# ZYM-PKU/UDiffText

Hardware: AMD Instinct MI355X
Metric: 512x512 50-step denoised images/sec (UDiffText hot path: conditioner + 50 CFG Euler steps + VAE decode) (higher is better)
Workload: dtype bf16; 1 GPU; 512x512, 50 Euler/DDIM(eta 0) steps, CFG 5.0, 9-char labels, noise_iters 0; global batch 4 per step sharded over 1 GPU(s) = 4 images per GPU in micro-batches of 4: every UNet call runs ONE batch of 4 (8 samples with CFG); 3 such batch(es) in flight per GPU on separate launch streams; BASELINE.json configs[1]; global_batch=4, weights=synthetic (name-keyed recipe), 1361.2 M parameters, launch=hipGraph replay of the sampler steps, in_flight=3, batches_per_unet_call=1

## Files before the change

include/udt_kernels.h:

```cpp
#ifndef UDT_KERNELS_H
#define UDT_KERNELS_H

#include <stddef.h>
#include <stdint.h>

#ifdef __cplusplus
extern "C" {
#endif

typedef enum {
  UDT_OK = 0,
  UDT_ERR_BAD_SHAPE = -1,
  UDT_ERR_BAD_ARG = -2,
  UDT_ERR_WORKSPACE = -3,
  UDT_ERR_HIP = -4,
  UDT_ERR_NO_DEVICE = -5,
  UDT_ERR_ASYNC = -6
} udt_status;

typedef enum {
  UDT_DTYPE_F32 = 0,
  UDT_DTYPE_BF16 = 1,
  UDT_DTYPE_FP8_E4M3 = 2
} udt_dtype;

#define UDT_GEMM_OUT_F32     (1 << 0)
#define UDT_GEMM_GEGLU       (1 << 1)
#define UDT_GEMM_RELU        (1 << 2)
#define UDT_GEMM_TRANSPOSED  (1 << 3)
#define UDT_GEMM_CONV        (1 << 4)
#define UDT_GEMM_SILU_OUT    (1 << 5)
#define UDT_GEMM_MX8         (1 << 7)

typedef struct {
  const void* a;
  const void* a2;
  const void* w;
  const float* bias;
  const void* residual;
  const float* rowvec;
  void* out;
  int32_t M, N, K;
  int32_t lda, ldo, ldr;
  int32_t ldw;
  int32_t batch;
  int64_t stride_a, stride_w, stride_out, stride_res;
  int32_t Hin, Win, C1, C2, Hout, Wout;
  int32_t ksize;
  int32_t stride;
  int32_t pad_t, pad_l;
  int32_t upsample;
  int32_t rows_per_batch;
  int32_t ld_rowvec;
  int32_t flags;
  float alpha;
  const float* colscale;
  const float* in_scsh;
  int32_t in_act;
  float* colstats;
  int32_t cu_share;
  const float* ln_colsum;
  float ln_eps;
  const void* a_scale;
  void* q8_out;
  void* q8_scale;
  int32_t ld_q8;
  int32_t q8_fixed_col;
  float q8_fixed_mul;
  float* rowstat_out;
  const float* rowstat_in;
  int32_t rowstat_in_parts;
} udt_gemm_desc;

size_t udt_gemm_workspace_bytes(const udt_gemm_desc* d);
int udt_gemm(const udt_gemm_desc* d, void* workspace, size_t workspace_bytes, void* stream);
int32_t udt_gemm_colstats_rows(const udt_gemm_desc* d);
int32_t udt_gemm_rowstat_parts(const udt_gemm_desc* d);
int32_t udt_gemm_q8_ok(const udt_gemm_desc* d);
int32_t udt_gemm_colstats_slots(const udt_gemm_desc* d);
int32_t udt_gemm_in_scsh_ok(const udt_gemm_desc* d);
int udt_gn_silu_conv3x3_fwd(const udt_gemm_desc* d, void* workspace, size_t workspace_bytes, void* stream);
int udt_ln_gemm_fwd(const udt_gemm_desc* d, void* workspace, size_t workspace_bytes, void* stream);
int udt_check_async_error(void* workspace, size_t workspace_bytes, void* stream);

int udt_attn_fwd(const void* q, const void* k, const void* vt, void* o,
                 int32_t batch, int32_t heads, int32_t nq, int32_t nk,
                 int32_t ldq, int32_t ldk, int32_t ldvt, int32_t ldo,
                 int64_t q_bstride, int64_t k_bstride, int64_t vt_bstride, int64_t o_bstride,
                 float scale, void* stream);

int udt_xattn_fwd(const void* q, const void* k, const void* v, void* o, float* probs,
                  int32_t batch, int32_t heads, int32_t head_dim, int32_t nq, int32_t L,
                  int32_t ldq, int32_t ldkv, int32_t ldo, float scale, void* stream);

int udt_attn_rowv_fwd(const void* q, const void* k, const void* v, void* o,
                      int32_t batch, int32_t heads, int32_t nq, int32_t nk,
                      int32_t ldq, int32_t ldk, int32_t ldv, int32_t ldo,
                      int64_t q_bstride, int64_t k_bstride, int64_t v_bstride, int64_t o_bstride,
                      float scale, void* stream);
int udt_attn_rowv_q8_fwd(const void* q, const void* k, const void* v, void* o,
                         int32_t batch, int32_t heads, int32_t nq, int32_t nk,
                         int32_t ldq, int32_t ldk, int32_t ldv, int32_t ldo,
                         int64_t q_bstride, int64_t k_bstride, int64_t v_bstride, int64_t o_bstride,
                         float scale, void* q8_out, void* q8_scale, int32_t ld_q8, void* stream);

int udt_attn_mx8_fwd(const void* qkv8, const void* qkv_scale, void* o, int32_t batch, int32_t heads, int32_t n,
                     int32_t ld8, int32_t ldo, float scale, float v_inv, void* q8_out, void* q8_scale, int32_t ld_q8,
                     void* stream);

int udt_attn512_fwd(const void* q, const void* k, const void* v, void* o,
                    int32_t batch, int32_t nq, int32_t nk,
                    int32_t ldq, int32_t ldk, int32_t ldv, int32_t ldo,
                    int64_t q_bstride, int64_t k_bstride, int64_t v_bstride, int64_t o_bstride,
                    float scale, void* stream);

size_t udt_attn512_workspace_bytes(int32_t batch, int32_t nq, int32_t nk);
int udt_attn512_split_fwd(const void* q, const void* k, const void* v, void* o,
                          int32_t batch, int32_t nq, int32_t nk,
                          int32_t ldq, int32_t ldk, int32_t ldv, int32_t ldo,
                          int64_t q_bstride, int64_t k_bstride, int64_t v_bstride, int64_t o_bstride,
                          float scale, void* workspace, size_t workspace_bytes, void* stream);

int udt_mattn_fwd(const void* q, const void* k, const void* v, void* o, const float* mask, const uint8_t* kpm,
                  int32_t batch, int32_t heads, int32_t head_dim, int32_t nq, int32_t lk,
                  int32_t ldq, int32_t ldk, int32_t ldv, int32_t ldo, int32_t ldmask,
                  int64_t q_bstride, int64_t k_bstride, int64_t v_bstride, int64_t o_bstride, float scale, void* stream);

int32_t udt_tattn_hp(int32_t heads);
int udt_tattn_prepare(const void* kv, int32_t ldkv, const void* wq, int32_t ldwq, const void* wo, int32_t ldwo,
                      const float* gamma, const float* beta, void* A, float* sc, void* BmT, int32_t B, int32_t L,
                      int32_t C, int32_t heads, float scale, void* stream);
int udt_tattn_fused(const void* x, void* out, const void* A, const float* sc, const void* BmT, const float* bias,
                    int32_t B, int32_t n_tok, int32_t C, int32_t heads, int32_t zero_samples, float eps, void* stream);
int32_t udt_tattn_rowstat_parts(int32_t B, int32_t n_tok, int32_t C);
int udt_tattn_fused_q8(const void* x, void* out, const void* A, const float* sc, const void* BmT, const float* bias,
                       int32_t B, int32_t n_tok, int32_t C, int32_t heads, int32_t zero_samples, float eps, void* q8_out,
                       void* q8_scale, float* rowstat_out, void* stream);

int udt_softmax_rows(void* x, int64_t rows, int32_t cols, int32_t ld, void* stream);

int32_t udt_gn_nchunks(int64_t HW, int32_t C);
int udt_gn_stats(const void* x, const void* x2, float* partials, int32_t B, int64_t HW, int32_t C, int32_t C2,
                 int32_t G, void* stream);
int udt_gn_apply(const void* x, const void* x2, void* y, const float* partials, const float* gamma,
                 const float* beta, int32_t B, int64_t HW, int32_t C, int32_t C2, int32_t G, float eps, int32_t act,
                 void* stream);
int32_t udt_gn_strip_ok(int32_t B, int64_t HW, int32_t C1, int32_t C2, int32_t G);
int udt_gn_strip(const void* x, const void* x2, void* y, const float* gamma, const float* beta, int32_t B, int64_t HW,
                 int32_t C1, int32_t C2, int32_t G, float eps, int32_t act, void* stream);

int udt_gn_finalize(const float* stats1, int32_t slots1, int32_t C1, const float* stats2, int32_t slots2, int32_t C2,
                    const float* gamma, const float* beta, float* scsh, int32_t B, int64_t HW, int32_t G, float eps,
                    void* stream);

int udt_gn_apply_scsh(const void* x, const void* x2, void* y, const float* scsh, int32_t B, int64_t HW, int32_t C1,
                      int32_t C2, int32_t act, void* stream);

int udt_gn_strip_stats(const void* x, const void* x2, void* y, const float* stats1, int32_t slots1, const float* stats2,
                       int32_t slots2, const float* gamma, const float* beta, int32_t B, int64_t HW, int32_t C1, int32_t C2,
                       int32_t G, float eps, int32_t act, void* stream);

int udt_layernorm(const void* x, void* y, const float* gamma, const float* beta,
                  int64_t rows, int32_t C, float eps, void* stream);
int udt_unet_input(const float* x, void* xin, int32_t B, int32_t hw, int32_t cpad, float c_in, void* stream);
int udt_cfg_euler_step(float* x, const float* eps, float* denoised_out, int32_t B, int32_t hw, int32_t ld_eps,
                       float c_out, float sigma, float sigma_next, float cfg_scale, void* stream);
typedef struct {
  float kx, kd, ka, kp, kn;
  float c_out, scale;
} udt_sampler_coefs;
int udt_cfg_sampler_step(const float* xin, const float* eps, const float* aux, const float* prev, const float* noise,
                         float* xout, float* denoised_out, int32_t B, int32_t hw, int32_t ld_eps, udt_sampler_coefs k,
                         void* stream);
#define UDT_MULTISTEP_MAX 8
typedef struct {
  float c_out, scale, sigma;
  int32_t n;
  float k[UDT_MULTISTEP_MAX];
  const float* hist[UDT_MULTISTEP_MAX];
} udt_multistep_coefs;
int udt_cfg_multistep_step(const float* xin, const float* eps, float* xout, float* d_out, int32_t B, int32_t hw,
                           int32_t ld_eps, udt_multistep_coefs k, void* stream);
int udt_posterior_sample(const float* moments, const float* noise, float* z, int32_t B, int32_t hw, int32_t ldm,
                         float scale, void* stream);
int udt_nchw_to_nhwc(const float* x, void* y, int32_t B, int32_t C, int64_t HW, int32_t cpad, float scale,
                     void* stream);
int udt_nhwc_to_nchw(const void* x, float* y, int32_t B, int32_t C, int64_t HW, int32_t ld, int32_t src_is_f32,
                     void* stream);
int udt_nhwc_set_channels(const float* src, void* dst, int32_t B, int32_t C, int64_t HW, int32_t cpad, int32_t c0,
                          void* stream);
int udt_embed_tokens(const int32_t* idx, const float* table, const float* pe, void* out, int32_t n_tok, int32_t L,
                     int32_t D, void* stream);
int udt_timestep_embedding(const float* t, void* out, int32_t n, int32_t dim, void* stream);
int udt_mask_downsample(const float* mask, float* out, int32_t B, int32_t H, int32_t W, void* stream);
int udt_local_loss(const float* probs, const float* mask, const float* seg_mask, const float* gkernel9,
                   float* loss_accum, int32_t B, int32_t heads, int32_t size, int32_t L, int32_t seg_l,
                   int32_t Hm, int32_t Wm, void* stream);
int udt_local_loss_tiled(const float* probs, const float* mask, const float* seg_mask, const float* gkernel9,
                         float* loss_accum, int32_t n_samples, int32_t mask_batch, int32_t heads, int32_t size, int32_t L,
                         int32_t seg_l, int32_t Hm, int32_t Wm, void* stream);
int udt_attn_bwd(const void* q, const void* k, const void* v, const void* o, const void* d_o, void* dq, void* dk, void* dv,
                 float* lse_ws, float* dsum_ws, int32_t batch, int32_t heads, int32_t n, int32_t ldq, int32_t ldo, int32_t ldd,
                 float scale, void* stream);
int udt_xattn_bwd(const void* k, const void* v, const float* probs, const float* d_probs, const void* d_o, void* dq, int32_t batch,
                  int32_t heads, int32_t head_dim, int32_t nq, int32_t L, int32_t ldkv, int32_t ldo, int32_t lddq, float scale,
                  void* stream);
int udt_local_loss_bwd(const float* probs, const float* mask, const float* seg_mask, const float* gkernel9, float* d_probs,
                       float* loss_accum, float* scratch , int32_t n_samples,
                       int32_t mask_batch, int32_t heads, int32_t size, int32_t L, int32_t seg_l, int32_t Hm, int32_t Wm, float weight,
                       void* stream);
int udt_local_loss_bwd_hw(const float* probs, const float* mask, const float* seg_mask, const float* gkernel9, float* d_probs,
                          float* loss_accum, float* scratch , int32_t n_samples, int32_t mask_batch,
                          int32_t heads, int32_t h, int32_t w, int32_t L, int32_t seg_l, int32_t Hm, int32_t Wm, float weight,
                          void* stream);
int udt_local_loss_tiled_hw(const float* probs, const float* mask, const float* seg_mask, const float* gkernel9, float* loss_accum,
                            float* scratch , int32_t n_samples, int32_t mask_batch, int32_t heads,
                            int32_t h, int32_t w, int32_t L, int32_t seg_l, int32_t Hm, int32_t Wm, void* stream);
int udt_layernorm_bwd(const void* x, const void* dy, const float* gamma, const void* add, void* dx, int64_t rows, int32_t C, float eps,
                      void* stream);
int udt_gn_bwd(const void* x, const void* dy, const float* gamma, const float* beta, const void* add, void* dx, float* partials, int32_t B,
               int32_t HW, int32_t C, int32_t groups, float eps, int32_t silu, void* stream);
int udt_geglu_fwd(const void* ag, void* out, int64_t rows, int32_t inner, void* stream);
int udt_geglu_bwd(const void* ag, const void* dy, void* dag, int64_t rows, int32_t inner, void* stream);
int udt_sum2x2_bf16(const void* dy, void* dx, int32_t B, int32_t H, int32_t W, int32_t C, void* stream);
int udt_center_tokens(const float* x, void* out, int32_t B, int32_t L, int32_t D, void* stream);
int udt_transpose_bf16(const void* in, void* out, int32_t R, int32_t C, int32_t ld, int32_t Rp, void* stream);
int udt_reduce_rows_f32(const float* in, float* out, int32_t P, int64_t n, int32_t accumulate, void* stream);
int32_t udt_colparts(int64_t rows);
int udt_colsum_bf16(const void* x, float* partials, float* out, int64_t rows, int32_t C, void* stream);
int udt_ln_param_grad(const void* x, const void* dy, float* partials, float* dgamma_dbeta, int64_t rows, int32_t C, float eps, void* stream);
int32_t udt_wgrad_splits(int64_t R, int32_t N, int32_t K);
int udt_wgrad_bf16(const void* dy, const void* x, float* dw, float* partials, int64_t R, int32_t N, int32_t K, int32_t ldy, int32_t ldx,
                   void* stream);
// ... 55 lines not shown
```

udifftext_amd/csrc/gemm.hip:

```cpp
#include "common.h"
#include <stdio.h>
#include <stdlib.h>
#include <string.h>
#include <atomic>
#include <cmath>

hipError_t udt_lean_launch_gemm(int cfg, const void* lparams, int smem, int G, int geglu, int ln, hipStream_t s);
hipError_t udt_lean_launch_conv3(const void* c3params, hipStream_t s);

namespace {
#include "tile_common.h"

struct GemmParams {
  const uint16_t* a;
  const uint16_t* a2;
  const uint16_t* w;
  const uint16_t* zero;
  const float* bias;
  const uint16_t* res;
  const float* rowvec;
  void* out;
  const float* colscale;
  const float* in_scsh;
  float* colstats;
// ... 728 lines not shown
  if (mx8 || emit) {
    if (conv1 || d->rowvec || mode == 0 || (mode > 0 && mode != 1)) return false;
    if (mx8 && (!d->a_scale || d->K % 128 != 0 || d->lda % 16 != 0 || (d->ldw > 0 && d->ldw % 16 != 0))) return false;
    if (mx8 && ln && (!d->rowstat_in || d->rowstat_in_parts <= 0)) return false;
    if (!mx8 && geglu) return false;
    if (mx8 && geglu && !(ln && emit)) return false;
    if (mx8 && !geglu && ln && emit && d->rowstat_out) return false;
    if (emit && (want_stats || !d->q8_scale || d->ld_q8 % 8 != 0 || d->N % (geglu ? 64 : 32) != 0)) return false;
    if (d->rowstat_out && (!emit || geglu)) return false;
    if (d->q8_fixed_col > 0 && (!emit || geglu || d->q8_fixed_col % 32 != 0 || !(d->q8_fixed_mul > 0.f))) return false;
    if ((reinterpret_cast<uintptr_t>(d->q8_out) | reinterpret_cast<uintptr_t>(d->colscale)) & 15) return false;
  } else if (d->rowstat_out || d->rowstat_in) {
    return false;
  }
  const int KT = mx8 ? 128 : BK;
  if (d->N <= 64 || d->N % 8 != 0 || d->K % KT != 0 || (!conv1 && d->lda % 8 != 0) || (d->ldo % 8 != 0 && d->out)) return false;
  if (d->residual && d->ldr % 8 != 0) return false;
  if (geglu && (d->N % 64 != 0 || d->residual || d->rowvec)) return false;
  const long long ldw = d->ldw > 0 ? d->ldw : d->K;
  const long long lda_eff = conv1 ? (d->C1 > d->C2 ? d->C1 : d->C2) : d->lda;
  if ((long long)d->M * lda_eff * 2 >= (1LL << 31) || (long long)d->N * ldw * 2 >= (1LL << 31)) return false;
  if (d->M >= (1 << 28)) return false;
  if ((reinterpret_cast<uintptr_t>(d->out) | reinterpret_cast<uintptr_t>(d->residual) | reinterpret_cast<uintptr_t>(d->bias) |
       reinterpret_cast<uintptr_t>(d->rowvec) | reinterpret_cast<uintptr_t>(d->ln_colsum)) & 15) return false;
  if (d->rowvec && ((d->ld_rowvec > 0 ? d->ld_rowvec : d->N) % 4 != 0)) return false;
  if (mode > 0 && mode != 1 && mode != 6 && mode != 7) return false;
  if (!mx8 && (!emit || (ln && !geglu && !d->rowstat_out)) && (mode == 7 || (mode < 0 && rowres_on()))) {
    const bool emit_fits = !emit || ((d->q8_fixed_col <= 0 || d->q8_fixed_col % 64 == 0) && (long long)d->M * d->ld_q8 < (1LL << 31) &&
                                     (long long)d->M * (d->out ? d->ldo : 0) * 2 < (1LL << 31) && (long long)((d->N + 127) / 128) * d->M * 4 < (1LL << 31));
    if (ln && !want_stats && d->K == 320 && d->N % 64 == 0 && !d->residual && !d->rowvec && !conv1 && emit_fits &&
        (reinterpret_cast<uintptr_t>(d->a) & 15) == 0) {
      const int tiles_m = (d->M + 255) / 256, chunks = d->N / 64;
      int ns = (device_cus() + tiles_m - 1) / tiles_m;
      if (ns > chunks / 4) ns = chunks / 4;
      const int cmax = geglu ? 20 : 16;
      const int ns_min = (chunks + cmax - 1) / cmax;
      if (ns < ns_min) ns = ns_min;
      const long long wgs = (long long)tiles_m * ns;
      if (ns >= 1 && (mode == 7 || emit || (geglu ? wgs * 4 >= 3LL * device_cus() : wgs >= device_cus()))) {
        t.cfg = 7; t.stats_rows = 0; t.nw = 4; t.bm = 256; t.bn = 64; t.smem = 0;
        t.tiles_m = tiles_m; t.kt_per = (chunks + ns - 1) / ns; t.tiles_n = (chunks + t.kt_per - 1) / t.kt_per;
        t.tiles = t.tiles_m * t.tiles_n; t.nkt = d->K / BK; t.splitk = 1; t.n_block = 1;
        t.G = round_workgroups(t.tiles);
        return true;
      }
    }
    if (mode == 7 || (emit && ln)) return false;
  }
  t.cfg = (mode > 0) ? mode : 1;
  if (!mx8 && !emit) {
  if (!geglu && d->N % 160 == 0 && d->N % 128 != 0 && t.cfg == 1) t.cfg = 5;
  if (mode <= 0 && d->N >= 768 && (long long)((d->M + 255) / 256) * ((d->N + 255) / 256) >= 2LL * device_cus() &&
      (d->cu_share <= 1 || lean256_under_lanes())) t.cfg = 6;
  }
  t.stats_rows = 0;
  if (want_stats) {
    if (t.cfg != 1 && t.cfg != 5) {
      if (mode > 0) return false;
      t.cfg = (d->N % 160 == 0 && d->N % 128 != 0) ? 5 : 1;
    }
    if (mx8) t.cfg = 1;
    t.stats_rows = t.cfg == 1 ? 64 : 32;
    const int rpb = d->rows_per_batch > 0 ? d->rows_per_batch : d->M;
    if (rpb % t.stats_rows != 0) return false;
  }
  switch (t.cfg) {
    case 1: t.nw = 4; t.bm = 128; t.bn = 128; t.smem = 2 * (128 + 128) * ROW_BYTES; break;
    case 5: t.nw = 4; t.bm = 128; t.bn = 160; t.smem = 128 * 160 * 4; break;
    case 6: t.nw = 8; t.bm = 256; t.bn = 256; t.smem = 2 * (256 + 256) * ROW_BYTES; break;
    default: return false;
  }
  {
    const int epi = (t.cfg == 6 ? t.bm * t.bn : t.bm * t.bn * 4) + ((ln && t.cfg != 5) ? t.bm * 8 : 0);
    if (t.smem < epi) t.smem = epi;
  }
  t.tiles_m = (d->M + t.bm - 1) / t.bm;
  t.tiles_n = (d->N + t.bn - 1) / t.bn;
  t.tiles = t.tiles_m * t.tiles_n;
  t.nkt = d->K / KT;
  int slots = device_cus() * ((t.cfg == 1 || t.cfg == 5) ? 2 : 1) / share_of(d);
  if (slots < 1) slots = 1;
  int sk = 1;
  const int knob = lean_splitk_knob();
  if (!ln && t.tiles <= 1023) {
    if (knob > 1) sk = knob;
    else if (knob < 0 && t.tiles * 2 <= slots && t.nkt >= (mx8 ? 20 : 40)) { sk = slots / t.tiles; if (sk > t.nkt / (mx8 ? 8 : 16)) sk = t.nkt / (mx8 ? 8 : 16); }
    if (sk > t.nkt / 4) sk = t.nkt / 4;
    while (sk > 1 && (long long)t.tiles * sk * t.bm * t.bn * 4 > (64LL << 20)) --sk;
    if (sk < 1) sk = 1;
  }
  t.kt_per = (t.nkt + sk - 1) / sk;
  t.splitk = (t.nkt + t.kt_per - 1) / t.kt_per;
  const int units = t.tiles * t.splitk;
  t.G = round_workgroups(units);
  int nb = g_n_block.load(std::memory_order_relaxed);
  if (nb <= 0) nb = (t.tiles_m <= 8) ? t.tiles_n : 8;
  if (nb > t.tiles_n) nb = t.tiles_n;
  t.n_block = nb;
  return true;
}

size_t lean_workspace(const LeanPlan& t) {
  return t.splitk > 1 ? G8_HEADER_BYTES + (size_t)t.tiles * t.splitk * t.bm * t.bn * sizeof(float) : 0;
}

std::atomic<int> g_lean_conv{-1};
std::atomic<int> g_wide_conv{-2};
int wide_conv_mode() {
  int v = g_wide_conv.load(std::memory_order_relaxed);
  if (v == -2) {
    const char* e = getenv("UDT_WIDE_CONV");
    v = e ? atoi(e) : -1;
    g_wide_conv.store(v, std::memory_order_relaxed);
  }
  return v;
}
#ifdef UDT_MEASURE
std::atomic<int> g_lconv_dbg{0};
#endif

std::atomic<int> g_wide_lanes_eff{-2};
double wide_lanes_eff() {
  int v = g_wide_lanes_eff.load(std::memory_order_relaxed);
  if (v == -2) {
    const char* e = getenv("UDT_WIDE_LANES_EFF");
    v = e ? atoi(e) : 70;
    g_wide_lanes_eff.store(v, std::memory_order_relaxed);
  }
  return v / 100.0;
}

int conv_chunk_slices(long long tiles, int slots, int chunks, int knob) {
  long long sk = 1;
  if (tiles <= 1023) {
    if (knob > 1) { sk = knob; if (sk > chunks) sk = chunks; }
    else if (knob < 0 && tiles * 2 <= slots && chunks >= 10) { sk = slots / tiles; if (sk > chunks / 4) sk = chunks / 4; }
    if (sk < 1) sk = 1;
  }
  return (int)sk;
}

bool lean_conv_plan(const udt_gemm_desc* d, lg::C3Params& c, bool want_stats) {
  int on = g_lean_conv.load(std::memory_order_relaxed);
  if (on < 0) {
    const char* e = getenv("UDT_LEAN_CONV");
    on = (e && e[0] == '0') ? 0 : 1;
    g_lean_conv.store(on, std::memory_order_relaxed);
  }
  if (!on || lean_mode() == 0) return false;
  if (d->flags != UDT_GEMM_CONV || d->ksize != 3 || d->stride != 1 || d->pad_t != 1 || d->pad_l != 1) return false;
  if (d->C2 != 0 || d->in_scsh || d->colscale || d->batch > 1) return false;
  if (want_stats && !lean_stats_enabled()) return false;
  if (d->N < 128 || d->N % 8 != 0 || d->C1 <= 0 || d->C1 % 64 != 0) return false;
  const bool ups = d->upsample != 0;
  if (d->Hout != (d->Hin << (ups ? 1 : 0)) || d->Wout != (d->Win << (ups ? 1 : 0))) return false;
  c.bn = 128; c.wgm = 2;
  bool wide = false;
  int wide_slots = device_cus();
  {
    const int wm = wide_conv_mode();
    if (wm != 0 && !ups && d->N % 160 == 0 && d->Wout % 16 == 0 && d->Hout % 16 == 0) {
      const int cus = device_cus(), share = d->cu_share > 1 ? d->cu_share : 1;
      wide_slots = cus / share > 0 ? cus / share : 1;
      const long long wt = (long long)(d->M / 256) * (d->N / 160);
      const long long sk = conv_chunk_slices(wt, wide_slots, d->C1 / 64, lean_splitk_knob());
      const long long units = wt * sk;
      const long long rounds = (units + cus - 1) / cus;
      const double eff = units > cus ? (double)units / (double)(rounds * cus) : ((double)units * share >= cus ? 1.0 : (double)units * share / cus);
      wide = (wm > 0) || (sk <= 2 && eff >= ((share >= 3 && share_of(d) >= 3) ? wide_lanes_eff() : 0.85));
    }
  }
  if (wide) { c.geo = 3; c.tw = 16; c.th = 16; c.bn = 160; c.wgm = 4; }
  else if (d->Wout % 16 == 0 && d->Hout % 8 == 0) { c.geo = ups ? 2 : 0; c.tw = 16; c.th = 8; }
  else if (!ups && d->Wout % 8 == 0 && d->Hout % 8 == 0) { c.geo = 1; c.tw = 8; c.th = 8; }
  else return false;
  if (d->ldo % 8 != 0 || (d->residual && d->ldr % 8 != 0)) return false;
  const long long ldw = d->ldw > 0 ? d->ldw : d->K;
  if ((long long)d->M * d->C1 * 2 >= (1LL << 31) || (long long)d->N * ldw * 2 >= (1LL << 31)) return false;
  if ((reinterpret_cast<uintptr_t>(d->out) | reinterpret_cast<uintptr_t>(d->residual) | reinterpret_cast<uintptr_t>(d->bias) |
       reinterpret_cast<uintptr_t>(d->rowvec)) & 15) return false;
  if (d->rowvec && ((d->ld_rowvec > 0 ? d->ld_rowvec : d->N) % 4 != 0)) return false;
  c.dbg = 0;
#ifdef UDT_MEASURE
  c.dbg = g_lconv_dbg.load(std::memory_order_relaxed);
#endif
  c.N = d->N; c.C = d->C1; c.H = d->Hin; c.W = d->Win; c.B = d->M / (d->Hout * d->Wout);
  c.ldw = (int)ldw; c.ldo = d->ldo; c.ldr = d->ldr; c.ldrv = d->ld_rowvec > 0 ? d->ld_rowvec : d->N;
  c.alpha = d->alpha;
  c.tiles_x = d->Wout / c.tw; c.tiles_y = d->Hout / c.th;
  c.tiles_m = c.B * c.tiles_x * c.tiles_y;
  c.tiles_n = (d->N + c.bn - 1) / c.bn;
  c.tiles = c.tiles_m * c.tiles_n;
  c.chunks = c.C / 64;
  const int slots = c.geo == 3 ? wide_slots : (2 * device_cus() / share_of(d) > 0 ? 2 * device_cus() / share_of(d) : 1);
  int sk = conv_chunk_slices(c.tiles, slots, c.chunks, lean_splitk_knob());
  while (sk > 1 && (long long)c.tiles * sk * c.tw * c.th * c.bn * 4 > (64LL << 20)) --sk;
  c.ch_per = (c.chunks + sk - 1) / sk;
  c.splitk = (c.chunks + c.ch_per - 1) / c.ch_per;
  c.G = round_workgroups(c.tiles * c.splitk);
  {
    const double patch = (double)((ups ? c.tw / 2 : c.tw) + 2) * ((ups ? c.th / 2 : c.th) + 2) * c.C * 2.0, wtile = 9.0 * c.bn * c.C * 2.0;
    int nb = g_n_block.load(std::memory_order_relaxed);
    if (nb <= 0) nb = (int)(std::sqrt(64.0 * patch / wtile) + 0.5);
    if (nb < 1) nb = 1;
    if (nb > c.tiles_n) nb = c.tiles_n;
    c.n_block = nb;
  }
  c.a_bytes = (unsigned)((long long)c.B * d->Hin * d->Win * d->C1 * 2);
  c.w_bytes = (unsigned)((long long)d->N * ldw * 2);
  c.counters = nullptr; c.slabs = nullptr;
  return true;
}

size_t lean_conv_workspace(const lg::C3Params& c) {
  return c.splitk > 1 ? G8_HEADER_BYTES + (size_t)c.tiles * c.splitk * c.tw * c.th * c.bn * sizeof(float) : 0;
}

bool lean_stats_probe(const udt_gemm_desc* d, int& rows, int& slots) {
  if (d->in_scsh) return false;
  {
    lg::C3Params c3;
    if (lean_conv_plan(d, c3, true)) {
      rows = c3.tw * c3.th / c3.wgm;
      slots = c3.tiles_m * c3.wgm;
      return true;
    }
  }
  if ((d->flags & UDT_GEMM_CONV) && d->ksize == 3) return false;
  LeanPlan lt;
  if (lean_plan(d, lt, true)) {
    rows = lt.stats_rows;
    slots = lt.tiles_m * (lt.bm / lt.stats_rows);
    return true;
  }
  return false;
}
}

extern "C" int udt_debug_set(const char* key, int32_t value) {
  if (!key) return UDT_ERR_BAD_ARG;
  if (!strcmp(key, "n_block")) { g_n_block.store(value); return UDT_OK; }
  if (!strcmp(key, "rows_epi")) { g_rows_epi.store(value ? 1 : 0); return UDT_OK; }
  if (!strcmp(key, "lean")) { g_lean.store(value < 0 ? -2 : value); return UDT_OK; }
  if (!strcmp(key, "rowres")) { g_rowres.store(value < 0 ? 1 : (value ? 1 : 0)); return UDT_OK; }
  if (!strcmp(key, "wide_lanes_eff")) { g_wide_lanes_eff.store(value < 0 ? -2 : value); return UDT_OK; }
  if (!strcmp(key, "conv_n4")) { g_conv_n4.store(value < 0 ? -2 : (value ? 1 : 0)); return UDT_OK; }
  if (!strcmp(key, "lean256_lanes")) { g_lean256_lanes.store(value < 0 ? -2 : (value ? 1 : 0)); return UDT_OK; }
  if (!strcmp(key, "lean_splitk")) { g_lean_splitk.store(value); return UDT_OK; }
  if (!strcmp(key, "share_splitk")) { g_share_splitk.store(value < 0 ? -2 : (value ? 1 : 0)); return UDT_OK; }
  if (!strcmp(key, "lean_conv")) { g_lean_conv.store(value < 0 ? -1 : (value ? 1 : 0)); return UDT_OK; }
  if (!strcmp(key, "wide_conv")) { g_wide_conv.store(value < 0 ? -1 : (value ? 1 : 0)); return UDT_OK; }
#ifdef UDT_MEASURE
  if (!strcmp(key, "lconv_dbg")) { g_lconv_dbg.store(value); return UDT_OK; }
  static const struct { const char* k; int bit; } bits[] = {{"no_xchg", 28}, {"no_epi", 27}, {"no_store", 26}, {"no_res", 25},
                                                            {"no_bias", 24}, {"no_fast", 22}};
  for (const auto& b : bits)
    if (!strcmp(key, b.k)) {
      int cur = g_dbg_bits.load();
      g_dbg_bits.store((cur & ~(1 << b.bit)) | (value ? (1 << b.bit) : 0));
      return UDT_OK;
    }
#endif
  return UDT_ERR_BAD_ARG;
}

extern "C" int udt_check_async_error(void* workspace, size_t workspace_bytes, void* stream) {
  if (!workspace || workspace_bytes < G8_HEADER_BYTES) return UDT_ERR_BAD_ARG;
  hipStream_t s = reinterpret_cast<hipStream_t>(stream);
  int err = 0;
  hipError_t e = hipMemcpyAsync(&err, reinterpret_cast<int*>(workspace) + 1023, sizeof(int), hipMemcpyDeviceToHost, s);
  if (e == hipSuccess) e = hipStreamSynchronize(s);
  if (e != hipSuccess) return udt_set_hip_error(e);
  if (err == 0) return UDT_OK;
  e = hipMemsetAsync(workspace, 0, G8_HEADER_BYTES, s);
  if (e == hipSuccess) e = hipStreamSynchronize(s);
  if (e != hipSuccess) return udt_set_hip_error(e);
  return UDT_ERR_ASYNC;
}

extern "C" int32_t udt_gemm_colstats_rows(const udt_gemm_desc* d) { return d ? colstats_rows(d) : 0; }
extern "C" int32_t udt_gemm_colstats_slots(const udt_gemm_desc* d) { return d ? colstats_slots(d) : 0; }
extern "C" int32_t udt_gemm_q8_ok(const udt_gemm_desc* d) {
  if (!d || !d->q8_out || d->M <= 0 || d->N <= 0 || d->K <= 0) return 0;
  LeanPlan lt;
  return lean_plan(d, lt, d->colstats != nullptr) ? 1 : 0;
}

extern "C" int32_t udt_gemm_rowstat_parts(const udt_gemm_desc* d) {
  if (!d || d->M <= 0 || d->N <= 0 || d->K <= 0) return 0;
  udt_gemm_desc t = *d;
  alignas(16) static const uint64_t probe_dst[2] = {0, 0};
  if (!t.q8_out) { t.q8_out = const_cast<uint64_t*>(probe_dst); t.q8_scale = const_cast<uint64_t*>(probe_dst); if (t.ld_q8 <= 0) t.ld_q8 = (t.N + 15) / 16 * 16; }
  LeanPlan lt;
  if (!lean_plan(&t, lt, false) || lt.cfg != 1 || (d->flags & UDT_GEMM_GEGLU)) return 0;
  return (d->N + 63) / 64;
}
extern "C" int32_t udt_gemm_in_scsh_ok(const udt_gemm_desc* d) {
  if (!d || d->K <= 0 || d->K % BK != 0) return 0;
  c3p::Geo ge;
  return conv3p_geometry(d, ge, true) ? 1 : 0;
}

extern "C" int udt_gn_silu_conv3x3_fwd(const udt_gemm_desc* d, void* workspace, size_t workspace_bytes, void* stream) {
  if (!d || !(d->flags & UDT_GEMM_CONV) || d->ksize != 3 || d->stride != 1 || d->pad_t != 1 || d->pad_l != 1 || !d->in_scsh)
    return UDT_ERR_BAD_ARG;
  return udt_gemm(d, workspace, workspace_bytes, stream);
}

extern "C" int udt_ln_gemm_fwd(const udt_gemm_desc* d, void* workspace, size_t workspace_bytes, void* stream) {
  if (!d || !d->ln_colsum || !d->bias || !(d->ln_eps > 0.f)) return UDT_ERR_BAD_ARG;
  LeanPlan lt;
  if (!lean_plan(d, lt, false)) return UDT_ERR_BAD_SHAPE;
  return udt_gemm(d, workspace, workspace_bytes, stream);
}

extern "C" size_t udt_gemm_workspace_bytes(const udt_gemm_desc* d) {
  if (!d || d->K <= 0 || d->M <= 0 || d->N <= 0 || d->K % k_tile(d) != 0) return 0;
  if (conv_n4_applies(d)) return 0;
  {
    LeanPlan lt;
    if (lean_plan(d, lt, d->colstats != nullptr)) return lean_workspace(lt);
    lg::C3Params c3;
    if (lean_conv_plan(d, c3, d->colstats != nullptr)) return lean_conv_workspace(c3);
  }
  {
    c3p::Geo ge;
    if (conv3p_geometry(d, ge, d->in_scsh != nullptr)) {
      TilePlan t3 = plan_tiles3p(d, ge);
      if (!t3.fixup) return 0;
      return G8_HEADER_BYTES + (size_t)t3.G * t3.bm * t3.bn * sizeof(float);
    }
  }
  if (use_gemm8(d)) {
    TilePlan t8 = plan_tiles8(d);
    if (!t8.fixup) return 0;
    return G8_HEADER_BYTES + (size_t)t8.G * t8.bm * t8.bn * sizeof(float);
  }
  TilePlan t = plan_tiles(d);
  if (t.bm != 256 || !t.fixup) return 0;
  return G8_HEADER_BYTES + (size_t)t.G * 2 * SLAB_FLOATS * sizeof(float);
}

extern "C" int udt_gemm(const udt_gemm_desc* d, void* workspace, size_t workspace_bytes, void* stream) {
  if (!d || !d->a || !d->w) return UDT_ERR_BAD_ARG;
  if (d->M <= 0 || d->N <= 0 || d->K <= 0) return UDT_ERR_BAD_SHAPE;
  if (d->K % k_tile(d) != 0) return UDT_ERR_BAD_SHAPE;
  if (d->N % 4 != 0) return UDT_ERR_BAD_SHAPE;
  const bool mx8 = (d->flags & UDT_GEMM_MX8) != 0;
  if (mx8 || d->q8_out || d->rowstat_out || d->rowstat_in) {
    LeanPlan lt8;
    if (!lean_plan(d, lt8, d->colstats != nullptr)) return UDT_ERR_BAD_ARG;
  } else if (d->colscale) {
    return UDT_ERR_BAD_ARG;
  }
  const bool conv = (d->flags & UDT_GEMM_CONV) != 0;
  const bool trans = (d->flags & UDT_GEMM_TRANSPOSED) != 0;
  const int batch = d->batch > 0 ? d->batch : 1;
  if (conv) {
    if (d->ksize != 1 && d->ksize != 3) return UDT_ERR_BAD_SHAPE;
    if (d->C1 <= 0 || d->C1 % BK != 0 || d->C2 % BK != 0) return UDT_ERR_BAD_SHAPE;
    if (d->C2 > 0 && !d->a2) return UDT_ERR_BAD_ARG;
    if (d->K != d->ksize * d->ksize * (d->C1 + d->C2)) return UDT_ERR_BAD_SHAPE;
    if (d->Hout <= 0 || d->Wout <= 0 || d->M % (d->Hout * d->Wout) != 0) return UDT_ERR_BAD_SHAPE;
    if (d->stride != 1 && d->stride != 2) return UDT_ERR_BAD_SHAPE;
    if (trans || batch != 1) return UDT_ERR_BAD_ARG;
  } else {
    if (d->lda < d->K || d->lda % 8 != 0) return UDT_ERR_BAD_SHAPE;
  }
  if (!d->out && !d->q8_out) return UDT_ERR_BAD_ARG;
  if (trans) {
    if (d->rows_per_batch <= 0 || d->rows_per_batch % 4 != 0 || d->M % d->rows_per_batch != 0)
      return UDT_ERR_BAD_SHAPE;
    if (d->flags & (UDT_GEMM_OUT_F32 | UDT_GEMM_GEGLU | UDT_GEMM_RELU | UDT_GEMM_SILU_OUT)) return UDT_ERR_BAD_ARG;
    if (d->residual || d->rowvec || batch != 1) return UDT_ERR_BAD_ARG;
  } else {
    if (d->ldo % 4 != 0) return UDT_ERR_BAD_SHAPE;
    if (d->residual && d->ldr % 4 != 0) return UDT_ERR_BAD_SHAPE;
  }
  if (d->flags & UDT_GEMM_GEGLU) {
    if (d->N % 64 != 0 || (d->flags & UDT_GEMM_OUT_F32) || d->residual || d->rowvec) return UDT_ERR_BAD_ARG;
  }
  if (d->rowvec && d->rows_per_batch <= 0) return UDT_ERR_BAD_ARG;

  hipStream_t s = reinterpret_cast<hipStream_t>(stream);
  if (conv_n4_applies(d)) {
    cn4::Params cp;
    cp.a = reinterpret_cast<const uint16_t*>(d->a); cp.w = reinterpret_cast<const uint16_t*>(d->w); cp.bias = d->bias;
    cp.out = reinterpret_cast<float*>(d->out);
    cp.B = d->M / (d->Hout * d->Wout); cp.H = d->Hin; cp.W = d->Win; cp.C = d->C1;
    cp.ldw = d->ldw > 0 ? d->ldw : d->K; cp.ldo = d->ldo;
    cp.tiles_x = (d->Win + 7) / 8; cp.tiles_y = (d->Hin + 7) / 8;
    const size_t smem = (size_t)100 * (d->C1 + 8) * 2 + (size_t)4 * 9 * d->C1 * 2;
    static AttrOnce once;
    hipError_t ea = once.ensure(reinterpret_cast<const void*>(cn4::conv3x3_n4_kernel), 100 * (512 + 8) * 2 + 4 * 9 * 512 * 2);
    if (ea != hipSuccess) return udt_set_hip_error(ea);
    UdtProfScope profn(0, s);
    if (profn.rec) {
      char tag[96];
      snprintf(tag, sizeof(tag), "conv_n4 M=%d N=%d K=%d %dx%d", d->M, d->N, d->K, d->Hin, d->Win);
      udt_prof_tag(profn.rec, tag);
    }
    hipLaunchKernelGGL(cn4::conv3x3_n4_kernel, dim3((unsigned)(cp.B * cp.tiles_x * cp.tiles_y)), dim3(256), smem, s, cp);
    UDT_CHECK_LAUNCH();
    return UDT_OK;
  }
  TilePlan t = plan_tiles(d);

  GemmParams p;
  p.a = reinterpret_cast<const uint16_t*>(d->a);
  p.a2 = reinterpret_cast<const uint16_t*>(d->a2);
  p.w = reinterpret_cast<const uint16_t*>(d->w);
  p.zero = udt_zero_page();
  if (!p.zero) return UDT_ERR_HIP;
  p.bias = d->bias;
  p.res = reinterpret_cast<const uint16_t*>(d->residual);
  p.rowvec = d->rowvec;
  p.out = d->out;
  p.colscale = d->colscale;
  p.in_scsh = d->in_scsh;
  p.in_act = d->in_act;
  p.colstats = d->colstats;
  p.slabs = nullptr;
  if (d->colstats && colstats_rows(d) == 0) return UDT_ERR_BAD_ARG;
  if (d->in_scsh && !udt_gemm_in_scsh_ok(d)) return UDT_ERR_BAD_ARG;
  if (d->in_act != 0 && d->in_act != 1) return UDT_ERR_BAD_ARG;
  p.M = d->M; p.N = d->N; p.K = d->K;
  p.lda = d->lda; p.ldo = d->ldo; p.ldr = d->ldr;
  p.ldw = d->ldw > 0 ? d->ldw : d->K;
  if (p.ldw < d->K || p.ldw % 8 != 0) return UDT_ERR_BAD_SHAPE;
  if (mx8 && d->lda < d->K) return UDT_ERR_BAD_SHAPE;
  p.sA = d->stride_a; p.sW = d->stride_w; p.sO = d->stride_out; p.sR = d->stride_res;
  p.Hin = d->Hin; p.Win = d->Win; p.C1 = d->C1; p.C2 = d->C2; p.Hout = d->Hout; p.Wout = d->Wout;
  p.ksz = d->ksize; p.stride = d->stride; p.pad_t = d->pad_t; p.pad_l = d->pad_l; p.ups = d->upsample ? 1 : 0;
  p.rows_per_batch = d->rows_per_batch > 0 ? d->rows_per_batch : d->M;
  p.ldrv = d->ld_rowvec > 0 ? d->ld_rowvec : d->N;
  if (d->flags & ~PUBLIC_FLAGS) return UDT_ERR_BAD_ARG;
  p.flags = d->flags | (g_rows_epi.load(std::memory_order_relaxed) ? 0 : INTERNAL_DIRECT_EPI);
#ifdef UDT_MEASURE
  p.flags |= g_dbg_bits.load(std::memory_order_relaxed);
#endif
  p.n_block = 1;
  p.alpha = d->alpha;
  const int cls = (conv && d->ksize == 3) ? 0 : 1;
  {
    LeanPlan lt;
    if (lean_plan(d, lt, d->colstats != nullptr)) {
      lg::LParams lp;
      lp.colstats = d->colstats;
      const bool conv1 = (d->flags & UDT_GEMM_CONV) != 0;
      lp.a = p.a; lp.a2 = (conv1 && d->C2 > 0) ? p.a2 : nullptr; lp.w = p.w; lp.bias = p.bias; lp.res = p.res; lp.rowvec = p.rowvec;
      lp.ln_s = d->ln_colsum;
      lp.out = reinterpret_cast<uint16_t*>(d->out);
      lp.M = d->M; lp.N = d->N; lp.K = d->K;
      lp.lda = conv1 ? d->C1 : p.lda; lp.ldw = p.ldw; lp.ldo = p.ldo; lp.ldr = p.ldr; lp.ldrv = p.ldrv; lp.rows_per_batch = p.rows_per_batch;
      lp.lda2 = conv1 ? d->C2 : 0;
      lp.kt_split = (conv1 && d->C2 > 0) ? d->C1 / BK : lt.nkt;
      lp.a2_bytes = (unsigned)((long long)d->M * (conv1 ? d->C2 : 0) * 2);
      lp.alpha = d->alpha; lp.ln_eps = d->ln_eps;
      lp.tiles_m = lt.tiles_m; lp.tiles_n = lt.tiles_n; lp.n_block = lt.n_block; lp.tiles = lt.tiles;
      lp.nkt = lt.nkt; lp.splitk = lt.splitk; lp.kt_per = lt.kt_per;
      lp.a_bytes = (unsigned)((long long)d->M * lp.lda * elem_bytes(d));
      lp.w_bytes = (unsigned)((long long)d->N * p.ldw * elem_bytes(d));
      lp.a_scale = mx8 ? reinterpret_cast<const uint32_t*>(d->a_scale) : nullptr;
      lp.colscale = d->colscale;
      lp.rowstat_in = d->rowstat_in; lp.rowstat_in_parts = d->rowstat_in_parts;
      lp.q8_out = reinterpret_cast<uint8_t*>(d->q8_out); lp.q8_scale = reinterpret_cast<uint32_t*>(d->q8_scale); lp.ld_q8 = d->ld_q8;
      lp.rowstat_out = d->rowstat_out;
      lp.q8_fixed_col = d->q8_fixed_col > 0 ? d->q8_fixed_col : 0x7fffffff;
      lp.q8_fixed_mul = d->q8_fixed_mul;
      lp.G = lt.G;
      lp.counters = nullptr; lp.slabs = nullptr;
      if (lt.splitk > 1) {
        if (!workspace || workspace_bytes < lean_workspace(lt)) return UDT_ERR_WORKSPACE;
        lp.counters = reinterpret_cast<int*>(workspace);
        lp.slabs = reinterpret_cast<float*>(reinterpret_cast<char*>(workspace) + G8_HEADER_BYTES);
      }
      UdtProfScope profl(cls, s);
      if (profl.rec) {
        char tag[96];
        snprintf(tag, sizeof(tag), "lean%d%s%s M=%d N=%d K=%d fl=0x%x ln=%d tile=%dx%d units=%d splitk=%d", lt.cfg, mx8 ? "-mx8" : "", d->q8_out ? "+q8" : "",
                 d->M, d->N, d->K, d->flags, d->ln_colsum ? 1 : 0, lt.bm, lt.bn, lt.tiles * lt.splitk, lt.splitk);
        udt_prof_tag(profl.rec, tag);
      }
      const bool geglu = (d->flags & UDT_GEMM_GEGLU) != 0, ln = d->ln_colsum != nullptr;
      hipError_t el;
      el = udt_lean_launch_gemm(lt.cfg, &lp, lt.smem, lt.G, geglu ? 1 : 0, ln ? 1 : 0, s);
      if (el != hipSuccess) return udt_set_hip_error(el);
      return UDT_OK;
    }
  }
  if (d->ln_colsum) return UDT_ERR_BAD_ARG;
  {
    lg::C3Params c3;
    if (lean_conv_plan(d, c3, d->colstats != nullptr)) {
      c3.colstats = d->colstats;
      c3.a = p.a; c3.w = p.w; c3.bias = p.bias; c3.res = p.res; c3.rowvec = p.rowvec; c3.out = reinterpret_cast<uint16_t*>(d->out);
      if (c3.splitk > 1) {
        if (!workspace || workspace_bytes < lean_conv_workspace(c3)) return UDT_ERR_WORKSPACE;
        c3.counters = reinterpret_cast<int*>(workspace);
        c3.slabs = reinterpret_cast<float*>(reinterpret_cast<char*>(workspace) + G8_HEADER_BYTES);
      }
      UdtProfScope profc(cls, s);
      if (profc.rec) {
        char tag[96];
        snprintf(tag, sizeof(tag), "%s%s M=%d N=%d K=%d %dx%d tile=%dx%d units=%d splitk=%d nb=%d", c3.geo == 3 ? "wconv3" : "lconv3", d->upsample ? "+up" : "", d->M, d->N, d->K,
                 d->Hin, d->Win, c3.tw, c3.th, c3.tiles * c3.splitk, c3.splitk, c3.n_block);
        udt_prof_tag(profc.rec, tag);
      }
      const hipError_t ec = udt_lean_launch_conv3(&c3, s);
      if (ec != hipSuccess) return udt_set_hip_error(ec);
      return UDT_OK;
    }
  }
  {
    c3p::CParams cp;
    if (conv3p_geometry(d, cp.geo, d->in_scsh != nullptr)) {
      const TilePlan t3 = plan_tiles3p(d, cp.geo);
      p.tiles_m = t3.tiles_m; p.tiles_n = t3.tiles_n; p.tiles_per_batch = t3.tiles_m * t3.tiles_n;
      {
        const double patch = (double)cp.geo.prows_img * cp.geo.NI * cp.geo.C * 2.0;
        const double wtile = 9.0 * t3.bn * cp.geo.C * 2.0;
        const double S = (double)(t3.tiles < t3.G ? t3.tiles : t3.G) / 8.0;
        int nb = (int)(std::sqrt((S < 1.0 ? 1.0 : S) * patch / wtile) + 0.5);
        if (nb < 1) nb = 1;
        if (nb > t3.tiles_n) nb = t3.tiles_n;
        p.n_block = nb;
      }
      p.n_ktiles = t3.nkt;
      p.total_iters = t3.total;
      p.iters_per_wg = t3.ipw;
      p.G = t3.G;
      const long long in_px = (long long)cp.geo.B * d->Hin * d->Win;
      cp.base.a_bytes = (unsigned)(in_px * d->C1 * 2);
      cp.a2_bytes = (unsigned)((long long)d->M * d->C2 * 2);
      cp.scsh_bytes = (unsigned)((long long)cp.geo.B * cp.geo.chunks * 512);
      cp.base.w_bytes = (unsigned)((long long)d->N * p.ldw * 2);
      cp.base.g = p;
      cp.base.flags = nullptr; cp.base.err = nullptr; cp.base.slab_base = nullptr;
      if (t3.fixup) {
        const size_t need = G8_HEADER_BYTES + (size_t)t3.G * t3.bm * t3.bn * sizeof(float);
        if (!workspace || workspace_bytes < need) return UDT_ERR_WORKSPACE;
        cp.base.flags = reinterpret_cast<int*>(workspace);
        cp.base.err = cp.base.flags + 1023;
        cp.base.slab_base = reinterpret_cast<float*>(reinterpret_cast<char*>(workspace) + G8_HEADER_BYTES);
      }
      UdtProfScope prof3(cls, s);
      if (prof3.rec) {
        char tag[96];
        snprintf(tag, sizeof(tag), "conv3p%s%s M=%d N=%d K=%d %dx%d tile=%dx%dx%d bn=%d G=%d ipw=%d", d->in_scsh ? "+gn" : "", d->upsample ? "+up" : "", d->M,
                 d->N, d->K, d->Hin, d->Win, cp.geo.TW, cp.geo.TH, cp.geo.NI, t3.bn, t3.G, t3.ipw);
        udt_prof_tag(prof3.rec, tag);
      }
      hipError_t e3;
      const bool st3 = d->colstats != nullptr;
      if (t3.bn == 160) e3 = st3 ? launch3p<8, 1, 1, 5, true, true>(cp, t3, s) : launch3p<8, 1, 1, 5, true, false>(cp, t3, s);
      else e3 = st3 ? launch3p<4, 2, 2, 2, true, true>(cp, t3, s) : launch3p<4, 2, 2, 2, true, false>(cp, t3, s);
      if (e3 != hipSuccess) return udt_set_hip_error(e3);
      return UDT_OK;
    }
  }
  if (use_gemm8(d)) {
    const TilePlan t8 = plan_tiles8(d);
    p.tiles_m = t8.tiles_m; p.tiles_n = t8.tiles_n; p.tiles_per_batch = t8.tiles_m * t8.tiles_n;
    const int n_block_knob = g_n_block.load(std::memory_order_relaxed);
    if (n_block_knob != 0 && !conv) {
      const long long wt = (long long)t8.bn * d->K * elem_bytes(d);
      long long nb = 1;
      if (n_block_knob > 0) nb = n_block_knob;
      else if (t8.tiles_m <= 8 || trans) nb = t8.tiles_n;
      else if (t8.tiles_n >= 8) nb = (4LL << 20) / (wt > 0 ? wt : 1);
      if (nb < 1) nb = 1;
      if (nb > t8.tiles_n) nb = t8.tiles_n;
      p.n_block = (int)nb;
    }
    p.n_ktiles = t8.nkt;
    p.total_iters = t8.total;
    p.iters_per_wg = t8.ipw;
    p.G = t8.G;
    g8::Params pp;
    pp.g = p;
    pp.flags = nullptr; pp.err = nullptr; pp.slab_base = nullptr;
    pp.a_bytes = conv ? 0u : (unsigned)((long long)d->M * d->lda * elem_bytes(d));
    pp.w_bytes = (unsigned)((long long)d->N * p.ldw * elem_bytes(d));
    if (t8.fixup) {
      const size_t need = G8_HEADER_BYTES + (size_t)t8.G * t8.bm * t8.bn * sizeof(float);
      if (!workspace || workspace_bytes < need) return UDT_ERR_WORKSPACE;
      pp.flags = reinterpret_cast<int*>(workspace);
      pp.err = pp.flags + 1023;
      pp.slab_base = reinterpret_cast<float*>(reinterpret_cast<char*>(workspace) + G8_HEADER_BYTES);
    }
    UdtProfScope prof8(cls, s);
    if (prof8.rec) {
      char tag[96];
      snprintf(tag, sizeof(tag), "gemm8 M=%d N=%d K=%d conv=%d ks=%d fl=0x%x tile=%dx%d G=%d ipw=%d b=%d",
               d->M, d->N, d->K, conv ? 1 : 0, d->ksize, d->flags, t8.bm, t8.bn, t8.G, t8.ipw, batch);
      udt_prof_tag(prof8.rec, tag);
    }
    hipError_t e8;
    const bool st = d->colstats != nullptr;
    if (t8.bn == 160) {
      if (st) e8 = conv ? launch8<8, 1, 1, 5, true, false, true>(pp, t8, s) : launch8<8, 1, 1, 5, false, false, true>(pp, t8, s);
      else e8 = conv ? launch8<8, 1, 1, 5, true, false>(pp, t8, s) : launch8<8, 1, 1, 5, false, false>(pp, t8, s);
    } else if (trans) {
      e8 = launch8<4, 2, 2, 2, false, true>(pp, t8, s);
    } else if (st) {
      e8 = conv ? launch8<4, 2, 2, 2, true, false, true>(pp, t8, s) : launch8<4, 2, 2, 2, false, false, true>(pp, t8, s);
    } else {
      e8 = conv ? launch8<4, 2, 2, 2, true, false>(pp, t8, s) : launch8<4, 2, 2, 2, false, false>(pp, t8, s);
    }
    if (e8 != hipSuccess) return udt_set_hip_error(e8);
    return UDT_OK;
  }

  p.tiles_m = t.tiles_m; p.tiles_n = t.tiles_n; p.tiles_per_batch = t.tiles_m * t.tiles_n;
  p.n_ktiles = t.nkt;
  p.total_iters = t.total;
  p.iters_per_wg = t.ipw;
  p.G = t.G;

  if (t.fixup) {
    const size_t need = G8_HEADER_BYTES + (size_t)t.G * 2 * SLAB_FLOATS * sizeof(float);
    if (!workspace || workspace_bytes < need) return UDT_ERR_WORKSPACE;
    p.slabs = reinterpret_cast<float*>(reinterpret_cast<char*>(workspace) + G8_HEADER_BYTES);
  }

  UdtProfScope prof(cls, s);
  if (prof.rec) {
    char tag[96];
    snprintf(tag, sizeof(tag), "gemm M=%d N=%d K=%d conv=%d ks=%d fl=0x%x tile=%dx%d G=%d ipw=%d b=%d", d->M, d->N, d->K,
             conv ? 1 : 0, d->ksize, d->flags, t.bm, t.bn, t.G, t.ipw, batch);
    udt_prof_tag(prof.rec, tag);
  }

  if (t.bm != 256) return UDT_ERR_BAD_SHAPE;
  const hipError_t e = conv ? launch_cfg<256, 64, 4, 1, true, false>(p, t, s) : launch_cfg<256, 64, 4, 1, false, false>(p, t, s);
  if (e != hipSuccess) return udt_set_hip_error(e);
  return UDT_OK;
}
```

udifftext_amd/csrc/lean.h:

```cpp
#pragma once

namespace lg {

using g8::wait_vm;
UDT_DEVINL void raw_barrier() {
  asm volatile("s_waitcnt lgkmcnt(0)" ::: "memory");
  __builtin_amdgcn_s_barrier();
  asm volatile("" ::: "memory");
}
using g8::buf_lds16;
using g8::OOB;

typedef __attribute__((ext_vector_type(2))) __bf16 bf2_t;
UDT_DEVINL float dot2_bf16(uint32_t a, uint32_t b, float c) {
  return __builtin_amdgcn_fdot2_f32_bf16(__builtin_bit_cast(bf2_t, a), __builtin_bit_cast(bf2_t, b), c, false);
}

template <int CPR, int RPI>
UDT_DEVINL void wave_colstats(char* wl, int lane, const float (&cs)[8], const float (&cq)[8], float* dst, bool col_ok) {
#pragma unroll
  for (int h = 0; h < 2; ++h) {
    f32x4 a = {cs[4 * h + 0], cs[4 * h + 1], cs[4 * h + 2], cs[4 * h + 3]};
    f32x4 b = {cq[4 * h + 0], cq[4 * h + 1], cq[4 * h + 2], cq[4 * h + 3]};
    *reinterpret_cast<f32x4*>(wl + lane * 64 + h * 16) = a;
// ... 450 lines not shown
      if (p.res) {
#pragma unroll
        for (int i = 0; i < NIT; ++i) {
          const int row = i * RPI + rl;
          const int m = m0 + row0 + prow0 + row;
          u32x4 z = {0u, 0u, 0u, 0u};
          rv[i] = z;
          if (col_ok && row < PROWS && m < p.M) rv[i] = *reinterpret_cast<const u32x4*>(p.res + (long long)m * p.ldr + n);
        }
      }
#pragma unroll
      for (int tb = 0; tb < TMB; ++tb) {
        const int row = tb * 32 + l31;
#pragma unroll
        for (int tn = 0; tn < TN; ++tn)
#pragma unroll
          for (int q = 0; q < 4; ++q) {
            const int chunk = (tn * 8 + q * 2 + hi) ^ (row & 7);
            const f32x16& a16 = acc[pass * TMB + tb][tn];
            f32x4 v = {a16[q * 4 + 0], a16[q * 4 + 1], a16[q * 4 + 2], a16[q * 4 + 3]};
            *reinterpret_cast<f32x4*>(wl + row * EROW + chunk * 16) = v;
          }
      }
#pragma unroll
      for (int i = 0; i < NIT; ++i) {
        const int row = i * RPI + rl;
        const int m = m0 + row0 + prow0 + row;
        const bool ok = col_ok && row < PROWS && m < p.M;
        const int rr = row < PROWS ? row : 0;
        const char* rp = wl + rr * EROW;
        const int sw = rr & 7;
        const f32x4 v0 = *reinterpret_cast<const f32x4*>(rp + (((2 * c8) ^ sw) << 4));
        const f32x4 v1 = *reinterpret_cast<const f32x4*>(rp + (((2 * c8 + 1) ^ sw) << 4));
        float o[8];
#pragma unroll
        for (int j = 0; j < 4; ++j) {
          o[j] = v0[j];
          o[4 + j] = v1[j];
        }
        if constexpr (FP8) {
#pragma unroll
          for (int j = 0; j < 4; ++j) o[j] *= w0[j], o[4 + j] *= w1[j];
        }
        if constexpr (LN) {
          float mean, rstd;
          row_stats(prow0 + rr, mean, rstd);
#pragma unroll
          for (int j = 0; j < 4; ++j) {
            o[j] = rstd * (o[j] - mean * s0[j]);
            o[4 + j] = rstd * (o[4 + j] - mean * s1[j]);
          }
        }
#pragma unroll
        for (int j = 0; j < 4; ++j) {
          o[j] = o[j] * p.alpha + b0[j];
          o[4 + j] = o[4 + j] * p.alpha + b1[j];
        }
        if (p.rowvec && ok) {
          const float* rvp = p.rowvec + (long long)(m / p.rows_per_batch) * p.ldrv + n;
          const f32x4 r0 = *reinterpret_cast<const f32x4*>(rvp);
          const f32x4 r1 = *reinterpret_cast<const f32x4*>(rvp + 4);
#pragma unroll
          for (int j = 0; j < 4; ++j) {
            o[j] += r0[j];
            o[4 + j] += r1[j];
          }
        }
        if (p.res) {
#pragma unroll
          for (int j = 0; j < 4; ++j) {
            o[2 * j] += bf16_lo(rv[i][j]);
            o[2 * j + 1] += bf16_hi(rv[i][j]);
          }
        }
        if constexpr (EMIT) {
          {
            const u32x4 rb = {pack_bf16x2(o[0], o[1]), pack_bf16x2(o[2], o[3]), pack_bf16x2(o[4], o[5]), pack_bf16x2(o[6], o[7])};
#pragma unroll
            for (int j = 0; j < 4; ++j) o[2 * j] = bf16_lo(rb[j]), o[2 * j + 1] = bf16_hi(rb[j]);
          }
          uint32_t sb;
          u32x2 q8 = mx8_quant_row8(o, sb);
          if (n >= p.q8_fixed_col) {
            q8 = e4m3_fixed_row8(o, p.q8_fixed_mul);
            sb = 127u;
          }
          float ps = 0.f, pq = 0.f;
          if (p.rowstat_out) {
            static_assert(CPR == 8 || CPR == 16, "row statistics: 64- or 128-column wave blocks");
#pragma unroll
            for (int j = 0; j < 8; ++j) ps += o[j], pq += o[j] * o[j];
            ps = dpp_add<0xB1>(ps); pq = dpp_add<0xB1>(pq);
            ps = dpp_add<0x4E>(ps); pq = dpp_add<0x4E>(pq);
            ps = dpp_add<0x141>(ps); pq = dpp_add<0x141>(pq);
            if constexpr (CPR == 16) { ps = dpp_add<0x140>(ps); pq = dpp_add<0x140>(pq); }
          }
          if (ok) {
            *reinterpret_cast<u32x2*>(p.q8_out + (long long)m * p.ld_q8 + n) = q8;
            if ((c8 & 3) == 0) reinterpret_cast<uint8_t*>(p.q8_scale)[((long long)(n >> 7) * p.M + m) * 4 + ((n >> 5) & 3)] = (uint8_t)sb;
            if (p.rowstat_out && c8 == 0) {
              f32x2 st2 = {ps, pq};
              reinterpret_cast<f32x2*>(p.rowstat_out)[(long long)((n0 + col0) / WCOLS) * p.M + m] = st2;
            }
          }
        }
        if (ok) {
          u32x4 pk = {pack_bf16x2(o[0], o[1]), pack_bf16x2(o[2], o[3]), pack_bf16x2(o[4], o[5]), pack_bf16x2(o[6], o[7])};
          if (!EMIT || p.out) *reinterpret_cast<u32x4*>(p.out + (long long)m * p.ldo + n) = pk;
          if constexpr (STATS) {
#pragma unroll
            for (int j = 0; j < 4; ++j) {
              const float a = bf16_lo(pk[j]), bb = bf16_hi(pk[j]);
              cs[2 * j] += a; cq[2 * j] += a * a;
              cs[2 * j + 1] += bb; cq[2 * j + 1] += bb * bb;
            }
          }
        }
      }
    }
    if constexpr (STATS) {
      const int slot = (m0 + row0) / WROWS;
      wave_colstats<CPR, RPI>(wl, lane, cs, cq, p.colstats + ((long long)slot * p.N + n) * 2, col_ok);
    }
  }
}


template <int MAXN>
UDT_DEVINL void wait_vm_upto(int n) {
  if constexpr (MAXN == 0) wait_vm<0>();
  else {
    if (n >= MAXN) wait_vm<MAXN>();
    else wait_vm_upto<MAXN - 1>(n);
  }
}

template <int TW, int TH, bool UPS>
struct C3Geo {
  static constexpr int PX = TW * TH;
  static constexpr int TM = PX / 64;
  static constexpr int PW = (UPS ? TW / 2 : TW) + 2, PH = (UPS ? TH / 2 : TH) + 2;
  static constexpr int PROWS = PW * PH;
  static constexpr int PIECES = (PROWS + 7) / 8;
  static constexpr int PATCH_BYTES = PIECES * 1024;
  static constexpr int W_BYTES = 128 * ROW_BYTES;
  static constexpr int NRING = (3 * W_BYTES + 2 * PATCH_BYTES <= 80 * 1024) ? 3 : 2;
  static constexpr int RING = NRING * W_BYTES + 2 * PATCH_BYTES;
  static constexpr int STAGING = 4 * TM * 32 * 256;
  static constexpr int SMEM = RING > STAGING ? RING : STAGING;
  static_assert(PX == 128 || PX == 64, "128 or 64 output pixels per workgroup");
  static_assert(SMEM <= 80 * 1024, "two workgroups per CU");
};

template <int TW, int TH, bool UPS, bool STATS = false>
__global__ void __launch_bounds__(256, 2) lconv3_kernel(const C3Params p) {
  using Geo = C3Geo<TW, TH, UPS>;
  constexpr int NW = 4, TM = Geo::TM, TN = 2, BN = 128, BMPX = Geo::PX;
  constexpr int C3_PW = Geo::PW, C3_PROWS = Geo::PROWS, C3_PIECES = Geo::PIECES, C3_PATCH_BYTES = Geo::PATCH_BYTES;
  constexpr int C3_W_BYTES = Geo::W_BYTES, C3_TW = TW, C3_TH = TH;
  constexpr int WROWS = TM * 32;
  constexpr int WP = 4;
  constexpr int PP = (C3_PIECES + NW - 1) / NW;
  constexpr int EROW = 64 * 4;
  extern __shared__ __attribute__((aligned(16))) char smem[];
  char* const wring = smem;
  constexpr int NR = Geo::NRING;
  char* const patches = smem + NR * C3_W_BYTES;

  const int tid = threadIdx.x;
  const int wave = __builtin_amdgcn_readfirstlane(tid >> 6);
  const int lane = tid & 63;
  const int l31 = lane & 31;
  const int hi = lane >> 5;
  const int l3 = lane >> 3;
  const int pslot = lane & 7;
  const int wm = wave >> 1, wn = wave & 1;
  const int row0 = wm * WROWS, col0 = wn * 64;
  const int swz_w = (l31 >> 1) & 7;
  const int w_frag_row = (col0 + l31) * ROW_BYTES;

  const int unit = range_index(blockIdx.x, p.G);
  if (unit >= p.tiles * p.splitk) return;
  const int tile = unit / p.splitk;
  const int slice = unit - tile * p.splitk;
  int tile_m, n0;
  {
    const int per_block = p.tiles_m * p.n_block;
    const int blk = tile / per_block;
    const int r = tile - blk * per_block;
    int nbw = p.tiles_n - blk * p.n_block;
    if (nbw > p.n_block) nbw = p.n_block;
    tile_m = r / nbw;
    n0 = (blk * p.n_block + (r - tile_m * nbw)) * BN;
  }
  const int per_img = p.tiles_x * p.tiles_y;
  const int b = tile_m / per_img;
  const int rt = tile_m - b * per_img;
  const int ty = rt / p.tiles_x;
  const int y0 = ty * C3_TH, x0 = (rt - ty * p.tiles_x) * C3_TW;
  const int c0 = slice * p.ch_per;
  int c1 = c0 + p.ch_per;
  if (c1 > p.chunks) c1 = p.chunks;

  const __amdgpu_buffer_rsrc_t rsrc_a = __builtin_amdgcn_make_buffer_rsrc(const_cast<uint16_t*>(p.a), 0, p.a_bytes, 0x00020000);
  const __amdgpu_buffer_rsrc_t rsrc_w = __builtin_amdgcn_make_buffer_rsrc(const_cast<uint16_t*>(p.w), 0, p.w_bytes, 0x00020000);
  auto patch_swz = [](int prow, int yy) { return ((prow - 2 * yy) >> 1) & 7; };
  unsigned w_voff[WP], p_voff[PP];
  int p_piece[PP];
#pragma unroll
  for (int i = 0; i < WP; ++i) {
    const int row = (wave + NW * i) * 8 + l3;
    const int kw = (pslot ^ ((row >> 1) & 7)) * 8;
    const int n = n0 + row;
    w_voff[i] = (n < p.N) ? (unsigned)(((long long)n * p.ldw + kw) * 2) : OOB;
  }
#pragma unroll
  for (int i = 0; i < PP; ++i) {
    int idx = wave + NW * i;
    while (idx >= C3_PIECES) idx -= NW;
    p_piece[i] = idx;
    const int prow = idx * 8 + l3;
    const int yy = prow / C3_PW;
    const int xx = prow - yy * C3_PW;
    const int gy = (UPS ? (y0 >> 1) : y0) + yy - 1, gx = (UPS ? (x0 >> 1) : x0) + xx - 1;
    const bool ok = (prow < C3_PROWS) && ((unsigned)gy < (unsigned)p.H) && ((unsigned)gx < (unsigned)p.W);
    const int koff = (pslot ^ patch_swz(prow, yy)) * 8;
    p_voff[i] = ok ? (unsigned)(((((long long)b * p.H + gy) * p.W + gx) * p.C + koff) * 2) : OOB;
  }
  int a_prow[TM], a_py[TM];
#pragma unroll
  for (int tm = 0; tm < TM; ++tm) {
    const int ml = row0 + tm * 32 + l31;
    const int py = ml / TW, px = ml - py * TW;
    a_py[tm] = py;
    a_prow[tm] = UPS ? (py | (px << 16)) : (py * C3_PW + px);
  }
  auto issue_w = [&](int st, int c, int tap) {
    const int soff = (tap * p.C + c * 64) * 2;
    char* wbuf = wring + st * C3_W_BYTES;
#pragma unroll
    for (int i = 0; i < WP; ++i) buf_lds16(rsrc_w, wbuf + (wave + NW * i) * 1024, w_voff[i], soff);
  };
  auto issue_patch = [&](int c) {
    char* pbuf = patches + (c & 1) * C3_PATCH_BYTES;
#pragma unroll
    for (int i = 0; i < PP; ++i) buf_lds16(rsrc_a, pbuf + p_piece[i] * 1024, p_voff[i], c * 128);
  };

  f32x16 acc[TM][TN];
#pragma unroll
  for (int i = 0; i < TM; ++i)
#pragma unroll
    for (int j = 0; j < TN; ++j)
#pragma unroll
      for (int r = 0; r < 16; ++r) acc[i][j][r] = 0.f;

  issue_patch(c0);
#pragma unroll
  for (int j = 0; j < NR - 1; ++j) issue_w(j, c0, j);
  int st = 0;
  for (int c = c0; c < c1; ++c) {
    const bool nxt = (c + 1 < c1);
    const char* pbuf = patches + (c & 1) * C3_PATCH_BYTES;
#pragma unroll
    for (int tap = 0; tap < 9; ++tap) {
      {
        const int w_ahead = nxt ? NR - 2 : ((8 - tap) < NR - 2 ? (8 - tap) : NR - 2);
        const bool patch_ahead = nxt && tap >= 1 && tap <= NR - 1;
        wait_vm_upto<(NR - 2) * WP + PP>(w_ahead * WP + (patch_ahead ? PP : 0));
      }
      raw_barrier();
      if (!UDT_DBG(p.dbg, 0)) {
        const int ahead = tap + NR - 1;
        int s2 = st + NR - 1;
        if (s2 >= NR) s2 -= NR;
        if (ahead < 9) issue_w(s2, c, ahead);
        else if (nxt) issue_w(s2, c + 1, ahead - 9);
      }
      if (tap == 0 && nxt && !UDT_DBG(p.dbg, 1)) issue_patch(c + 1);
      const int dy = tap / 3, dx = tap - dy * 3;
      const char* wbuf = wring + st * C3_W_BYTES;
      bf16x8_t fx[4][TM], fw[4][TN];
      if (!UDT_DBG(p.dbg, 3)) {
#pragma unroll
        for (int t = 0; t < TM; ++t) {
          int prow, yy;
          if constexpr (UPS) {
            const int py = a_prow[t] & 0xffff, px = a_prow[t] >> 16;
            yy = ((py + dy - 1) >> 1) + 1;
            prow = yy * C3_PW + (((px + dx - 1) >> 1) + 1);
          } else {
            yy = a_py[t] + dy;
            prow = a_prow[t] + dy * C3_PW + dx;
          }
          const int arow = prow * ROW_BYTES, aswz = patch_swz(prow, yy);
#pragma unroll
          for (int ks = 0; ks < 4; ++ks) fx[ks][t] = lds_read_frag(pbuf + arow + (((ks * 2 + hi) ^ aswz) << 4));
        }
#pragma unroll
        for (int ks = 0; ks < 4; ++ks) {
          const int slot = ((ks * 2 + hi) ^ swz_w) << 4;
#pragma unroll
          for (int t = 0; t < TN; ++t) fw[ks][t] = lds_read_frag(wbuf + w_frag_row + t * 32 * ROW_BYTES + slot);
        }
      }
      if (UDT_DBG(p.dbg, 2)) {
#pragma unroll
        for (int ks = 0; ks < 4; ++ks) {
#pragma unroll
          for (int tm = 0; tm < TM; ++tm) asm volatile("" ::"v"(fx[ks][tm]));
#pragma unroll
          for (int tn = 0; tn < TN; ++tn) asm volatile("" ::"v"(fw[ks][tn]));
        }
      } else {
#pragma unroll
        for (int ks = 0; ks < 4; ++ks)
#pragma unroll
          for (int tm = 0; tm < TM; ++tm)
#pragma unroll
            for (int tn = 0; tn < TN; ++tn) acc[tm][tn] = mfma32(fw[ks][tn], fx[ks][tm], acc[tm][tn]);
      }
      st = (st + 1 == NR) ? 0 : st + 1;
    }
  }
  raw_barrier();

  if (p.splitk > 1) {
    f32x4* slab = reinterpret_cast<f32x4*>(p.slabs + (long long)unit * (BMPX * BN));
#pragma unroll
    for (int tm = 0; tm < TM; ++tm)
#pragma unroll
      for (int tn = 0; tn < TN; ++tn)
#pragma unroll
        for (int q = 0; q < 4; ++q) {
          f32x4 v = {acc[tm][tn][q * 4 + 0], acc[tm][tn][q * 4 + 1], acc[tm][tn][q * 4 + 2], acc[tm][tn][q * 4 + 3]};
          store16_sc1(slab + ((tm * TN + tn) * 4 + q) * 256 + tid, v);
        }
    asm volatile("s_waitcnt vmcnt(0)" ::: "memory");
    __syncthreads();
    int* const bcast = reinterpret_cast<int*>(smem);
    if (tid == 0) {
      const int t = __hip_atomic_fetch_add(p.counters + tile, 1, __ATOMIC_RELAXED, __HIP_MEMORY_SCOPE_AGENT);
      const int last = (t == p.splitk - 1) ? 1 : 0;
      if (last) {
        __builtin_amdgcn_fence(__ATOMIC_ACQUIRE, "agent");
        __hip_atomic_store(p.counters + tile, 0, __ATOMIC_RELAXED, __HIP_MEMORY_SCOPE_AGENT);
      }
      *bcast = last;
    }
    __syncthreads();
    const bool last = *bcast != 0;
    __syncthreads();
    if (!last) return;
#pragma unroll
    for (int i = 0; i < TM; ++i)
#pragma unroll
      for (int j = 0; j < TN; ++j)
#pragma unroll
        for (int r = 0; r < 16; ++r) acc[i][j][r] = 0.f;
    for (int s = 0; s < p.splitk; ++s) {
      const f32x4* sl = reinterpret_cast<const f32x4*>(p.slabs + ((long long)tile * p.splitk + s) * (BMPX * BN));
#pragma unroll
      for (int tm = 0; tm < TM; ++tm)
#pragma unroll
        for (int tn = 0; tn < TN; ++tn)
#pragma unroll
          for (int q = 0; q < 4; ++q) {
            const f32x4 v = sl[((tm * TN + tn) * 4 + q) * 256 + tid];
#pragma unroll
            for (int r = 0; r < 4; ++r) acc[tm][tn][q * 4 + r] += v[r];
          }
    }
  }

  char* const wl = smem + wave * (WROWS * EROW);
#pragma unroll
  for (int tm = 0; tm < TM; ++tm) {
    const int row = tm * 32 + l31;
#pragma unroll
    for (int tn = 0; tn < TN; ++tn)
#pragma unroll
      for (int q = 0; q < 4; ++q) {
        const int chunk = (tn * 8 + q * 2 + hi) ^ (row & 7);
        f32x4 v = {acc[tm][tn][q * 4 + 0], acc[tm][tn][q * 4 + 1], acc[tm][tn][q * 4 + 2], acc[tm][tn][q * 4 + 3]};
        *reinterpret_cast<f32x4*>(wl + row * EROW + chunk * 16) = v;
      }
  }
  const int rl = lane >> 3, c8 = lane & 7;
  const int n = n0 + col0 + c8 * 8;
  const bool col_ok = n < p.N;
  f32x4 b0 = {0.f, 0.f, 0.f, 0.f}, b1 = b0;
  if (col_ok) {
    if (p.bias) {
      b0 = *reinterpret_cast<const f32x4*>(p.bias + n);
      b1 = *reinterpret_cast<const f32x4*>(p.bias + n + 4);
    }
    if (p.rowvec) {
      const float* rvp = p.rowvec + (long long)b * p.ldrv + n;
      const f32x4 r0 = *reinterpret_cast<const f32x4*>(rvp), r1 = *reinterpret_cast<const f32x4*>(rvp + 4);
#pragma unroll
      for (int j = 0; j < 4; ++j) b0[j] += r0[j], b1[j] += r1[j];
    }
  }
  constexpr int NIT = TM * 4;
  const int Ho = UPS ? 2 * p.H : p.H, Wo = UPS ? 2 * p.W : p.W;
  long long mrow[NIT];
#pragma unroll
  for (int i = 0; i < NIT; ++i) {
    const int ml = row0 + i * 8 + rl;
    const int py = ml / TW, px = ml - py * TW;
    mrow[i] = ((long long)b * Ho + (y0 + py)) * Wo + (x0 + px);
  }
  u32x4 rv[NIT];
  if (p.res) {
#pragma unroll
    for (int i = 0; i < NIT; ++i) {
      u32x4 z = {0u, 0u, 0u, 0u};
      rv[i] = z;
      if (col_ok) rv[i] = *reinterpret_cast<const u32x4*>(p.res + mrow[i] * p.ldr + n);
    }
  }
  float cs[8], cq[8];
#pragma unroll
  for (int j = 0; j < 8; ++j) cs[j] = cq[j] = 0.f;
#pragma unroll
  for (int i = 0; i < NIT; ++i) {
    const int row = i * 8 + rl;
    const char* rp = wl + row * EROW;
    const int sw = row & 7;
    const f32x4 v0 = *reinterpret_cast<const f32x4*>(rp + (((2 * c8) ^ sw) << 4));
    const f32x4 v1 = *reinterpret_cast<const f32x4*>(rp + (((2 * c8 + 1) ^ sw) << 4));
    float o[8];
#pragma unroll
    for (int j = 0; j < 4; ++j) {
      o[j] = v0[j] * p.alpha + b0[j];
      o[4 + j] = v1[j] * p.alpha + b1[j];
    }
    if (p.res) {
#pragma unroll
      for (int j = 0; j < 4; ++j) {
        o[2 * j] += bf16_lo(rv[i][j]);
        o[2 * j + 1] += bf16_hi(rv[i][j]);
      }
    }
    if (col_ok) {
      u32x4 pk = {pack_bf16x2(o[0], o[1]), pack_bf16x2(o[2], o[3]), pack_bf16x2(o[4], o[5]), pack_bf16x2(o[6], o[7])};
      *reinterpret_cast<u32x4*>(p.out + mrow[i] * p.ldo + n) = pk;
      if constexpr (STATS) {
#pragma unroll
        for (int j = 0; j < 4; ++j) {
          const float a = bf16_lo(pk[j]), bb = bf16_hi(pk[j]);
          cs[2 * j] += a; cq[2 * j] += a * a;
          cs[2 * j + 1] += bb; cq[2 * j + 1] += bb * bb;
        }
      }
    }
  }
  if constexpr (STATS) {
    const int slot = tile_m * 2 + wm;
    wave_colstats<8, 8>(wl, lane, cs, cq, p.colstats + ((long long)slot * p.N + n) * 2, col_ok);
  }
}

}
```

udifftext_amd/csrc/lean.hip:

```cpp
#include "common.h"
#include <stdio.h>
#include <stdlib.h>
#include <atomic>

namespace {
#include "tile_common.h"
#include "lean_params.h"
#include "lean.h"
#include "wide.h"
#include "rowres.h"

template <int NW, int WGM, int WGN, int TM, int TN, int NST, int TMB = TM>
hipError_t launch_lean(const lg::LParams& lp, int smem, int G, bool geglu, bool ln, hipStream_t s) {
  static AttrOnce once[5];
  const void* fn;
  const bool stats = lp.colstats != nullptr;
  if constexpr (NW == 4 && NST == 2) {
    if (stats) {
      fn = (const void*)lg::lgemm_kernel<NW, WGM, WGN, TM, TN, NST, false, false, TMB, true>;
      hipError_t e = once[4].ensure(fn, smem);
      if (e != hipSuccess) return e;
      void* args[] = {const_cast<lg::LParams*>(&lp)};
      return hipLaunchKernel(fn, dim3(G), dim3(NW * 64), args, smem, s);
    }
  }
  if (stats) return hipErrorInvalidValue;
  if constexpr (TN == 2) {
    fn = geglu ? (ln ? (const void*)lg::lgemm_kernel<NW, WGM, WGN, TM, TN, NST, true, true, TMB> : (const void*)lg::lgemm_kernel<NW, WGM, WGN, TM, TN, NST, true, false, TMB>)
               : (ln ? (const void*)lg::lgemm_kernel<NW, WGM, WGN, TM, TN, NST, false, true, TMB> : (const void*)lg::lgemm_kernel<NW, WGM, WGN, TM, TN, NST, false, false, TMB>);
  } else {
    fn = ln ? (const void*)lg::lgemm_kernel<NW, WGM, WGN, TM, TN, NST, false, true, TMB> : (const void*)lg::lgemm_kernel<NW, WGM, WGN, TM, TN, NST, false, false, TMB>;
  }
  hipError_t e = once[(geglu ? 2 : 0) + (ln ? 1 : 0)].ensure(fn, smem);
  if (e != hipSuccess) return e;
  void* args[] = {const_cast<lg::LParams*>(&lp)};
  return hipLaunchKernel(fn, dim3(G), dim3(NW * 64), args, smem, s);
}

template <bool GEGLU, bool LN, bool STATS, bool FP8, bool EMIT>
hipError_t launch_lean_mx8_k(const lg::LParams& lp, int smem, int G, hipStream_t s) {
  static AttrOnce once;
  const void* fn = (const void*)lg::lgemm_kernel<4, 2, 2, 2, 2, 2, GEGLU, LN, 2, STATS, FP8, EMIT>;
  hipError_t e = once.ensure(fn, smem);
  if (e != hipSuccess) return e;
  void* args[] = {const_cast<lg::LParams*>(&lp)};
  return hipLaunchKernel(fn, dim3(G), dim3(256), args, smem, s);
}
hipError_t launch_lean_mx8(const lg::LParams& lp, int smem, int G, bool geglu, bool ln, bool fp8, bool emit, hipStream_t s) {
  const bool stats = lp.colstats != nullptr;
  if (!fp8) {
    if (emit && !geglu && !ln && !stats) return launch_lean_mx8_k<false, false, false, false, true>(lp, smem, G, s);
    return hipErrorInvalidValue;
  }
  if (geglu) return (ln && emit && !stats) ? launch_lean_mx8_k<true, true, false, true, true>(lp, smem, G, s) : hipErrorInvalidValue;
  if (ln) return stats ? hipErrorInvalidValue
                 : emit ? launch_lean_mx8_k<false, true, false, true, true>(lp, smem, G, s)
                        : launch_lean_mx8_k<false, true, false, true, false>(lp, smem, G, s);
  if (stats) return emit ? hipErrorInvalidValue : launch_lean_mx8_k<false, false, true, true, false>(lp, smem, G, s);
  return emit ? launch_lean_mx8_k<false, false, false, true, true>(lp, smem, G, s) : launch_lean_mx8_k<false, false, false, true, false>(lp, smem, G, s);
}

template <int TW, int TH, bool UPS, bool STATS>
hipError_t launch_lconv3s(const lg::C3Params& c3, hipStream_t s) {
  static AttrOnce once;
  constexpr int smem = lg::C3Geo<TW, TH, UPS>::SMEM;
  hipError_t e = once.ensure(reinterpret_cast<const void*>(lg::lconv3_kernel<TW, TH, UPS, STATS>), smem);
  if (e != hipSuccess) return e;
  hipLaunchKernelGGL((lg::lconv3_kernel<TW, TH, UPS, STATS>), dim3(c3.G), dim3(256), smem, s, c3);
  return hipGetLastError();
}
template <int TW, int TH, bool UPS>
hipError_t launch_lconv3(const lg::C3Params& c3, hipStream_t s) {
  return c3.colstats ? launch_lconv3s<TW, TH, UPS, true>(c3, s) : launch_lconv3s<TW, TH, UPS, false>(c3, s);
}

template <bool STATS>
hipError_t launch_wconv3s(const lg::C3Params& c3, hipStream_t s) {
  static AttrOnce once;
  constexpr int smem = wd::WGeo::SMEM;
  hipError_t e = once.ensure(reinterpret_cast<const void*>(wd::wconv3_kernel<STATS>), smem);
  if (e != hipSuccess) return e;
  hipLaunchKernelGGL((wd::wconv3_kernel<STATS>), dim3(c3.G), dim3(256), smem, s, c3);
  return hipGetLastError();
}
template <int KT, bool GEGLU, bool EMIT = false>
hipError_t launch_rowres(const lg::LParams& lp, int G, hipStream_t s) {
  static AttrOnce once;
  constexpr int smem = rr::RGeo<KT, GEGLU>::SMEM;
  hipError_t e = once.ensure(reinterpret_cast<const void*>(rr::rgemm_kernel<KT, GEGLU, EMIT>), smem);
  if (e != hipSuccess) return e;
  hipLaunchKernelGGL((rr::rgemm_kernel<KT, GEGLU, EMIT>), dim3(G), dim3(256), smem, s, lp);
  return hipGetLastError();
}

hipError_t launch_wconv3(const lg::C3Params& c3, hipStream_t s) {
  return c3.colstats ? launch_wconv3s<true>(c3, s) : launch_wconv3s<false>(c3, s);
}

}

hipError_t udt_lean_launch_gemm(int cfg, const void* lparams, int smem, int G, int geglu, int ln, hipStream_t s) {
  const lg::LParams& lp = *static_cast<const lg::LParams*>(lparams);
  const bool fp8 = lp.a_scale != nullptr, emit = lp.q8_out != nullptr;
  if (cfg == 7 && emit && !fp8 && !geglu && ln && lp.K == 320) return launch_rowres<5, false, true>(lp, G, s);
  if (fp8 || emit) return cfg == 1 ? launch_lean_mx8(lp, smem, G, geglu != 0, ln != 0, fp8, emit, s) : hipErrorInvalidValue;
  switch (cfg) {
    case 1: return launch_lean<4, 2, 2, 2, 2, 2>(lp, smem, G, geglu != 0, ln != 0, s);
    case 6: return launch_lean<8, 2, 4, 4, 2, 2, 1>(lp, smem, G, geglu != 0, ln != 0, s);
    case 5: return geglu ? hipErrorInvalidValue : launch_lean<4, 4, 1, 1, 5, 2>(lp, smem, G, false, ln != 0, s);
    case 7:
      if (!ln || lp.K != 320) return hipErrorInvalidValue;
      return geglu ? launch_rowres<5, true>(lp, G, s) : launch_rowres<5, false>(lp, G, s);
    default: return hipErrorInvalidValue;
  }
}

hipError_t udt_lean_launch_conv3(const void* c3params, hipStream_t s) {
  const lg::C3Params& c3 = *static_cast<const lg::C3Params*>(c3params);
  return c3.geo == 3 ? launch_wconv3(c3, s) : c3.geo == 2 ? launch_lconv3<16, 8, true>(c3, s)
         : c3.geo == 1 ? launch_lconv3<8, 8, false>(c3, s) : launch_lconv3<16, 8, false>(c3, s);
}
```

udifftext_amd/csrc/lean_params.h:

```cpp
#pragma once

namespace lg {

struct LParams {
  const uint16_t* a;
  const uint16_t* a2;
  const uint16_t* w;
  const float* bias;
  const uint16_t* res;
  const float* rowvec;
  const float* ln_s;
  uint16_t* out;
  int M, N, K;
  int lda, ldw, ldo, ldr, ldrv, rows_per_batch;
  float alpha, ln_eps;
  int tiles_m, tiles_n, n_block, tiles;
  int nkt;
  int splitk, kt_per;
  unsigned a_bytes, w_bytes;
  int kt_split, lda2;
  unsigned a2_bytes;
  int G;
  int* counters;
  float* slabs;
  float* colstats;
  const uint32_t* a_scale;
  const float* colscale;
  const float* rowstat_in;
  int rowstat_in_parts;
  uint8_t* q8_out;
  uint32_t* q8_scale;
  int ld_q8;
  int q8_fixed_col;
  float q8_fixed_mul;
  float* rowstat_out;
};

struct C3Params {
  const uint16_t* a;
  const uint16_t* w;
  const float* bias;
  const uint16_t* res;
  const float* rowvec;
  uint16_t* out;
  int N, C;
  int B, H, W;
  int ldw, ldo, ldr, ldrv;
  float alpha;
  int tiles_x, tiles_y, tiles_m, tiles_n, n_block, tiles;
  int chunks, splitk, ch_per;
  unsigned a_bytes, w_bytes;
  int G;
  int* counters;
  float* slabs;
  float* colstats;
  int geo, tw, th;
  int bn, wgm;
  int dbg;
};

}
```

udifftext_amd/csrc/wide.h:

```cpp
#pragma once
#include <type_traits>

namespace wd {

using g8::buf_lds16;
using g8::OOB;
using g8::wait_vm;
using lg::C3Params;
using lg::raw_barrier;
using lg::wait_vm_upto;
using lg::wave_colstats;

struct WGeo {
  static constexpr int TW = 16, TH = 16, NW = 4;
  static constexpr int TM = 2, TN = 5, BN = TN * 32;
  static constexpr int PW = TW + 2, PH = TH + 2, PROWS = PW * PH;
  static constexpr int PIECES = (PROWS + 7) / 8;
  static constexpr int PATCH_BYTES = PIECES * 1024;
  static constexpr int W_BYTES = BN * ROW_BYTES;
  static constexpr int NRING = 3;
  static constexpr int RING = NRING * W_BYTES + 2 * PATCH_BYTES;
  static constexpr int EROW = BN * 4;
  static constexpr int STAGING = NW * 32 * EROW;
  static constexpr int SMEM = RING > STAGING ? RING : STAGING;
  static_assert(SMEM <= 160 * 1024, "one workgroup per CU");
};

template <bool STATS>
__global__ void __launch_bounds__(256, 1) wconv3_kernel(const C3Params p) {
  using G = WGeo;
  constexpr int NW = G::NW, TM = G::TM, TN = G::TN, BN = G::BN, PW = G::PW, NR = G::NRING;
  constexpr int WP = (BN / 8) / NW;
  constexpr int PP = (G::PIECES + NW - 1) / NW;
  constexpr int EROW = G::EROW;
  static_assert((BN / 8) % NW == 0, "weight pieces split evenly over the waves");
  extern __shared__ __attribute__((aligned(16))) char smem[];
  char* const wring = smem;
  char* const patches = smem + NR * G::W_BYTES;

  const int tid = threadIdx.x;
  const int wave = __builtin_amdgcn_readfirstlane(tid >> 6);
  const int lane = tid & 63;
  const int l31 = lane & 31;
  const int hi = lane >> 5;
  const int l3 = lane >> 3;
  const int pslot = lane & 7;
  const int row0 = wave * (TM * 32);
  const int swz_w = (l31 >> 1) & 7;
  const int w_frag_row = l31 * ROW_BYTES;

  const int unit = range_index(blockIdx.x, p.G);
  if (unit >= p.tiles * p.splitk) return;
  const int tile = unit / p.splitk;
  const int slice = unit - tile * p.splitk;
  int tile_m, n0;
  {
    const int per_block = p.tiles_m * p.n_block;
    const int blk = tile / per_block;
    const int r = tile - blk * per_block;
    int nbw = p.tiles_n - blk * p.n_block;
    if (nbw > p.n_block) nbw = p.n_block;
    tile_m = r / nbw;
    n0 = (blk * p.n_block + (r - tile_m * nbw)) * BN;
  }
  const int per_img = p.tiles_x * p.tiles_y;
  const int b = tile_m / per_img;
  const int rt = tile_m - b * per_img;
  const int ty = rt / p.tiles_x;
  const int y0 = ty * G::TH, x0 = (rt - ty * p.tiles_x) * G::TW;
  const int c0 = slice * p.ch_per;
  int c1 = c0 + p.ch_per;
  if (c1 > p.chunks) c1 = p.chunks;

  const __amdgpu_buffer_rsrc_t rsrc_a = __builtin_amdgcn_make_buffer_rsrc(const_cast<uint16_t*>(p.a), 0, p.a_bytes, 0x00020000);
  const __amdgpu_buffer_rsrc_t rsrc_w = __builtin_amdgcn_make_buffer_rsrc(const_cast<uint16_t*>(p.w), 0, p.w_bytes, 0x00020000);
  auto patch_swz = [](int prow, int yy) { return ((prow - 2 * yy) >> 1) & 7; };
  unsigned w_voff[WP], p_voff[PP];
  int p_piece[PP];
#pragma unroll
  for (int i = 0; i < WP; ++i) {
    const int row = (wave + NW * i) * 8 + l3;
    const int kw = (pslot ^ ((row >> 1) & 7)) * 8;
    const int n = n0 + row;
    w_voff[i] = (n < p.N) ? (unsigned)(((long long)n * p.ldw + kw) * 2) : OOB;
  }
#pragma unroll
  for (int i = 0; i < PP; ++i) {
    int idx = wave + NW * i;
    while (idx >= G::PIECES) idx -= NW;
    p_piece[i] = idx;
    const int prow = idx * 8 + l3;
    const int yy = prow / PW;
    const int xx = prow - yy * PW;
    const int gy = y0 + yy - 1, gx = x0 + xx - 1;
    const bool ok = (prow < G::PROWS) && ((unsigned)gy < (unsigned)p.H) && ((unsigned)gx < (unsigned)p.W);
    const int koff = (pslot ^ patch_swz(prow, yy)) * 8;
    p_voff[i] = ok ? (unsigned)(((((long long)b * p.H + gy) * p.W + gx) * p.C + koff) * 2) : OOB;
  }
  int a_prow[TM], a_py[TM];
#pragma unroll
  for (int tm = 0; tm < TM; ++tm) {
    const int ml = row0 + tm * 32 + l31;
    const int py = ml / G::TW, px = ml - py * G::TW;
    a_py[tm] = py;
    a_prow[tm] = py * PW + px;
  }
  auto issue_w = [&](int st, int c, int tap) {
    const int soff = (tap * p.C + c * 64) * 2;
    char* wbuf = wring + st * G::W_BYTES;
#pragma unroll
    for (int i = 0; i < WP; ++i) buf_lds16(rsrc_w, wbuf + (wave + NW * i) * 1024, w_voff[i], soff);
  };
  auto issue_patch = [&](int buf, int c) {
    char* pbuf = patches + buf * G::PATCH_BYTES;
#pragma unroll
    for (int i = 0; i < PP; ++i) buf_lds16(rsrc_a, pbuf + p_piece[i] * 1024, p_voff[i], c * 128);
  };

  f32x16 acc[TM][TN];
#pragma unroll
  for (int i = 0; i < TM; ++i)
#pragma unroll
    for (int j = 0; j < TN; ++j)
#pragma unroll
      for (int r = 0; r < 16; ++r) acc[i][j][r] = 0.f;

  constexpr int PPT = 2, PTAPS = (PP + PPT - 1) / PPT;
  static_assert(PTAPS <= 7, "the next patch is complete two taps before its chunk starts");
  auto issue_patch_part = [&](int buf, int c, int part) {
    char* pbuf = patches + buf * G::PATCH_BYTES;
#pragma unroll
    for (int j = 0; j < PPT; ++j) {
      const int i = part * PPT + j;
      if (i < PP) buf_lds16(rsrc_a, pbuf + p_piece[i] * 1024, p_voff[i], c * 128);
    }
  };
  issue_patch(c0 & 1, c0);
#pragma unroll
  for (int j = 0; j < NR - 1; ++j) issue_w(j, c0, j);
  int st = 0;
  for (int c = c0; c < c1; ++c) {
    const int cn = (c + 1 < c1) ? c + 1 : c;
    const char* pbuf = patches + (c & 1) * G::PATCH_BYTES;
    auto tap_body = [&](auto tap_c) {
      constexpr int tap = decltype(tap_c)::value;
      constexpr auto pcount = [](int t) { const int tt = (t + 9) % 9; return tt < PTAPS ? ((tt + 1) * PPT <= PP ? PPT : PP - tt * PPT) : 0; };
      wait_vm<pcount(tap - 2) + WP + pcount(tap - 1)>();
      raw_barrier();
      const int dy = tap / 3, dx = tap - dy * 3;
      const char* wbuf = wring + st * G::W_BYTES;
      int arow[TM], aswz[TM];
#pragma unroll
      for (int t = 0; t < TM; ++t) {
        const int prow = a_prow[t] + dy * PW + dx;
        arow[t] = prow * ROW_BYTES;
        aswz[t] = patch_swz(prow, a_py[t] + dy);
      }
      bf16x8_t fx[2][TM], fw[2][TN];
      auto read_ks = [&](int ks, int slot2) {
        if (UDT_DBG(p.dbg, 3)) return;
#pragma unroll
        for (int t = 0; t < TM; ++t) fx[slot2][t] = lds_read_frag(pbuf + arow[t] + (((ks * 2 + hi) ^ aswz[t]) << 4));
        const int slot = ((ks * 2 + hi) ^ swz_w) << 4;
#pragma unroll
        for (int t = 0; t < TN; ++t) fw[slot2][t] = lds_read_frag(wbuf + w_frag_row + t * 32 * ROW_BYTES + slot);
      };
      read_ks(0, 0);
#pragma unroll
      for (int ks = 0; ks < 4; ++ks) {
        if (ks + 1 < 4) read_ks(ks + 1, (ks + 1) & 1);
        if (ks == 3) {
          const int ahead = tap + NR - 1;
          int s2 = st + NR - 1;
          if (s2 >= NR) s2 -= NR;
          if (!UDT_DBG(p.dbg, 0)) {
            if (ahead < 9) issue_w(s2, c, ahead);
            else issue_w(s2, cn, ahead - 9);
          }
          if constexpr (tap < PTAPS) {
            if (!UDT_DBG(p.dbg, 1)) issue_patch_part((c + 1) & 1, cn, tap);
          }
        }
        if (UDT_DBG(p.dbg, 2)) {
#pragma unroll
          for (int tm = 0; tm < TM; ++tm) asm volatile("" ::"v"(fx[ks & 1][tm]));
#pragma unroll
          for (int tn = 0; tn < TN; ++tn) asm volatile("" ::"v"(fw[ks & 1][tn]));
        } else {
#pragma unroll
          for (int tm = 0; tm < TM; ++tm)
#pragma unroll
            for (int tn = 0; tn < TN; ++tn) acc[tm][tn] = mfma32(fw[ks & 1][tn], fx[ks & 1][tm], acc[tm][tn]);
        }
      }
      __builtin_amdgcn_sched_group_barrier(0x100, TM + TN, 0);
#pragma unroll
      for (int ks = 0; ks < 3; ++ks) {
#pragma unroll
        for (int i = 0; i < TM + TN; ++i) {
          __builtin_amdgcn_sched_group_barrier(0x008, 1, 0);
          __builtin_amdgcn_sched_group_barrier(0x100, 1, 0);
        }
        __builtin_amdgcn_sched_group_barrier(0x008, TM * TN - (TM + TN), 0);
      }
      constexpr int NV = WP + pcount(tap);
#pragma unroll
      for (int i = 0; i < NV; ++i) {
        __builtin_amdgcn_sched_group_barrier(0x008, 1, 0);
        __builtin_amdgcn_sched_group_barrier(0x020, 1, 0);
      }
      __builtin_amdgcn_sched_group_barrier(0x008, TM * TN - NV, 0);
      st = (st + 1 == NR) ? 0 : st + 1;
    };
    tap_body(std::integral_constant<int, 0>{}); tap_body(std::integral_constant<int, 1>{}); tap_body(std::integral_constant<int, 2>{});
    tap_body(std::integral_constant<int, 3>{}); tap_body(std::integral_constant<int, 4>{}); tap_body(std::integral_constant<int, 5>{});
    tap_body(std::integral_constant<int, 6>{}); tap_body(std::integral_constant<int, 7>{}); tap_body(std::integral_constant<int, 8>{});
  }
  constexpr int CPR = TN * 4;
  constexpr int RPI = 64 / CPR;
  constexpr int NIT = (32 + RPI - 1) / RPI;
  const int rl = lane / CPR;
  const int c8 = lane - rl * CPR;
  const int n = n0 + c8 * 8;
  const bool col_ok = (rl < RPI) && (n < p.N);
  long long mrow[TM][NIT];
  bool rok[TM][NIT];
  u32x4 rv[TM][NIT];
#pragma unroll
  for (int tm = 0; tm < TM; ++tm)
#pragma unroll
    for (int i = 0; i < NIT; ++i) {
      const int row = i * RPI + rl;
      rok[tm][i] = col_ok && row < 32;
      const int ml = row0 + tm * 32 + (row < 32 ? row : 0);
      const int py = ml / G::TW, px = ml - py * G::TW;
      mrow[tm][i] = ((long long)b * p.H + (y0 + py)) * p.W + (x0 + px);
      u32x4 z = {0u, 0u, 0u, 0u};
      rv[tm][i] = z;
      if (p.res && rok[tm][i]) rv[tm][i] = *reinterpret_cast<const u32x4*>(p.res + mrow[tm][i] * p.ldr + n);
    }
  wait_vm<0>();
  raw_barrier();

  if (p.splitk > 1) {
    f32x4* slab = reinterpret_cast<f32x4*>(p.slabs + (long long)unit * (G::TW * G::TH * BN));
#pragma unroll
    for (int tm = 0; tm < TM; ++tm)
#pragma unroll
      for (int tn = 0; tn < TN; ++tn)
#pragma unroll
        for (int q = 0; q < 4; ++q) {
          f32x4 v = {acc[tm][tn][q * 4 + 0], acc[tm][tn][q * 4 + 1], acc[tm][tn][q * 4 + 2], acc[tm][tn][q * 4 + 3]};
          store16_sc1(slab + ((tm * TN + tn) * 4 + q) * 256 + tid, v);
        }
    asm volatile("s_waitcnt vmcnt(0)" ::: "memory");
    __syncthreads();
    int* const bcast = reinterpret_cast<int*>(smem);
    if (tid == 0) {
      const int t = __hip_atomic_fetch_add(p.counters + tile, 1, __ATOMIC_RELAXED, __HIP_MEMORY_SCOPE_AGENT);
      const int last = (t == p.splitk - 1) ? 1 : 0;
      if (last) {
        __builtin_amdgcn_fence(__ATOMIC_ACQUIRE, "agent");
        __hip_atomic_store(p.counters + tile, 0, __ATOMIC_RELAXED, __HIP_MEMORY_SCOPE_AGENT);
      }
      *bcast = last;
    }
    __syncthreads();
    const bool last = *bcast != 0;
    __syncthreads();
    if (!last) return;
#pragma unroll
    for (int i = 0; i < TM; ++i)
#pragma unroll
      for (int j = 0; j < TN; ++j)
#pragma unroll
        for (int r = 0; r < 16; ++r) acc[i][j][r] = 0.f;
    for (int s = 0; s < p.splitk; ++s) {
      const f32x4* sl = reinterpret_cast<const f32x4*>(p.slabs + ((long long)tile * p.splitk + s) * (G::TW * G::TH * BN));
#pragma unroll
      for (int tm = 0; tm < TM; ++tm)
#pragma unroll
        for (int tn = 0; tn < TN; ++tn)
#pragma unroll
          for (int q = 0; q < 4; ++q) {
            const f32x4 v = sl[((tm * TN + tn) * 4 + q) * 256 + tid];
#pragma unroll
            for (int r = 0; r < 4; ++r) acc[tm][tn][q * 4 + r] += v[r];
          }
    }
  }

  char* const wl = smem + wave * (32 * EROW);
  f32x4 b0 = {0.f, 0.f, 0.f, 0.f}, b1 = b0;
  if (col_ok) {
    if (p.bias) {
      b0 = *reinterpret_cast<const f32x4*>(p.bias + n);
      b1 = *reinterpret_cast<const f32x4*>(p.bias + n + 4);
    }
    if (p.rowvec) {
      const float* rvp = p.rowvec + (long long)b * p.ldrv + n;
      const f32x4 r0 = *reinterpret_cast<const f32x4*>(rvp), r1 = *reinterpret_cast<const f32x4*>(rvp + 4);
#pragma unroll
      for (int j = 0; j < 4; ++j) b0[j] += r0[j], b1[j] += r1[j];
    }
  }
  float cs[8], cq[8];
#pragma unroll
  for (int j = 0; j < 8; ++j) cs[j] = cq[j] = 0.f;
#pragma unroll
  for (int tm = 0; tm < TM; ++tm) {
    {
      const int row = l31;
#pragma unroll
      for (int tn = 0; tn < TN; ++tn)
#pragma unroll
        for (int q = 0; q < 4; ++q) {
          const int chunk = (tn * 8 + q * 2 + hi) ^ (row & 7);
          f32x4 v = {acc[tm][tn][q * 4 + 0], acc[tm][tn][q * 4 + 1], acc[tm][tn][q * 4 + 2], acc[tm][tn][q * 4 + 3]};
          *reinterpret_cast<f32x4*>(wl + row * EROW + chunk * 16) = v;
        }
    }
#pragma unroll
    for (int i = 0; i < NIT; ++i) {
      const int row = i * RPI + rl;
      const int rr = row < 32 ? row : 0;
      const char* rp = wl + rr * EROW;
      const int sw = rr & 7;
      const f32x4 v0 = *reinterpret_cast<const f32x4*>(rp + (((2 * c8) ^ sw) << 4));
      const f32x4 v1 = *reinterpret_cast<const f32x4*>(rp + (((2 * c8 + 1) ^ sw) << 4));
      float o[8];
#pragma unroll
      for (int j = 0; j < 4; ++j) {
        o[j] = v0[j] * p.alpha + b0[j];
        o[4 + j] = v1[j] * p.alpha + b1[j];
      }
      if (p.res) {
#pragma unroll
        for (int j = 0; j < 4; ++j) {
          o[2 * j] += bf16_lo(rv[tm][i][j]);
          o[2 * j + 1] += bf16_hi(rv[tm][i][j]);
        }
      }
      if (rok[tm][i]) {
        u32x4 pk = {pack_bf16x2(o[0], o[1]), pack_bf16x2(o[2], o[3]), pack_bf16x2(o[4], o[5]), pack_bf16x2(o[6], o[7])};
        *reinterpret_cast<u32x4*>(p.out + mrow[tm][i] * p.ldo + n) = pk;
        if constexpr (STATS) {
#pragma unroll
          for (int j = 0; j < 4; ++j) {
            const float a = bf16_lo(pk[j]), bb = bf16_hi(pk[j]);
            cs[2 * j] += a; cq[2 * j] += a * a;
            cs[2 * j + 1] += bb; cq[2 * j + 1] += bb * bb;
          }
        }
      }
    }
  }
  if constexpr (STATS) {
    const int slot = tile_m * NW + wave;
    wave_colstats<CPR, RPI>(wl, lane, cs, cq, p.colstats + ((long long)slot * p.N + n) * 2, col_ok);
  }
}

}
```

udifftext_amd/lib.py:

```python
from __future__ import annotations

import ctypes as C
import os

_HERE = os.path.dirname(os.path.abspath(__file__))
LIB_PATH = os.path.join(_HERE, "libudt_kernels.so")

GEMM_OUT_F32 = 1 << 0
DTYPE_F32, DTYPE_BF16, DTYPE_FP8_E4M3 = 0, 1, 2
GEMM_GEGLU = 1 << 1
GEMM_RELU = 1 << 2
GEMM_TRANSPOSED = 1 << 3
GEMM_CONV = 1 << 4
GEMM_SILU_OUT = 1 << 5
GEMM_MX8 = 1 << 7

PROF_CONV3X3, PROF_GEMM, PROF_ATTN, PROF_XATTN, PROF_NORM, PROF_ELEMENTWISE = range(6)


class GemmDesc(C.Structure):
    _fields_ = [
        ("a", C.c_void_p), ("a2", C.c_void_p), ("w", C.c_void_p), ("bias", C.c_void_p),
        ("residual", C.c_void_p), ("rowvec", C.c_void_p), ("out", C.c_void_p),
        ("M", C.c_int32), ("N", C.c_int32), ("K", C.c_int32),
        ("lda", C.c_int32), ("ldo", C.c_int32), ("ldr", C.c_int32), ("ldw", C.c_int32),
        ("batch", C.c_int32),
        ("stride_a", C.c_int64), ("stride_w", C.c_int64), ("stride_out", C.c_int64), ("stride_res", C.c_int64),
        ("Hin", C.c_int32), ("Win", C.c_int32), ("C1", C.c_int32), ("C2", C.c_int32),
        ("Hout", C.c_int32), ("Wout", C.c_int32),
        ("ksize", C.c_int32), ("stride", C.c_int32), ("pad_t", C.c_int32), ("pad_l", C.c_int32),
        ("upsample", C.c_int32), ("rows_per_batch", C.c_int32), ("ld_rowvec", C.c_int32), ("flags", C.c_int32),
        ("alpha", C.c_float), ("colscale", C.c_void_p), ("in_scsh", C.c_void_p), ("in_act", C.c_int32), ("colstats", C.c_void_p),
        ("cu_share", C.c_int32), ("ln_colsum", C.c_void_p), ("ln_eps", C.c_float),
        ("a_scale", C.c_void_p), ("q8_out", C.c_void_p), ("q8_scale", C.c_void_p), ("ld_q8", C.c_int32),
        ("q8_fixed_col", C.c_int32), ("q8_fixed_mul", C.c_float),
        ("rowstat_out", C.c_void_p), ("rowstat_in", C.c_void_p), ("rowstat_in_parts", C.c_int32),
    ]


class SamplerCoefs(C.Structure):
    _fields_ = [("kx", C.c_float), ("kd", C.c_float), ("ka", C.c_float), ("kp", C.c_float), ("kn", C.c_float),
                ("c_out", C.c_float), ("scale", C.c_float)]


MULTISTEP_MAX = 8


class MultistepCoefs(C.Structure):
    _fields_ = [("c_out", C.c_float), ("scale", C.c_float), ("sigma", C.c_float), ("n", C.c_int32),
                ("k", C.c_float * MULTISTEP_MAX), ("hist", C.c_void_p * MULTISTEP_MAX)]


_vp, _i32, _i64, _f32, _fp = C.c_void_p, C.c_int32, C.c_int64, C.c_float, C.c_void_p
SYMBOLS = {
    "udt_gemm_workspace_bytes": (C.c_size_t, [C.POINTER(GemmDesc)]),
    "udt_gemm": (C.c_int, [C.POINTER(GemmDesc), _vp, C.c_size_t, _vp]),
    "udt_gemm_fwd": (C.c_int, [C.POINTER(GemmDesc), _vp, C.c_size_t, _vp]),
    "udt_conv1x1_fwd": (C.c_int, [C.POINTER(GemmDesc), _vp, C.c_size_t, _vp]),
    "udt_workspace_bytes": (C.c_size_t, [C.POINTER(GemmDesc)]),
    "udt_pack_linear": (C.c_int, [_fp, _fp, _i32, _i32, _i32, _i32, C.POINTER(_vp), _vp]),
    "udt_pack_conv": (C.c_int, [_fp, _fp, _i32, _i32, _i32, _i32, C.POINTER(_i32), _i32, _i32, C.POINTER(_vp), _vp]),
    "udt_packed_weight": (_vp, [_vp]),
    "udt_packed_bias": (_vp, [_vp]),
    "udt_packed_colscale": (_vp, [_vp]),
    "udt_packed_dim": (_i32, [_vp, _i32]),
    "udt_free_packed": (C.c_int, [_vp]),
    "udt_check_async_error": (C.c_int, [_vp, C.c_size_t, _vp]),
    "udt_gemm_colstats_rows": (_i32, [C.POINTER(GemmDesc)]),
    "udt_gemm_colstats_slots": (_i32, [C.POINTER(GemmDesc)]),
    "udt_gemm_rowstat_parts": (_i32, [C.POINTER(GemmDesc)]),
    "udt_gemm_q8_ok": (_i32, [C.POINTER(GemmDesc)]),
    "udt_gemm_in_scsh_ok": (_i32, [C.POINTER(GemmDesc)]),
    "udt_gn_silu_conv3x3_fwd": (C.c_int, [C.POINTER(GemmDesc), _vp, C.c_size_t, _vp]),
    "udt_ln_gemm_fwd": (C.c_int, [C.POINTER(GemmDesc), _vp, C.c_size_t, _vp]),
    "udt_gn_finalize": (C.c_int, [_fp, _i32, _i32, _fp, _i32, _i32, _fp, _fp, _fp, _i32, _i64, _i32, _f32, _vp]),
    "udt_gn_apply_scsh": (C.c_int, [_vp, _vp, _vp, _fp, _i32, _i64, _i32, _i32, _i32, _vp]),
    "udt_gn_strip_stats": (C.c_int, [_vp, _vp, _vp, _fp, _i32, _fp, _i32, _fp, _fp, _i32, _i64, _i32, _i32, _i32, _f32, _i32, _vp]),
    "udt_attn_fwd": (C.c_int, [_vp, _vp, _vp, _vp, _i32, _i32, _i32, _i32, _i32, _i32, _i32, _i32,
                               _i64, _i64, _i64, _i64, _f32, _vp]),
    "udt_attn_rowv_fwd": (C.c_int, [_vp, _vp, _vp, _vp, _i32, _i32, _i32, _i32, _i32, _i32, _i32, _i32,
                                    _i64, _i64, _i64, _i64, _f32, _vp]),
    "udt_attn_rowv_q8_fwd": (C.c_int, [_vp, _vp, _vp, _vp, _i32, _i32, _i32, _i32, _i32, _i32, _i32, _i32,
                                       _i64, _i64, _i64, _i64, _f32, _vp, _vp, _i32, _vp]),
    "udt_attn_mx8_fwd": (C.c_int, [_vp, _vp, _vp, _i32, _i32, _i32, _i32, _i32, _f32, _f32, _vp, _vp, _i32, _vp]),
    "udt_attn512_fwd": (C.c_int, [_vp, _vp, _vp, _vp, _i32, _i32, _i32, _i32, _i32, _i32, _i32, _i64, _i64, _i64, _i64, _f32, _vp]),
    "udt_attn512_workspace_bytes": (C.c_size_t, [_i32, _i32, _i32]),
    "udt_attn512_split_fwd": (C.c_int, [_vp, _vp, _vp, _vp, _i32, _i32, _i32, _i32, _i32, _i32, _i32, _i64, _i64, _i64, _i64, _f32,
                                        _vp, C.c_size_t, _vp]),
    "udt_xattn_fwd": (C.c_int, [_vp, _vp, _vp, _vp, _fp, _i32, _i32, _i32, _i32, _i32, _i32, _i32, _i32, _f32, _vp]),
    "udt_mattn_fwd": (C.c_int, [_vp, _vp, _vp, _vp, _fp, _vp, _i32, _i32, _i32, _i32, _i32, _i32, _i32, _i32, _i32, _i32,
                                _i64, _i64, _i64, _i64, _f32, _vp]),
    "udt_softmax_rows": (C.c_int, [_vp, _i64, _i32, _i32, _vp]),
    "udt_tattn_hp": (_i32, [_i32]),
    "udt_tattn_prepare": (C.c_int, [_vp, _i32, _vp, _i32, _vp, _i32, _fp, _fp, _vp, _fp, _vp, _i32, _i32, _i32, _i32, _f32, _vp]),
    "udt_tattn_fused": (C.c_int, [_vp, _vp, _vp, _fp, _vp, _fp, _i32, _i32, _i32, _i32, _i32, _f32, _vp]),
    "udt_tattn_rowstat_parts": (_i32, [_i32, _i32, _i32]),
    "udt_tattn_fused_q8": (C.c_int, [_vp, _vp, _vp, _fp, _vp, _fp, _i32, _i32, _i32, _i32, _i32, _f32, _vp, _vp, _fp, _vp]),
    "udt_gn_nchunks": (_i32, [_i64, _i32]),
    "udt_gn_stats": (C.c_int, [_vp, _vp, _fp, _i32, _i64, _i32, _i32, _i32, _vp]),
    "udt_gn_apply": (C.c_int, [_vp, _vp, _vp, _fp, _fp, _fp, _i32, _i64, _i32, _i32, _i32, _f32, _i32, _vp]),
    "udt_gn_strip_ok": (_i32, [_i32, _i64, _i32, _i32, _i32]),
    "udt_gn_strip": (C.c_int, [_vp, _vp, _vp, _fp, _fp, _i32, _i64, _i32, _i32, _i32, _f32, _i32, _vp]),
    "udt_layernorm": (C.c_int, [_vp, _vp, _fp, _fp, _i64, _i32, _f32, _vp]),
    "udt_unet_input": (C.c_int, [_fp, _vp, _i32, _i32, _i32, _f32, _vp]),
    "udt_cfg_euler_step": (C.c_int, [_fp, _fp, _fp, _i32, _i32, _i32, _f32, _f32, _f32, _f32, _vp]),
    "udt_cfg_sampler_step": (C.c_int, [_fp, _fp, _fp, _fp, _fp, _fp, _fp, _i32, _i32, _i32, SamplerCoefs, _vp]),
    "udt_cfg_multistep_step": (C.c_int, [_fp, _fp, _fp, _fp, _i32, _i32, _i32, MultistepCoefs, _vp]),
    "udt_sampler_step": (C.c_int, [_fp, _fp, _fp, _i32, _i32, _i32, _f32, _f32, _f32, _f32, _vp]),
    "udt_posterior_sample": (C.c_int, [_fp, _fp, _fp, _i32, _i32, _i32, _f32, _vp]),
    "udt_nchw_to_nhwc": (C.c_int, [_fp, _vp, _i32, _i32, _i64, _i32, _f32, _vp]),
    "udt_nhwc_to_nchw": (C.c_int, [_vp, _fp, _i32, _i32, _i64, _i32, _i32, _vp]),
    "udt_nhwc_set_channels": (C.c_int, [_fp, _vp, _i32, _i32, _i64, _i32, _i32, _vp]),
    "udt_embed_tokens": (C.c_int, [_vp, _fp, _fp, _vp, _i32, _i32, _i32, _vp]),
    "udt_timestep_embedding": (C.c_int, [_fp, _vp, _i32, _i32, _vp]),
    "udt_mask_downsample": (C.c_int, [_fp, _fp, _i32, _i32, _i32, _vp]),
    "udt_local_loss": (C.c_int, [_fp, _fp, _fp, _fp, _fp, _i32, _i32, _i32, _i32, _i32, _i32, _i32, _vp]),
    "udt_local_loss_tiled": (C.c_int, [_fp, _fp, _fp, _fp, _fp, _i32, _i32, _i32, _i32, _i32, _i32, _i32, _i32, _vp]),
    "udt_attn_bwd": (C.c_int, [_vp, _vp, _vp, _vp, _vp, _vp, _vp, _vp, _fp, _fp, _i32, _i32, _i32, _i32, _i32, _i32, _f32, _vp]),
    "udt_xattn_bwd": (C.c_int, [_vp, _vp, _fp, _fp, _vp, _vp, _i32, _i32, _i32, _i32, _i32, _i32, _i32, _i32, _f32, _vp]),
    "udt_local_loss_bwd": (C.c_int, [_fp, _fp, _fp, _fp, _fp, _fp, _fp, _i32, _i32, _i32, _i32, _i32, _i32, _i32, _i32, _f32, _vp]),
    "udt_local_loss_bwd_hw": (C.c_int, [_fp, _fp, _fp, _fp, _fp, _fp, _fp, _i32, _i32, _i32, _i32, _i32, _i32, _i32, _i32, _i32, _f32,
                                        _vp]),
    "udt_local_loss_tiled_hw": (C.c_int, [_fp, _fp, _fp, _fp, _fp, _fp, _i32, _i32, _i32, _i32, _i32, _i32, _i32, _i32, _i32, _vp]),
    "udt_layernorm_bwd": (C.c_int, [_vp, _vp, _fp, _vp, _vp, _i64, _i32, _f32, _vp]),
    "udt_gn_bwd": (C.c_int, [_vp, _vp, _fp, _fp, _vp, _vp, _fp, _i32, _i32, _i32, _i32, _f32, _i32, _vp]),
    "udt_geglu_fwd": (C.c_int, [_vp, _vp, _i64, _i32, _vp]),
    "udt_geglu_bwd": (C.c_int, [_vp, _vp, _vp, _i64, _i32, _vp]),
    "udt_sum2x2_bf16": (C.c_int, [_vp, _vp, _i32, _i32, _i32, _i32, _vp]),
    "udt_axpy_f32": (C.c_int, [_fp, _fp, _f32, _i64, _vp]),
    "udt_center_tokens": (C.c_int, [_fp, _vp, _i32, _i32, _i32, _vp]),
    "udt_transpose_bf16": (C.c_int, [_vp, _vp, _i32, _i32, _i32, _i32, _vp]),
    "udt_reduce_rows_f32": (C.c_int, [_fp, _fp, _i32, _i64, _i32, _vp]),
    "udt_colparts": (_i32, [_i64]),
    "udt_colsum_bf16": (C.c_int, [_vp, _fp, _fp, _i64, _i32, _vp]),
    "udt_ln_param_grad": (C.c_int, [_vp, _vp, _fp, _fp, _i64, _i32, _f32, _vp]),
    "udt_xattn_bwd_kv": (C.c_int, [_vp, _vp, _fp, _fp, _vp, _vp, _vp, _fp, _i32, _i32, _i32, _i32, _i32, _i32, _i32, _i32, _i32, _f32, _vp]),
    "udt_xattn_kv_splits": (_i32, [_i32]),
    "udt_wgrad_splits": (_i32, [_i64, _i32, _i32]),
    "udt_wgrad_bf16": (C.c_int, [_vp, _vp, _fp, _fp, _i64, _i32, _i32, _i32, _i32, _vp]),
    "udt_local_loss_seg_bwd": (C.c_int, [_fp, _fp, _fp, _fp, _fp, _fp, _fp, _i32, _i32, _i32, _i32, _i32, _i32, _i32, _f32, _vp]),
    "udt_local_loss_seg_bwd_hw": (C.c_int, [_fp, _fp, _fp, _fp, _fp, _fp, _fp, _i32, _i32, _i32, _i32, _i32, _i32, _i32, _i32, _f32,
                                            _vp]),
    "udt_diff_loss_grad": (C.c_int, [_fp, _fp, _fp, _fp, _vp, _fp, _i32, _i32, _i32, _i32, _vp]),
    "udt_adamw_f32": (C.c_int, [_fp, _fp, _fp, _fp, _i64, _f32, _f32, _f32, _f32, _f32, _i32, _f32, _vp]),
    "udt_add_bf16": (C.c_int, [_vp, _vp, _i64, _vp]),
    "udt_debug_set": (C.c_int, [C.c_char_p, _i32]),
    "udt_bias_add_bf16": (C.c_int, [_vp, _vp, _vp, _i64, _i32, _vp]),
    "udt_version": (C.c_char_p, []),
    "udt_status_string": (C.c_char_p, [C.c_int]),
    "udt_last_hip_error": (C.c_int, []),
    "udt_device_arch_ok": (C.c_int, []),
    "udt_prof_enable": (C.c_int, [C.c_uint32]),
    "udt_prof_reset": (C.c_int, []),
    "udt_prof_trace": (C.c_int, [_i32]),
    "udt_prof_dump": (C.c_int, [C.c_char_p]),
    "udt_prof_get": (C.c_int, [_i32, C.POINTER(C.c_double), C.POINTER(C.c_int64)]),
}

_lib = None


class UdtError(RuntimeError):
    pass


def load() -> C.CDLL:
    global _lib
    if _lib is not None:
        return _lib
    if not os.path.exists(LIB_PATH):
        raise UdtError(
            f"{LIB_PATH} not found: the HIP extension is not built. Run `python -m udifftext_amd.build` "
            "(or __graft_entry__.build()). There is no CPU fallback for the product path.")
    lib = C.CDLL(LIB_PATH)
    for name, (res, args) in SYMBOLS.items():
        fn = getattr(lib, name)
        fn.restype = res
        fn.argtypes = args
    _lib = lib
    return lib


def check(status: int, what: str = "") -> None:
    if status == 0:
        return
    lib = load()
    msg = lib.udt_status_string(status).decode()
    if status == -4:
        msg += f" [hipError {lib.udt_last_hip_error()}]"
    if status in (-1, -2):
        raise ValueError(f"{what}: {msg}")
    raise UdtError(f"{what}: {msg}")
```

udifftext_amd/ops.py:

```python
from __future__ import annotations

import contextlib
import ctypes as C
import os
import threading
from typing import NamedTuple, Optional, Sequence

import torch

from . import lib as L

WORKSPACE_BYTES = 96 << 20


class Workspace:

    def __init__(self, device, nbytes: int = WORKSPACE_BYTES):
        if torch.device(device).type != "cuda":
            raise L.UdtError("udifftext_amd workspaces live on the GPU (no CPU fallback)")
        self.buf = torch.zeros(nbytes, dtype=torch.uint8, device=device)

    def check(self, stream: Optional[int] = None) -> None:
        L.check(L.load().udt_check_async_error(self.buf.data_ptr(), self.buf.numel(), _stream() if stream is None else stream),
                "udt_check_async_error")
# ... 157 lines not shown
    assert x2.dim() == 2 and x2.stride(1) == 1
    M = x2.shape[0]
    N = w.shape[0] if n_out is None else n_out
    assert w.shape[1] == K and w.is_contiguous()
    n_cols = N // 2 if (flags & L.GEMM_GEGLU) else N
    if out is None:
        dt = torch.float32 if (flags & L.GEMM_OUT_F32) else torch.bfloat16
        if flags & L.GEMM_TRANSPOSED:
            assert rows_per_batch > 0
            out = torch.empty((M // rows_per_batch, N, rows_per_batch), dtype=dt, device=x.device)
        else:
            out = torch.empty((M, n_cols), dtype=dt, device=x.device)
    ldo = out.stride(0) if not (flags & L.GEMM_TRANSPOSED) else 0
    d = gemm_desc(a=_ptr(x2), w=_ptr(w), bias=_ptr(bias), residual=_ptr(residual), rowvec=_ptr(rowvec), out=_ptr(out),
                  M=M, N=N, K=K, lda=x2.stride(0), ldo=ldo, ldr=(residual.stride(0) if residual is not None else 0),
                  rows_per_batch=rows_per_batch, ld_rowvec=(rowvec.stride(0) if rowvec is not None else 0), flags=flags,
                  alpha=alpha)
    if not (colstats and rows_per_batch > 0 and out.is_contiguous() and _attach_colstats(d, out, n_cols, rows_per_batch)):
        _drop_stale_stats(out)
    q8 = None
    if emit_q8 and not (flags & (L.GEMM_OUT_F32 | L.GEMM_TRANSPOSED | L.GEMM_GEGLU)) and d.colstats is None and rowvec is None:
        q8 = _attach_q8(d, M, n_cols, x.device, emit_rowstats)
    run_gemm(d, x.device)
    if getattr(out, "mx8", None) is not None:
        del out.mx8
    if q8 is not None:
        out.mx8 = q8
    if WORK_COUNTER is not None:
        count_work("gemm", 2.0 * M * N * K)
        count_work("gemm_bytes", 2.0 * (M * K + N * K) + out.numel() * out.element_size()
                   + (2.0 * M * n_cols if residual is not None else 0.0))
        count_work("gemm_launches", 1.0)
    return out


def linear_mx8(x: Mx8Act, wq: torch.Tensor, colscale: torch.Tensor, bias: Optional[torch.Tensor] = None, *,
               out: Optional[torch.Tensor] = None, residual: Optional[torch.Tensor] = None, rows_per_batch: int = 0,
               flags: int = 0, n_out: Optional[int] = None, colstats: bool = False, emit_q8: bool = False,
               emit_rowstats: bool = False, ln_c: Optional[torch.Tensor] = None, ln_s: Optional[torch.Tensor] = None,
               eps: float = 1e-5, want_bf16: bool = True, q8_fixed: Optional[tuple] = None):
    xq = x.data
    assert xq.dtype == torch.uint8 and wq.dtype == torch.uint8 and xq.is_contiguous() and wq.is_contiguous()
    M, K = xq.shape
    N = wq.shape[0] if n_out is None else n_out
    assert wq.shape[1] == K and K % 128 == 0 and colscale.dtype == torch.float32 and colscale.numel() >= N
    assert x.scale.dtype == torch.int32 and x.scale.shape == (K // 128, M) and x.scale.is_contiguous()
    geglu = bool(flags & L.GEMM_GEGLU)
    n_cols = N // 2 if geglu else N
    only_q8 = emit_q8 and not want_bf16
    if out is None and not only_q8:
        out = torch.empty((M, n_cols), dtype=torch.bfloat16, device=xq.device)
    d = gemm_desc(a=_ptr(xq), w=_ptr(wq), bias=_ptr(ln_c if ln_c is not None else bias), residual=_ptr(residual),
                  out=_ptr(out), M=M, N=N, K=K, lda=K, ldo=(out.stride(0) if out is not None else 0),
                  ldr=(residual.stride(0) if residual is not None else 0), rows_per_batch=rows_per_batch,
                  flags=flags | L.GEMM_MX8, colscale=_ptr(colscale), a_scale=_ptr(x.scale))
    if ln_s is not None:
        if x.stats is None:
            raise L.UdtError("linear_mx8: a LayerNorm-folded MX8 GEMM needs the row statistics of its input (Mx8Act.stats)")
        assert x.stats.dtype == torch.float32 and x.stats.is_contiguous() and x.stats.shape[1:] == (M, 2)
        d.ln_colsum, d.ln_eps = _ptr(ln_s), eps
        d.rowstat_in, d.rowstat_in_parts = _ptr(x.stats), x.stats.shape[0]
    if out is not None and not (colstats and rows_per_batch > 0 and out.is_contiguous()
                                and _attach_colstats(d, out, n_cols, rows_per_batch)):
        _drop_stale_stats(out)
    q8 = None
    if emit_q8:
        q8 = _attach_q8(d, M, n_cols, xq.device, emit_rowstats and not geglu, fixed=q8_fixed)
        if q8 is None:
            raise L.UdtError(f"udt_gemm has no MX8-emitting plan for M={M} N={N} K={K} flags={flags:#x}")
    run_gemm(d, xq.device)
    if out is not None and getattr(out, "mx8", None) is not None:
        del out.mx8
    if WORK_COUNTER is not None:
        count_work("gemm_fp8", 2.0 * M * N * K)
        count_work("gemm_fp8_launches", 1.0)
    if only_q8:
        return q8
    if q8 is not None:
        out.mx8 = q8
    return out


def ln_linear(x: torch.Tensor, w_folded: torch.Tensor, c: torch.Tensor, s: torch.Tensor, *, eps: float = 1e-5,
              out: Optional[torch.Tensor] = None, residual: Optional[torch.Tensor] = None, flags: int = 0,
              n_out: Optional[int] = None, emit_q8: bool = False, want_bf16: bool = True, q8_fixed: Optional[tuple] = None,
              q8_or_none: bool = False):
    _bf16(x); _bf16(w_folded)
    K = x.shape[-1]
    x2 = x.reshape(-1, K) if x.is_contiguous() else x
    assert x2.dim() == 2 and x2.stride(1) == 1 and w_folded.shape[1] == K and w_folded.is_contiguous()
    M = x2.shape[0]
    N = w_folded.shape[0] if n_out is None else n_out
    n_cols = N // 2 if (flags & L.GEMM_GEGLU) else N
    only_q8 = emit_q8 and not want_bf16
    if out is None and not only_q8:
        out = torch.empty((M, n_cols), dtype=torch.bfloat16, device=x.device)
    d = gemm_desc(a=_ptr(x2), w=_ptr(w_folded), bias=_ptr(c), residual=_ptr(residual), out=_ptr(out), M=M, N=N, K=K,
                  lda=x2.stride(0), ldo=(out.stride(0) if out is not None else 0),
                  ldr=(residual.stride(0) if residual is not None else 0), flags=flags, ln_colsum=_ptr(s), ln_eps=eps)
    q8 = None
    if emit_q8:
        q8 = _attach_q8(d, M, n_cols, x.device, False, fixed=q8_fixed)
        if q8 is None:
            if q8_or_none:
                return None
            raise L.UdtError(f"udt_ln_gemm_fwd has no MX8-emitting plan for M={M} N={N} K={K}")
    lib = L.load()
    need = lib.udt_gemm_workspace_bytes(C.byref(d))
    ws_ptr, ws_bytes = None, 0
    if need:
        ws = _ws(need, x.device)
        ws_ptr, ws_bytes = ws.data_ptr(), ws.numel()
    rc = lib.udt_ln_gemm_fwd(C.byref(d), ws_ptr, ws_bytes, _stream())
    if rc in (-1, -2) and x.is_cuda:
        raise L.UdtError(f"udt_ln_gemm_fwd declined M={M} N={N} K={K} flags={flags:#x} (status {rc}): the LayerNorm-folded GEMM "
                         "needs the lean kernel family (UDT_LEAN / udt_debug_set('lean') != 0) and 16-byte aligned operands; "
                         "set UDT_LN_GEMM=0 to run layernorm + GEMM instead")
    L.check(rc, "udt_ln_gemm_fwd")
    if WORK_COUNTER is not None:
        count_work("gemm", 2.0 * M * N * K)
        count_work("gemm_bytes", 2.0 * (M * K + N * K) + (2.0 if out is not None else 0.0) * M * n_cols
                   + (1.0 * M * n_cols if q8 is not None else 0.0) + (2.0 * M * n_cols if residual is not None else 0.0))
        count_work("gemm_launches", 1.0)
    if only_q8:
        return q8
    if q8 is not None:
        out.mx8 = q8
    return out


def bmm_nt(a: torch.Tensor, w: torch.Tensor, *, out: Optional[torch.Tensor] = None, alpha: float = 1.0) -> torch.Tensor:
    _bf16(a); _bf16(w)
    B, M, K = a.shape
    N = w.shape[1]
    assert a.stride(2) == 1 and w.stride(2) == 1 and w.shape[0] == B and w.shape[2] == K
    if out is None:
        out = torch.empty((B, M, N), dtype=torch.bfloat16, device=a.device)
    d = gemm_desc(a=_ptr(a), w=_ptr(w), out=_ptr(out), M=M, N=N, K=K, lda=a.stride(1), ldw=w.stride(1),
                  ldo=out.stride(1), batch=B, stride_a=a.stride(0), stride_w=w.stride(0), stride_out=out.stride(0),
                  alpha=alpha)
    run_gemm(d, a.device)
    if WORK_COUNTER is not None:
        count_work("gemm", 2.0 * B * M * N * K)
        count_work("gemm_bytes", 2.0 * B * (M * K + N * K + M * N))
        count_work("gemm_launches", 1.0)
    return out


def conv2d(x: torch.Tensor, w: torch.Tensor, bias: Optional[torch.Tensor] = None, *, ksize: int = 3, stride: int = 1,
           pad: Optional[tuple] = None, upsample: bool = False, x2: Optional[torch.Tensor] = None,
           out_hw: Optional[tuple] = None, residual: Optional[torch.Tensor] = None,
           rowvec: Optional[torch.Tensor] = None, flags: int = 0, n_out: Optional[int] = None,
           out: Optional[torch.Tensor] = None, colstats: bool = False, in_scsh: Optional[torch.Tensor] = None,
           in_act: int = 0, probe_in_scsh: bool = False):
    _bf16(x); _bf16(w)
    assert x.is_contiguous() and w.is_contiguous()
    B, H, W_, C1 = x.shape
    C2 = 0
    if x2 is not None:
        _bf16(x2)
        assert x2.is_contiguous() and x2.shape[:3] == x.shape[:3]
        C2 = x2.shape[3]
    Hv, Wv = (H * 2, W_ * 2) if upsample else (H, W_)
    if pad is None:
        pad = (ksize // 2, ksize // 2)
    if out_hw is None:
        out_hw = ((Hv + 2 * pad[0] - ksize) // stride + 1, (Wv + 2 * pad[1] - ksize) // stride + 1)
    Ho, Wo = out_hw
    N = w.shape[0] if n_out is None else n_out
    K = ksize * ksize * (C1 + C2)
    assert w.shape[1] == K, (w.shape, K)
    M = B * Ho * Wo
    if out is None and not probe_in_scsh:
        dt = torch.float32 if (flags & L.GEMM_OUT_F32) else torch.bfloat16
        out = torch.empty((B, Ho, Wo, N), dtype=dt, device=x.device)
    d = gemm_desc(a=_ptr(x), a2=_ptr(x2), w=_ptr(w), bias=_ptr(bias), residual=_ptr(residual), rowvec=_ptr(rowvec),
                  out=_ptr(out), M=M, N=N, K=K, lda=0, ldo=(out.stride(2) if out is not None else N),
                  ldr=(residual.stride(2) if residual is not None else 0),
                  Hin=H, Win=W_, C1=C1, C2=C2, Hout=Ho, Wout=Wo, ksize=ksize, stride=stride, pad_t=pad[0], pad_l=pad[1],
                  upsample=1 if upsample else 0, rows_per_batch=Ho * Wo,
                  ld_rowvec=(rowvec.stride(0) if rowvec is not None else 0), flags=flags | L.GEMM_CONV)
    if probe_in_scsh:
        return bool(L.load().udt_gemm_in_scsh_ok(C.byref(d)))
    if in_scsh is not None:
        assert in_scsh.dtype == torch.float32 and in_scsh.is_contiguous() and in_scsh.numel() == B * (C1 + C2) * 2
        d.in_scsh = in_scsh.data_ptr()
        d.in_act = int(in_act)
    if not (colstats and _attach_colstats(d, out, N, Ho * Wo)):
        _drop_stale_stats(out)
    if in_scsh is not None:
        run_gemm(d, x.device, fused_gn=True)
    else:
        run_gemm(d, x.device)
    return out


def attention(q: torch.Tensor, k: torch.Tensor, vt: torch.Tensor, heads: int, scale: float,
              out: Optional[torch.Tensor] = None) -> torch.Tensor:
    _bf16(q); _bf16(k); _bf16(vt)
    B, Nq = q.shape[0], q.shape[1]
    Nk = k.shape[1]
    assert q.stride(2) == 1 and k.stride(2) == 1 and vt.stride(2) == 1
    if out is None:
        out = torch.empty((B, Nq, heads * 64), dtype=torch.bfloat16, device=q.device)
    L.check(L.load().udt_attn_fwd(_ptr(q), _ptr(k), _ptr(vt), _ptr(out), B, heads, Nq, Nk,
                                  q.stride(1), k.stride(1), vt.stride(1), out.stride(1),
                                  q.stride(0), k.stride(0), vt.stride(0), out.stride(0), scale, _stream()),
            "udt_attn_fwd")
    if WORK_COUNTER is not None:
        count_work("attn", 4.0 * B * heads * Nq * Nk * 64)
        count_work("attn_bytes", 2.0 * B * heads * 64 * (2 * Nq + 2 * Nk))
        count_work("attn_launches", 1.0)
    return out


def attention_rowv(q: torch.Tensor, k: torch.Tensor, v: torch.Tensor, heads: int, scale: float,
                   out: Optional[torch.Tensor] = None, emit_q8: bool = False) -> torch.Tensor:
    _bf16(q); _bf16(k); _bf16(v)
    B, Nq = q.shape[0], q.shape[1]
    Nk = k.shape[1]
    assert q.stride(2) == 1 and k.stride(2) == 1 and v.stride(2) == 1 and v.shape[1] == Nk
    if out is None:
        out = torch.empty((B, Nq, heads * 64), dtype=torch.bfloat16, device=q.device)
    if getattr(out, "mx8", None) is not None:
        del out.mx8
    if emit_q8 and heads % 2 == 0 and out.is_contiguous():
        q8 = _mx8_alloc(B * Nq, heads * 64, q.device)
        L.check(L.load().udt_attn_rowv_q8_fwd(_ptr(q), _ptr(k), _ptr(v), _ptr(out), B, heads, Nq, Nk,
                                              q.stride(1), k.stride(1), v.stride(1), out.stride(1),
                                              q.stride(0), k.stride(0), v.stride(0), out.stride(0), scale,
                                              _ptr(q8.data), _ptr(q8.scale), heads * 64, _stream()), "udt_attn_rowv_q8_fwd")
        out.mx8 = q8
    else:
        L.check(L.load().udt_attn_rowv_fwd(_ptr(q), _ptr(k), _ptr(v), _ptr(out), B, heads, Nq, Nk,
                                           q.stride(1), k.stride(1), v.stride(1), out.stride(1),
                                           q.stride(0), k.stride(0), v.stride(0), out.stride(0), scale, _stream()),
                "udt_attn_rowv_fwd")
    if WORK_COUNTER is not None:
        count_work("attn", 4.0 * B * heads * Nq * Nk * 64)
        count_work("attn_bytes", 2.0 * B * heads * 64 * (2 * Nq + 2 * Nk))
        count_work("attn_launches", 1.0)
    return out


def attention_mx8(qkv: Mx8Act, batch: int, heads: int, scale: float, v_mul: float, out: Optional[torch.Tensor] = None,
                  emit_q8: bool = False) -> torch.Tensor:
    C_ = heads * 64
    M, ld8 = qkv.data.shape
    assert qkv.data.dtype == torch.uint8 and qkv.data.is_contiguous() and ld8 >= 3 * C_ and M % batch == 0
    assert qkv.scale.dtype == torch.int32 and qkv.scale.is_contiguous() and qkv.scale.shape == ((ld8 + 127) // 128, M)
    N = M // batch
    if out is None:
        out = torch.empty((batch, N, C_), dtype=torch.bfloat16, device=qkv.data.device)
    assert out.is_contiguous()
    if getattr(out, "mx8", None) is not None:
        del out.mx8
    q8 = _mx8_alloc(M, C_, qkv.data.device) if emit_q8 else None
    L.check(L.load().udt_attn_mx8_fwd(_ptr(qkv.data), _ptr(qkv.scale), _ptr(out), batch, heads, N, ld8, out.stride(1), scale,
                                      1.0 / v_mul, _ptr(q8.data) if q8 else None, _ptr(q8.scale) if q8 else None, C_, _stream()),
            "udt_attn_mx8_fwd")
    if q8 is not None:
        out.mx8 = q8
    if WORK_COUNTER is not None:
        count_work("attn_fp8", 4.0 * batch * heads * N * N * 64)
        count_work("attn_fp8_bytes", 1.0 * batch * heads * 64 * 3 * N + 2.0 * batch * heads * 64 * N)
        count_work("attn_fp8_launches", 1.0)
    return out


def attention_d512(q: torch.Tensor, k: torch.Tensor, v: torch.Tensor, scale: float,
                   out: Optional[torch.Tensor] = None, key_split: bool = True) -> torch.Tensor:
    _bf16(q); _bf16(k); _bf16(v)
    B, Nq = q.shape[0], q.shape[1]
    Nk = k.shape[1]
    assert q.shape[2] == 512 and k.shape[2] == 512 and v.shape[2] == 512 and v.shape[1] == Nk
    assert q.stride(2) == 1 and k.stride(2) == 1 and v.stride(2) == 1
    if out is None:
        out = torch.empty((B, Nq, 512), dtype=torch.bfloat16, device=q.device)
    lib = L.load()
    need = int(lib.udt_attn512_workspace_bytes(B, Nq, Nk)) if key_split else 0
    if need:
        scratch = torch.empty((need,), dtype=torch.uint8, device=q.device)
        L.check(lib.udt_attn512_split_fwd(_ptr(q), _ptr(k), _ptr(v), _ptr(out), B, Nq, Nk,
                                          q.stride(1), k.stride(1), v.stride(1), out.stride(1),
                                          q.stride(0), k.stride(0), v.stride(0), out.stride(0), scale, _ptr(scratch), need, _stream()),
                "udt_attn512_split_fwd")
    else:
        L.check(lib.udt_attn512_fwd(_ptr(q), _ptr(k), _ptr(v), _ptr(out), B, Nq, Nk,
                                    q.stride(1), k.stride(1), v.stride(1), out.stride(1),
                                    q.stride(0), k.stride(0), v.stride(0), out.stride(0), scale, _stream()),
                "udt_attn512_fwd")
    if WORK_COUNTER is not None:
        count_work("attn", 4.0 * B * Nq * Nk * 512)
        count_work("attn_bytes", 2.0 * B * 512 * (2 * Nq + 2 * Nk))
        count_work("attn_launches", 1.0)
    return out


def xattention(q: torch.Tensor, k: torch.Tensor, v: torch.Tensor, heads: int, head_dim: int, scale: float,
               probs: Optional[torch.Tensor] = None, out: Optional[torch.Tensor] = None) -> torch.Tensor:
    _bf16(q); _bf16(k); _bf16(v)
    B, Nq = q.shape[0], q.shape[1]
    Lc = k.shape[1]
    assert q.is_contiguous() or (q.stride(2) == 1 and q.stride(0) == Nq * q.stride(1))
    assert k.stride(2) == 1 and v.stride(2) == 1 and k.stride(1) == v.stride(1)
    assert k.stride(0) == Lc * k.stride(1) and v.stride(0) == Lc * v.stride(1)
    if out is None:
        out = torch.empty((B, Nq, heads * head_dim), dtype=torch.bfloat16, device=q.device)
    if probs is not None:
        assert probs.dtype == torch.float32 and probs.is_contiguous() and probs.numel() == B * heads * Nq * Lc
    L.check(L.load().udt_xattn_fwd(_ptr(q), _ptr(k), _ptr(v), _ptr(out), _ptr(probs), B, heads, head_dim, Nq, Lc,
                                   q.stride(1), k.stride(1), out.stride(1), scale, _stream()), "udt_xattn_fwd")
    return out


def masked_attention(q: torch.Tensor, k: torch.Tensor, v: torch.Tensor, heads: int, scale: float,
                     mask: Optional[torch.Tensor] = None, key_padding_mask: Optional[torch.Tensor] = None,
                     out: Optional[torch.Tensor] = None) -> torch.Tensor:
    _bf16(q); _bf16(k); _bf16(v)
    B, Nq, Cq = q.shape
    Lk = k.shape[1]
    D = Cq // heads
    assert q.stride(2) == 1 and k.stride(2) == 1 and v.stride(2) == 1
    if out is None:
        out = torch.empty((B, Nq, heads * D), dtype=torch.bfloat16, device=q.device)
    if mask is not None:
        mask = mask.float().contiguous()
        assert mask.shape == (Nq, Lk)
    if key_padding_mask is not None:
        key_padding_mask = key_padding_mask.to(torch.uint8).contiguous()
        assert key_padding_mask.shape == (B, Lk)
    L.check(L.load().udt_mattn_fwd(_ptr(q), _ptr(k), _ptr(v), _ptr(out), _ptr(mask), _ptr(key_padding_mask), B, heads, D,
                                   Nq, Lk, q.stride(1), k.stride(1), v.stride(1), out.stride(1), Lk,
                                   q.stride(0), k.stride(0), v.stride(0), out.stride(0), scale, _stream()), "udt_mattn_fwd")
    return out

# ... 545 lines not shown
```

udifftext_amd/packing.py:

```python
from __future__ import annotations

import torch

KPAD = 64


def _round_up(v: int, m: int) -> int:
    return (v + m - 1) // m * m


def pad_channels(c: int) -> int:
    return _round_up(c, KPAD)


def pack_linear(w: torch.Tensor, n_pad_to: int = 4) -> torch.Tensor:
    N, K = w.shape
    Np, Kp = _round_up(N, n_pad_to), _round_up(K, KPAD)
    out = torch.zeros((Np, Kp), dtype=torch.bfloat16, device=w.device)
    out[:N, :K] = w.to(torch.bfloat16)
    return out.contiguous()


def pack_conv(w: torch.Tensor, segments=None, n_pad_to: int = 4) -> torch.Tensor:
    N, Cin, kh, kw = w.shape
    if segments is None:
        segments = [Cin]
    assert sum(segments) == Cin
    Np = _round_up(N, n_pad_to)
    parts = []
    c0 = 0
    for seg in segments:
        sp = pad_channels(seg)
        blk = torch.zeros((Np, kh, kw, sp), dtype=torch.bfloat16, device=w.device)
        blk[:N, :, :, :seg] = w[:, c0:c0 + seg].permute(0, 2, 3, 1).to(torch.bfloat16)
        parts.append(blk)
        c0 += seg
    out = torch.cat(parts, dim=3) if len(parts) > 1 else parts[0]
    return out.reshape(Np, -1).contiguous()


def pad_bias(b: torch.Tensor | None, n_pad_to: int = 4) -> torch.Tensor | None:
    if b is None:
        return None
    N = b.shape[0]
    Np = _round_up(N, n_pad_to)
    out = torch.zeros((Np,), dtype=torch.float32, device=b.device)
    out[:N] = b.float()
    return out


def geglu_permutation(inner: int) -> torch.Tensor:
    assert inner % 32 == 0
    blocks = inner // 32
    idx = torch.empty((blocks, 2, 32), dtype=torch.long)
    base = torch.arange(32)
    for k in range(blocks):
        idx[k, 0] = 32 * k + base
        idx[k, 1] = inner + 32 * k + base
    return idx.reshape(-1)


def pack_geglu(w: torch.Tensor, b: torch.Tensor):
    inner = w.shape[0] // 2
    perm = geglu_permutation(inner).to(w.device)
    return pack_linear(w[perm]), b[perm].float().contiguous()


def pack_ln_linear(w: torch.Tensor, b, gamma: torch.Tensor, beta: torch.Tensor, geglu: bool = False):
    wf = w.float()
    bf = torch.zeros((w.shape[0],), dtype=torch.float32, device=w.device) if b is None else b.float()
    if geglu:
        perm = geglu_permutation(w.shape[0] // 2).to(w.device)
        wf, bf = wf[perm], bf[perm]
    wp = pack_linear(wf * gamma.float()[None, :])
    s = wp[:, :w.shape[1]].float().sum(dim=1).contiguous()
    c = pad_bias((wf @ beta.float() + bf).contiguous())
    if c.shape[0] != wp.shape[0]:
        raise ValueError(f"pack_ln_linear: {w.shape[0]} output rows are not a multiple of the bias padding")
    return wp, c, s


FP8_KPAD = 128
FP8_MAX = 448.0


def pack_linear_fp8(w: torch.Tensor, n_pad_to: int = 4):
    N, K = w.shape
    Np, Kp = _round_up(N, n_pad_to), _round_up(K, FP8_KPAD)
    wf = w.float()
    amax = wf.abs().amax(dim=1).clamp_min(1e-12)
    scale = amax / FP8_MAX
    q = (wf / scale[:, None]).clamp(-FP8_MAX, FP8_MAX).to(torch.float8_e4m3fn).view(torch.uint8)
    out = torch.zeros((Np, Kp), dtype=torch.uint8, device=w.device)
    out[:N, :K] = q
    cs = torch.ones((Np,), dtype=torch.float32, device=w.device)
    cs[:N] = scale
    return out.contiguous(), cs


def pack_ln_linear_mx8(w: torch.Tensor, b, gamma: torch.Tensor, beta: torch.Tensor, geglu: bool = False):
    wf = w.float()
    bf = torch.zeros((w.shape[0],), dtype=torch.float32, device=w.device) if b is None else b.float()
    if geglu:
        perm = geglu_permutation(w.shape[0] // 2).to(w.device)
        wf, bf = wf[perm], bf[perm]
    wq, cs = pack_linear_fp8(wf * gamma.float()[None, :])
    s = (wq.view(torch.float8_e4m3fn).float() * cs[:, None]).sum(dim=1).contiguous()
    c = pad_bias((wf @ beta.float() + bf).contiguous())
    if c.shape[0] != wq.shape[0]:
        raise ValueError(f"pack_ln_linear_mx8: {w.shape[0]} output rows are not a multiple of the bias padding")
    return wq, cs, c, s
```

udifftext_amd/prepare.py:

```python
from __future__ import annotations

from typing import Dict

import torch


def _same_weights(a: torch.nn.Module, b: torch.nn.Module) -> bool:
    sa, sb = a.state_dict(), b.state_dict()
    if list(sa.keys()) != list(sb.keys()):
        return False
    return all(sa[k].shape == sb[k].shape and sa[k].device == sb[k].device and bool(torch.equal(sa[k], sb[k])) for k in sa)


def prepare(engine, free_masters: bool = False, dedup_vae: bool = True) -> Dict[str, float]:
    from sgm.modules import hipnn as H
    from sgm.modules.encoders.modules import LatentEncoder
    report = {"vae_deduplicated": 0, "packed_modules": 0, "packed_bytes": 0, "freed_bytes": 0}
    with torch.no_grad():
        if dedup_vae and getattr(engine, "conditioner", None) is not None:
            for emb in engine.conditioner.embedders:
                if isinstance(emb, LatentEncoder) and emb.model is not engine.first_stage_model \
                        and _same_weights(emb.model, engine.first_stage_model):
                    emb.model = engine.first_stage_model
                    report["vae_deduplicated"] += 1
                    engine._vae_alias_prefixes = ("first_stage_model.", "conditioner.embedders.%d.model." % list(engine.conditioner.embedders).index(emb))
        fused = set()
        for m in engine.modules():
            if isinstance(m, H._Packed):
                fused.update(id(c) for c in m.fused_children())
        unet = engine.model.diffusion_model
        fused.update(id(rb.emb_layers[1]) for rb in unet._resblocks)
        roots = [m for m in engine.modules() if isinstance(m, H._Packed) and id(m) not in fused]
        from sgm.modules.attention import BasicTransformerBlock as _BTB
        fold_on = H.LN_GEMM
        ln_only = set()
        if fold_on:
            for m in unet.modules():
                if isinstance(m, _BTB):
                    ln_only.update((id(m.attn1), id(m.ff.net[0])))
            roots = [m for m in roots if id(m) not in ln_only]
        seen = set()
        for m in roots:
            if id(m) in seen:
                continue
            seen.add(id(m))
            report["packed_modules"] += 1
            report["packed_bytes"] += H.nbytes(m.packed())
        report["packed_bytes"] += H.nbytes(unet._emb_pack())
        from sgm.modules.attention import BasicTransformerBlock
        if H.LN_GEMM:
            from sgm.modules.attention import SpatialTransformer
            for m in unet.modules():
                if isinstance(m, BasicTransformerBlock):
                    report["packed_bytes"] += m.prepare_ln()
                elif isinstance(m, SpatialTransformer):
                    report["packed_bytes"] += m.prepare_mx8()
                    report["packed_bytes"] += m.prepare_ffproj()
        if free_masters:
            victims = []
            for m in engine.modules():
                if hasattr(m, "_sources"):
                    H.freeze_layouts(m)
                if isinstance(m, H._Packed):
                    victims += list(m.parameters(recurse=False))
                    if hasattr(m, "own_masters"):
                        victims += m.own_masters()
            done = set()
            for p in victims:
                if id(p) in done:
                    continue
                done.add(id(p))
                report["freed_bytes"] += p.numel() * p.element_size()
                p.data = torch.empty(0, dtype=p.dtype, device=p.device)
    return report
```

udifftext_amd/sgm/modules/diffusionmodules/model.py:

```python
from __future__ import annotations

import os

import torch
import torch.nn as nn

from udifftext_amd import ops, packing

from .. import hipnn as H


def Normalize(in_channels, num_groups=32):
    return H.GroupNorm(num_groups, in_channels, eps=1e-6)


class Upsample(nn.Module):
    def __init__(self, in_channels, with_conv):
        super().__init__()
        assert with_conv
        self.conv = H.Conv2d(in_channels, in_channels, 3, padding=1)
        self.conv.emit_colstats = True

    def forward(self, x):
        return self.conv(x, upsample=True)


class Downsample(nn.Module):
    def __init__(self, in_channels, with_conv):
        super().__init__()
        assert with_conv
        self.conv = H.Conv2d(in_channels, in_channels, 3, stride=2, padding=0)
        self.conv.emit_colstats = True

    def forward(self, x):
        Hh, Ww = x.shape[1], x.shape[2]
        return self.conv(x, pad=(0, 0), out_hw=((Hh + 1 - 3) // 2 + 1, (Ww + 1 - 3) // 2 + 1))


class ResnetBlock(nn.Module):
    def __init__(self, *, in_channels, out_channels=None, conv_shortcut=False, dropout=0.0, temb_channels=512):
        super().__init__()
        if conv_shortcut or temb_channels > 0:
            raise NotImplementedError("VAE blocks run without time embedding / conv shortcut on this path")
        out_channels = in_channels if out_channels is None else out_channels
        self.in_channels, self.out_channels = in_channels, out_channels
        self.norm1 = Normalize(in_channels)
        self.conv1 = H.Conv2d(in_channels, out_channels, 3, padding=1)
        self.norm2 = Normalize(out_channels)
        self.conv2 = H.Conv2d(out_channels, out_channels, 3, padding=1)
        if in_channels != out_channels:
            self.nin_shortcut = H.Conv2d(in_channels, out_channels, 1)

    def forward(self, x, temb=None):
        h = self.conv1(x, norm=self.norm1, norm_silu=True, colstats=True)
        skip = self.nin_shortcut(x) if self.in_channels != self.out_channels else x
        return self.conv2(h, residual=skip, norm=self.norm2, norm_silu=True, colstats=True)


ATTN_FLASH_512 = os.environ.get("UDT_ATTN512", "1")


def _flash512(batch: int, n: int) -> bool:
    return ATTN_FLASH_512 != "0"


class MemoryEfficientAttnBlock(H._Packed):
    def __init__(self, in_channels):
        super().__init__()
        self.in_channels = in_channels
        self.norm = Normalize(in_channels)
        self.q = H.Conv2d(in_channels, in_channels, 1)
        self.k = H.Conv2d(in_channels, in_channels, 1)
        self.v = H.Conv2d(in_channels, in_channels, 1)
        self.proj_out = H.Conv2d(in_channels, in_channels, 1)

    def _sources(self):
        return [p for m in (self.q, self.k, self.v, self.proj_out) for p in (m.weight, m.bias)]

    def fused_children(self):
        return [self.q, self.k, self.v, self.proj_out]

    def _pack(self):
        c = self.in_channels
        f = lambda m: m.weight.reshape(c, c)
        return (H.fuse_rows(f(self.q), f(self.k), f(self.v)), torch.cat([self.q.bias, self.k.bias, self.v.bias]).float().contiguous(),
                packing.pack_linear(f(self.v)), packing.pad_bias(self.v.bias),
                packing.pack_linear(f(self.proj_out)), packing.pad_bias(self.proj_out.bias))

    def forward(self, x, **kwargs):
        B, Hh, Ww, C = x.shape
        N = Hh * Ww
        hn = self.norm(x).reshape(B * N, C)
        wqkv, bqkv, wv, bv, wo, bo = self.packed()
        if C == 512 and _flash512(B, N):
            qkv = ops.linear(hn, wqkv, bqkv).reshape(B, N, 3 * C)
            o = ops.attention_d512(qkv[..., :C], qkv[..., C:2 * C], qkv[..., 2 * C:], C ** -0.5)
        elif C == 64:
            qkv = ops.linear(hn, wqkv, bqkv).reshape(B, N, 3 * C)
            o = ops.attention_rowv(qkv[..., :C], qkv[..., C:2 * C], qkv[..., 2 * C:], 1, C ** -0.5)
        else:
            qk = ops.linear(hn, wqkv[:2 * C], bqkv[:2 * C]).reshape(B, N, 2 * C)
            vt = ops.linear(hn, wv, bv, flags=H.GEMM_TRANSPOSED, rows_per_batch=N)
            o = torch.empty((B, N, C), dtype=torch.bfloat16, device=x.device)
            QB = 1024
            for q0 in range(0, N, QB):
                q1 = min(N, q0 + QB)
                s = ops.bmm_nt(qk[:, q0:q1, :C], qk[..., C:], alpha=C ** -0.5)
                ops.softmax_rows_(s)
                ops.bmm_nt(s, vt, out=o[:, q0:q1])
        out = ops.linear(o.reshape(B * N, C), wo, bo, residual=x.reshape(B * N, C), rows_per_batch=N, colstats=H.want_stats(B, N, C))
        return H.carry_stats(out.reshape(B, Hh, Ww, C), out)


def make_attn(in_channels, attn_type="vanilla", attn_kwargs=None):
    if attn_type in ("vanilla", "vanilla-xformers"):
        return MemoryEfficientAttnBlock(in_channels)
    if attn_type == "none":
        return nn.Identity()
    raise NotImplementedError(f"attn_type {attn_type} is not used by configs/test/textdesign_sd_2.yaml")


class _Level(nn.Module):
    pass


class Encoder(nn.Module):
    def __init__(self, *, ch, out_ch, ch_mult=(1, 2, 4, 8), num_res_blocks, attn_resolutions, dropout=0.0,
                 resamp_with_conv=True, in_channels, resolution, z_channels, double_z=True, use_linear_attn=False,
                 attn_type="vanilla", **ignore_kwargs):
        super().__init__()
        if len(attn_resolutions) or use_linear_attn:
            raise NotImplementedError("level attention is not configured (attn_resolutions: [])")
        self.ch, self.num_resolutions, self.num_res_blocks = ch, len(ch_mult), num_res_blocks
        self.resolution, self.in_channels = resolution, in_channels
        self.conv_in = H.Conv2d(in_channels, ch, 3, padding=1)
        self.conv_in.emit_colstats = True
        in_ch_mult = (1,) + tuple(ch_mult)
        self.down = nn.ModuleList()
        block_in = ch
        for lv in range(self.num_resolutions):
            level = _Level()
            level.block = nn.ModuleList()
            level.attn = nn.ModuleList()
            block_in, block_out = ch * in_ch_mult[lv], ch * ch_mult[lv]
            for _ in range(num_res_blocks):
                level.block.append(ResnetBlock(in_channels=block_in, out_channels=block_out, temb_channels=0, dropout=dropout))
                block_in = block_out
            if lv != self.num_resolutions - 1:
                level.downsample = Downsample(block_in, resamp_with_conv)
            self.down.append(level)
        self.mid = _Level()
        self.mid.block_1 = ResnetBlock(in_channels=block_in, out_channels=block_in, temb_channels=0, dropout=dropout)
        self.mid.attn_1 = make_attn(block_in, attn_type=attn_type)
        self.mid.block_2 = ResnetBlock(in_channels=block_in, out_channels=block_in, temb_channels=0, dropout=dropout)
        self.norm_out = Normalize(block_in)
        self.conv_out = H.Conv2d(block_in, 2 * z_channels if double_z else z_channels, 3, padding=1)

    def forward(self, x):
        h = self.conv_in(x)
        for lv in range(self.num_resolutions):
            for blk in self.down[lv].block:
                h = blk(h)
            if lv != self.num_resolutions - 1:
                h = self.down[lv].downsample(h)
        h = self.mid.block_2(self.mid.attn_1(self.mid.block_1(h)))
        return self.conv_out(h, norm=self.norm_out, norm_silu=True)


class Decoder(nn.Module):
    def __init__(self, *, ch, out_ch, ch_mult=(1, 2, 4, 8), num_res_blocks, attn_resolutions, dropout=0.0,
                 resamp_with_conv=True, in_channels, resolution, z_channels, give_pre_end=False, tanh_out=False,
                 use_linear_attn=False, attn_type="vanilla", **ignorekwargs):
        super().__init__()
        if len(attn_resolutions) or use_linear_attn or give_pre_end or tanh_out:
# ... 38 lines not shown
```

udifftext_amd/sgm/modules/diffusionmodules/openaimodel.py:

```python
from __future__ import annotations

import os

from typing import List, Optional

import torch
import torch.nn as nn

from udifftext_amd import ops, packing

from ...util import default, exists, require_gpu
from .. import hipnn as H
from ..attention import SpatialTransformer
from .util import zero_module

CPAD = packing.KPAD


class Timestep(nn.Module):
    def __init__(self, dim):
        super().__init__()
        self.dim = dim

    def forward(self, t):
        return ops.timestep_embedding(t.float().contiguous(), self.dim)


class TimestepBlock(nn.Module):
    """a module whose forward takes the time-embedding contribution as second argument"""


class Upsample(nn.Module):
    def __init__(self, channels, use_conv, dims=2, out_channels=None, padding=1, third_up=False):
        super().__init__()
        assert dims == 2 and use_conv
        self.channels = channels
        self.out_channels = out_channels or channels
        self.conv = H.Conv2d(channels, self.out_channels, 3, padding=padding)
        self.conv.emit_colstats = True

    def forward(self, x):
        assert x.shape[-1] == self.channels
        return self.conv(x, upsample=True)


class Downsample(nn.Module):
    def __init__(self, channels, use_conv, dims=2, out_channels=None, padding=1, third_down=False):
        super().__init__()
        assert dims == 2 and use_conv
        self.channels = channels
        self.out_channels = out_channels or channels
        self.op = H.Conv2d(channels, self.out_channels, 3, stride=2, padding=padding)
        self.op.emit_colstats = True

    def forward(self, x):
        assert x.shape[-1] == self.channels
        return self.op(x)


class ResBlock(TimestepBlock):
    def __init__(self, channels, emb_channels, dropout, out_channels=None, use_conv=False, use_scale_shift_norm=False,
                 dims=2, up=False, down=False, kernel_size=3, exchange_temb_dims=False, skip_t_emb=False):
        super().__init__()
        if use_scale_shift_norm or up or down or use_conv or skip_t_emb or dims != 2 or kernel_size != 3:
            raise NotImplementedError("ResBlock variant not used by configs/test/textdesign_sd_2.yaml")
        self.channels = channels
        self.emb_channels = emb_channels
        self.out_channels = out_channels or channels
        self.in_layers = nn.Sequential(H.GroupNorm(32, channels), nn.Identity(),
                                       H.Conv2d(channels, self.out_channels, 3, padding=1))
        self.emb_layers = nn.Sequential(nn.Identity(), H.Linear(emb_channels, self.out_channels))
        self.out_layers = nn.Sequential(H.GroupNorm(32, self.out_channels), nn.Identity(), nn.Identity(),
                                        zero_module(H.Conv2d(self.out_channels, self.out_channels, 3, padding=1)))
        if self.out_channels == channels:
            self.skip_connection = nn.Identity()
        else:
            self.skip_connection = H.Conv2d(channels, self.out_channels, 1)

    def forward(self, x, emb_rows, x2=None):
        emb_out = emb_rows[:, self.emb_offset:self.emb_offset + self.out_channels]
        h = self.in_layers[2](x, x2=x2, rowvec=emb_out, norm=self.in_layers[0], norm_silu=True, colstats=True)
        if isinstance(self.skip_connection, nn.Identity):
            assert x2 is None
            skip = x
        else:
            skip = self.skip_connection(x, x2=x2)
        return self.out_layers[3](h, residual=skip, norm=self.out_layers[0], norm_silu=True, colstats=True)


class TimestepEmbedSequential(nn.Sequential, TimestepBlock):
    def forward(self, x, emb_rows=None, t_context=None, v_context=None, x2=None, t_kv=None, emit_map=False,
                zero_ctx_rows=0, t_fused=None):
        for layer in self:
            if isinstance(layer, ResBlock):
                x = layer(x, emb_rows, x2=x2)
                x2 = None
            elif isinstance(layer, SpatialTransformer):
                kv = t_kv[layer.st_index] if t_kv is not None else None
                tf = t_fused[layer.st_index] if t_fused is not None else None
                x = layer(x, t_context, v_context, t_kv=kv, emit_map=emit_map, zero_ctx_rows=zero_ctx_rows, t_fused=tf)
            else:
                x = layer(x)
        return x


class UnifiedUNetModel(nn.Module):
    def __init__(self, in_channels, ctrl_channels, model_channels, out_channels, num_res_blocks, attention_resolutions,
                 dropout=0, channel_mult=(1, 2, 4, 8), save_attn_type=None, save_attn_layers=[], conv_resample=True,
                 dims=2, use_label=None, num_heads=-1, num_head_channels=-1, num_heads_upsample=-1,
                 use_scale_shift_norm=False, resblock_updown=False, transformer_depth=1, t_context_dim=None,
                 v_context_dim=None, num_attention_blocks=None, use_linear_in_transformer=False, adm_in_channels=None,
                 transformer_depth_middle=None):
        super().__init__()
        if ctrl_channels or use_label is not None or resblock_updown or dims != 2 or not conv_resample:
            raise NotImplementedError("option not used by configs/test/textdesign_sd_2.yaml")
        if num_head_channels == -1:
            assert num_heads != -1, "Either num_heads or num_head_channels has to be set"
        self.in_channels, self.ctrl_channels = in_channels, ctrl_channels
        self.model_channels, self.out_channels = model_channels, out_channels
        channel_mult = tuple(channel_mult)
        depth = len(channel_mult) * [transformer_depth]
        depth_mid = default(transformer_depth_middle, depth[-1])
        self.num_res_blocks = len(channel_mult) * [num_res_blocks]
        self.attention_resolutions = tuple(attention_resolutions)
        self.channel_mult = channel_mult
        self.use_label = use_label
        self.num_heads, self.num_head_channels = num_heads, num_head_channels

        ted = model_channels * 4
        self.time_embed = nn.Sequential(H.Linear(model_channels, ted), nn.Identity(), H.Linear(ted, ted))

        def heads_of(ch):
            return (num_heads, ch // num_heads) if num_head_channels == -1 else (ch // num_head_channels, num_head_channels)

        def transformer(ch, d):
            nh, dh = heads_of(ch)
            return SpatialTransformer(ch, nh, dh, depth=d, t_context_dim=t_context_dim, v_context_dim=v_context_dim,
                                      use_linear=use_linear_in_transformer)

        self.input_blocks = nn.ModuleList([TimestepEmbedSequential(H.Conv2d(in_channels, model_channels, 3, padding=1))])
        self.input_blocks[0][0].emit_colstats = True
        chans = [model_channels]
        ch, ds = model_channels, 1
        for level, mult in enumerate(channel_mult):
            for nr in range(self.num_res_blocks[level]):
                layers = [ResBlock(ch, ted, dropout, out_channels=mult * model_channels)]
                ch = mult * model_channels
                if ds in self.attention_resolutions and (not exists(num_attention_blocks) or nr < num_attention_blocks[level]):
                    layers.append(transformer(ch, depth[level]))
                self.input_blocks.append(TimestepEmbedSequential(*layers))
                chans.append(ch)
            if level != len(channel_mult) - 1:
                self.input_blocks.append(TimestepEmbedSequential(Downsample(ch, True, out_channels=ch)))
                chans.append(ch)
                ds *= 2
        self.middle_block = TimestepEmbedSequential(ResBlock(ch, ted, dropout), transformer(ch, depth_mid),
                                                    ResBlock(ch, ted, dropout))
        self.output_blocks = nn.ModuleList([])
        for level, mult in list(enumerate(channel_mult))[::-1]:
            for i in range(self.num_res_blocks[level] + 1):
                ich = chans.pop()
                layers = [ResBlock(ch + ich, ted, dropout, out_channels=model_channels * mult)]
                ch = model_channels * mult
                if ds in self.attention_resolutions and (not exists(num_attention_blocks) or i < num_attention_blocks[level]):
                    layers.append(transformer(ch, depth[level]))
                if level and i == self.num_res_blocks[level]:
                    layers.append(Upsample(ch, True, out_channels=ch))
                    ds //= 2
                self.output_blocks.append(TimestepEmbedSequential(*layers))
        self.out = nn.Sequential(H.GroupNorm(32, ch), nn.Identity(),
                                 zero_module(H.Conv2d(model_channels, out_channels, 3, padding=1)))

        self.attn_type = save_attn_type or []
        self.attn_layers = save_attn_layers
        self.attn_map_cache = []
        for name, module in self.named_modules():
            if any(name.endswith(t) for t in self.attn_type):
                item = {"name": name, "heads": module.heads, "size": None, "hw": None, "attn_map": None}
                self.attn_map_cache.append(item)
                module.attn_map_cache = item
        self.cache_attn_maps = True
        self._resblocks = [m for m in self.modules() if isinstance(m, ResBlock)]
        self._transformers = [m for m in self.modules() if isinstance(m, SpatialTransformer)]
        off = 0
        for rb in self._resblocks:
            rb.emb_offset = off
            off += rb.out_channels
        for i, st in enumerate(self._transformers):
            st.st_index = i

    def clear_attn_map(self):
        for item in self.attn_map_cache:
# ... 92 lines not shown
```

udifftext_amd/sgm/modules/hipnn.py:

```python
from __future__ import annotations

import math
import os
from typing import Optional

import torch
import torch.nn as nn

from udifftext_amd import lib as L
from udifftext_amd import ops, packing

from ..util import init_skipped


def count_flops(kind: str, flops: float) -> None:
    ops.count_work(kind, flops)


FUSE_GN = os.environ.get("UDT_FUSE_GN", "0") != "0"

GN_EPI = os.environ.get("UDT_GN_EPI", "1") != "0" and os.environ.get("UDT_LEAN", "") != "0"
EMIT_STATS = FUSE_GN or GN_EPI


# ... 18 lines not shown

def mx8_width(c: int) -> bool:
    return FP8_LINEARS and LN_GEMM and c % 128 == 0

LN_GEMM = os.environ.get("UDT_LN_GEMM", "1") != "0" and os.environ.get("UDT_LEAN", "") != "0"


def carry_stats(dst: torch.Tensor, src: torch.Tensor) -> torch.Tensor:
    st = ops.gn_stats_of(src)
    if st is not None:
        dst.gn_stats = st
    return dst


def carry_mx8(dst: torch.Tensor, src: torch.Tensor) -> torch.Tensor:
    q = ops.mx8_of(src)
    if q is not None:
        dst.mx8 = q
    return dst


def _init_uniform_(p: torch.Tensor, fan_in: int) -> None:
    if init_skipped():
        return
    bound = 1.0 / math.sqrt(max(fan_in, 1))
    with torch.no_grad():
        p.uniform_(-bound, bound)


class _Layouts(dict):
    frozen = False


def _layouts(mod: nn.Module) -> _Layouts:
    store = mod.__dict__.get("_layouts")
    if store is None:
        store = mod.__dict__["_layouts"] = _Layouts()
    return store


def layout(mod: nn.Module, tag: str, build, *inputs):
    store = _layouts(mod)
    hit = store.get(tag)
    if store.frozen:
        if hit is None:
            raise L.UdtError(f"{type(mod).__name__}: layout {tag!r} was not built before prepare(free_masters=True) released the "
                             "fp32 masters; reload the checkpoint into a fresh engine to change the launch path")
        return hit[1]
    key = [(t.data_ptr(), t._version, t.device) if isinstance(t, torch.Tensor) else t for t in (*mod._sources(), *inputs)]
    if hit is None or hit[0] != key:
        with torch.no_grad():
            hit = store[tag] = (key, build())
    return hit[1]


def has_layout(mod: nn.Module, tag: str) -> bool:
    return tag in mod.__dict__.get("_layouts", ())


def freeze_layouts(mod: nn.Module) -> None:
    _layouts(mod).frozen = True


def drop_layouts(root: nn.Module) -> None:
    for m in root.modules():
        store = m.__dict__.get("_layouts")
        if store is not None and not store.frozen:
            store.clear()


def nbytes(*layouts) -> int:
    ts = [t for pk in layouts for t in (pk if isinstance(pk, (tuple, list)) else (pk,))]
    return sum(t.numel() * t.element_size() for t in ts if isinstance(t, torch.Tensor))


class _Packed(nn.Module):

    def _sources(self):
        return self._parameters.values()

    def fused_children(self):
        return []

    def packed(self):
        return layout(self, "plain", self._pack)

    def packed_fp8(self):
        return layout(self, "fp8", self._pack_fp8)

    def packed_ln(self, norm):
        return layout(self, "ln", lambda: self._pack_ln(norm.weight, norm.bias), norm.weight, norm.bias)

    def packed_ln_mx8(self, norm):
        return layout(self, "ln_mx8", lambda: self._pack_ln_mx8(norm.weight, norm.bias), norm.weight, norm.bias)


class Linear(_Packed):
    def __init__(self, in_features: int, out_features: int, bias: bool = True):
        super().__init__()
        self.in_features, self.out_features = in_features, out_features
        self.weight = nn.Parameter(torch.empty(out_features, in_features))
        _init_uniform_(self.weight, in_features)
        if bias:
            self.bias = nn.Parameter(torch.empty(out_features))
            _init_uniform_(self.bias, in_features)
        else:
            self.register_parameter("bias", None)

    def _pack(self):
        return packing.pack_linear(self.weight), packing.pad_bias(self.bias)

    def _pack_fp8(self):
        wq, cs = packing.pack_linear_fp8(self.weight)
        return wq, cs, packing.pad_bias(self.bias)

    def forward(self, x, residual=None, flags: int = 0, out=None, rowvec=None, rows_per_batch: int = 0,
                colstats: bool = False, x8=None, emit_q8: bool = False, emit_rowstats: bool = False):
        if x8 is not None:
            wq, cs, b = self.packed_fp8()
            M = x8.data.shape[0]
            if colstats:
                rpb = rows_per_batch if rows_per_batch > 0 else M
                colstats = want_stats(M // rpb, rpb, wq.shape[0])
            return ops.linear_mx8(x8, wq, cs, b, residual=residual, flags=flags, out=out, rows_per_batch=rows_per_batch,
                                  colstats=bool(colstats), emit_q8=emit_q8, emit_rowstats=emit_rowstats)
        w, b = self.packed()
        if colstats:
            rpb = rows_per_batch if rows_per_batch > 0 else x.shape[0]
            colstats = want_stats(x.shape[0] // rpb, rpb, w.shape[0])
        return ops.linear(x, w, b, residual=residual, flags=flags, out=out, rowvec=rowvec, rows_per_batch=rows_per_batch,
                          colstats=bool(colstats), emit_q8=emit_q8, emit_rowstats=emit_rowstats)


class Conv2d(_Packed):

    def __init__(self, in_channels: int, out_channels: int, kernel_size: int, stride: int = 1, padding: int = 0):
        super().__init__()
        self.in_channels, self.out_channels = in_channels, out_channels
        self.kernel_size, self.stride, self.padding = kernel_size, stride, padding
        self.weight = nn.Parameter(torch.empty(out_channels, in_channels, kernel_size, kernel_size))
        self.bias = nn.Parameter(torch.empty(out_channels))
        fan_in = in_channels * kernel_size * kernel_size
        _init_uniform_(self.weight, fan_in)
        _init_uniform_(self.bias, fan_in)
        self.segments = None
        self.n_pad = 4
        self.emit_colstats = False

    def _pack(self):
        return packing.pack_conv(self.weight, self.segments, self.n_pad), packing.pad_bias(self.bias, self.n_pad)

    def packed(self):
        return layout(self, "plain", self._pack, self.segments, self.n_pad)

    def forward(self, x, x2=None, residual=None, rowvec=None, upsample: bool = False, flags: int = 0,
                pad: Optional[tuple] = None, out_hw: Optional[tuple] = None, norm: Optional["GroupNorm"] = None,
                norm_silu: bool = False, colstats: Optional[bool] = None):
        if x2 is not None and self.segments is None and (x.shape[-1] % 64 != 0 or x2.shape[-1] % 64 != 0):
            self.segments = (x.shape[-1], x2.shape[-1])
        w, b = self.packed()
        if pad is None:
            pad = (self.padding, self.padding)
        if colstats is None:
            colstats = self.emit_colstats
        if colstats:
            oh, ow = out_hw if out_hw is not None else ((x.shape[1] * (2 if upsample else 1) + 2 * pad[0] - self.kernel_size) // self.stride + 1,
                                                        (x.shape[2] * (2 if upsample else 1) + 2 * pad[1] - self.kernel_size) // self.stride + 1)
            colstats = want_stats(x.shape[0], oh * ow, w.shape[0])
        colstats = bool(colstats)
        kw = dict(ksize=self.kernel_size, stride=self.stride, pad=pad, upsample=upsample, out_hw=out_hw, residual=residual,
                  rowvec=rowvec, flags=flags, n_out=w.shape[0], colstats=colstats)
        in_scsh = None
        if norm is not None:
            st1, st2 = ops.gn_stats_of(x), ops.gn_stats_of(x2)
            if (FUSE_GN and st1 is not None and (x2 is None or st2 is not None)
                    and ops.conv2d(x, w, b, x2=x2, probe_in_scsh=True, **kw)):
                B = x.shape[0]
                in_scsh = ops.gn_finalize(st1, x.shape[-1], st2, x2.shape[-1] if x2 is not None else 0, norm.weight,
                                          norm.bias, B, x.shape[1] * x.shape[2], norm.num_groups, norm.eps)
                count_flops("fused_gn_convs", 1)
            else:
                x, x2 = norm(x, x2=x2, silu=norm_silu), None
        out = ops.conv2d(x, w, b, x2=x2, in_scsh=in_scsh, in_act=1 if norm_silu else 0, **kw)
        if ops.WORK_COUNTER is not None:
            k = self.kernel_size
            kind = "conv3x3" if k == 3 else "conv1x1"
            npix_out = out.shape[0] * out.shape[1] * out.shape[2]
            count_flops(kind, 2.0 * npix_out * self.out_channels * self.in_channels * k * k)
            nbytes = 2.0 * x.numel() / x.shape[-1] * self.in_channels + 2.0 * self.weight.numel() \
                + npix_out * self.out_channels * (4.0 if (flags & L.GEMM_OUT_F32) else 2.0)
            if residual is not None:
                nbytes += 2.0 * npix_out * self.out_channels
            count_flops(kind + "_bytes", nbytes)
            Hh, Ww = x.shape[1], x.shape[2]
            if (k == 3 and self.stride == 1 and not upsample and tuple(pad) == (1, 1)
                    and self.out_channels > 64 and not (flags & L.GEMM_OUT_F32)
                    and ((Ww % 32 == 0 and Hh % 8 == 0) or (Ww % 16 == 0 and Hh % 16 == 0) or (Ww == 8 and Hh == 8))):
                count_flops("conv3p_bytes", nbytes)
                count_flops("conv3p_launches", 1.0)
        return out


class GroupNorm(nn.Module):
    def __init__(self, num_groups: int, num_channels: int, eps: float = 1e-5):
        super().__init__()
        self.num_groups, self.num_channels, self.eps = num_groups, num_channels, eps
        self.weight = nn.Parameter(torch.ones(num_channels))
        self.bias = nn.Parameter(torch.zeros(num_channels))

    def forward(self, x, x2=None, silu: bool = False):
        if GN_EPI:
            st1, st2 = ops.gn_stats_of(x), ops.gn_stats_of(x2)
            C1, C2 = x.shape[-1], (x2.shape[-1] if x2 is not None else 0)
            HW = x.numel() // (x.shape[0] * C1)
            if (st1 is not None and (x2 is None or st2 is not None)
                    and (ops.gn_strip_ok(x.shape[0], HW, C1, C2, self.num_groups)
                         or ((C1 + C2) % 64 == 0 and (C1 + C2) // self.num_groups <= 128))):
                count_flops("gn_from_epilogue_stats", 1)
                return ops.group_norm_from_stats(x, st1, self.weight, self.bias, self.num_groups, self.eps, silu, x2=x2, st2=st2)
        return ops.group_norm(x, self.weight, self.bias, self.num_groups, self.eps, silu, x2=x2)


class LayerNorm(nn.Module):
    def __init__(self, dim: int, eps: float = 1e-5):
        super().__init__()
        self.dim, self.eps = dim, eps
        self.weight = nn.Parameter(torch.ones(dim))
        self.bias = nn.Parameter(torch.zeros(dim))

    def forward(self, x):
        return ops.layer_norm(x, self.weight, self.bias, self.eps)


def fuse_rows(*weights: torch.Tensor) -> torch.Tensor:
    return packing.pack_linear(torch.cat(list(weights), dim=0))


GEMM_GEGLU = L.GEMM_GEGLU
GEMM_OUT_F32 = L.GEMM_OUT_F32
GEMM_RELU = L.GEMM_RELU
GEMM_TRANSPOSED = L.GEMM_TRANSPOSED
GEMM_SILU_OUT = L.GEMM_SILU_OUT
```

Measured before the change: 10.64 images/s.

## Run nearest-upsample 3x3 convs as four 2x2 phase convolutions on low-res input

```diff
diff --git a/include/udt_kernels.h b/include/udt_kernels.h
--- a/include/udt_kernels.h
+++ b/include/udt_kernels.h
@@ -79,6 +79,7 @@
 int32_t udt_gemm_q8_ok(const udt_gemm_desc* d);
 int32_t udt_gemm_colstats_slots(const udt_gemm_desc* d);
 int32_t udt_gemm_in_scsh_ok(const udt_gemm_desc* d);
+int32_t udt_gemm_up4_ok(const udt_gemm_desc* d);
 int udt_gn_silu_conv3x3_fwd(const udt_gemm_desc* d, void* workspace, size_t workspace_bytes, void* stream);
 int udt_ln_gemm_fwd(const udt_gemm_desc* d, void* workspace, size_t workspace_bytes, void* stream);
 int udt_check_async_error(void* workspace, size_t workspace_bytes, void* stream);
diff --git a/udifftext_amd/csrc/gemm.hip b/udifftext_amd/csrc/gemm.hip
--- a/udifftext_amd/csrc/gemm.hip
+++ b/udifftext_amd/csrc/gemm.hip
@@ -904,14 +904,18 @@
   if (d->C2 != 0 || d->in_scsh || d->colscale || d->batch > 1) return false;
   if (want_stats && !lean_stats_enabled()) return false;
   if (d->N < 128 || d->N % 8 != 0 || d->C1 <= 0 || d->C1 % 64 != 0) return false;
-  const bool ups = d->upsample != 0;
-  if (d->Hout != (d->Hin << (ups ? 1 : 0)) || d->Wout != (d->Win << (ups ? 1 : 0))) return false;
+  if (d->upsample != 0 && d->upsample != 1 && d->upsample != 2) return false;
+  const bool phase = d->upsample == 2, ups = d->upsample == 1;
+  const int nph = phase ? 4 : 1;
+  if (d->Hout != (d->Hin << (d->upsample ? 1 : 0)) || d->Wout != (d->Win << (d->upsample ? 1 : 0))) return false;
+  if (phase && d->ldw > 0 && d->ldw < 4 * d->C1) return false;
+  const int Ht = phase ? d->Hin : d->Hout, Wt = phase ? d->Win : d->Wout;
   c.bn = 128; c.wgm = 2;
   bool wide = false;
   int wide_slots = device_cus();
   {
     const int wm = wide_conv_mode();
-    if (wm != 0 && !ups && d->N % 160 == 0 && d->Wout % 16 == 0 && d->Hout % 16 == 0) {
+    if (wm != 0 && !ups && d->N % 160 == 0 && Wt % 16 == 0 && Ht % 16 == 0) {
       const int cus = device_cus(), share = d->cu_share > 1 ? d->cu_share : 1;
       wide_slots = cus / share > 0 ? cus / share : 1;
       const long long wt = (long long)(d->M / 256) * (d->N / 160);
@@ -922,12 +926,15 @@
       wide = (wm > 0) || (sk <= 2 && eff >= ((share >= 3 && share_of(d) >= 3) ? wide_lanes_eff() : 0.85));
     }
   }
-  if (wide) { c.geo = 3; c.tw = 16; c.th = 16; c.bn = 160; c.wgm = 4; }
-  else if (d->Wout % 16 == 0 && d->Hout % 8 == 0) { c.geo = ups ? 2 : 0; c.tw = 16; c.th = 8; }
-  else if (!ups && d->Wout % 8 == 0 && d->Hout % 8 == 0) { c.geo = 1; c.tw = 8; c.th = 8; }
+  if (wide) { c.geo = phase ? 6 : 3; c.tw = 16; c.th = 16; c.bn = 160; c.wgm = 4; }
+  else if (Wt % 16 == 0 && Ht % 8 == 0) { c.geo = ups ? 2 : phase ? 4 : 0; c.tw = 16; c.th = 8; }
+  else if (!ups && Wt % 8 == 0 && Ht % 8 == 0) { c.geo = phase ? 5 : 1; c.tw = 8; c.th = 8; }
   else return false;
   if (d->ldo % 8 != 0 || (d->residual && d->ldr % 8 != 0)) return false;
-  const long long ldw = d->ldw > 0 ? d->ldw : d->K;
+  const long long ldw = d->ldw > 0 ? d->ldw : (phase ? 4LL * d->C1 : (long long)d->K);
+  if (ldw % 8 != 0) return false;
+  c.w_phase = phase ? (d->stride_w > 0 ? d->stride_w : (long long)d->N * ldw) : 0;
+  if (phase && (c.w_phase < (long long)d->N * ldw || c.w_phase % 8 != 0)) return false;
   if ((long long)d->M * d->C1 * 2 >= (1LL << 31) || (long long)d->N * ldw * 2 >= (1LL << 31)) return false;
   if ((reinterpret_cast<uintptr_t>(d->out) | reinterpret_cast<uintptr_t>(d->residual) | reinterpret_cast<uintptr_t>(d->bias) |
        reinterpret_cast<uintptr_t>(d->rowvec)) & 15) return false;
@@ -939,19 +946,19 @@
   c.N = d->N; c.C = d->C1; c.H = d->Hin; c.W = d->Win; c.B = d->M / (d->Hout * d->Wout);
   c.ldw = (int)ldw; c.ldo = d->ldo; c.ldr = d->ldr; c.ldrv = d->ld_rowvec > 0 ? d->ld_rowvec : d->N;
   c.alpha = d->alpha;
-  c.tiles_x = d->Wout / c.tw; c.tiles_y = d->Hout / c.th;
+  c.tiles_x = Wt / c.tw; c.tiles_y = Ht / c.th;
   c.tiles_m = c.B * c.tiles_x * c.tiles_y;
   c.tiles_n = (d->N + c.bn - 1) / c.bn;
   c.tiles = c.tiles_m * c.tiles_n;
   c.chunks = c.C / 64;
-  const int slots = c.geo == 3 ? wide_slots : (2 * device_cus() / share_of(d) > 0 ? 2 * device_cus() / share_of(d) : 1);
-  int sk = conv_chunk_slices(c.tiles, slots, c.chunks, lean_splitk_knob());
-  while (sk > 1 && (long long)c.tiles * sk * c.tw * c.th * c.bn * 4 > (64LL << 20)) --sk;
+  const int slots = wide ? wide_slots : (2 * device_cus() / share_of(d) > 0 ? 2 * device_cus() / share_of(d) : 1);
+  int sk = conv_chunk_slices((long long)c.tiles * nph, slots, c.chunks, lean_splitk_knob());
+  while (sk > 1 && (long long)c.tiles * nph * sk * c.tw * c.th * c.bn * 4 > (64LL << 20)) --sk;
   c.ch_per = (c.chunks + sk - 1) / sk;
   c.splitk = (c.chunks + c.ch_per - 1) / c.ch_per;
-  c.G = round_workgroups(c.tiles * c.splitk);
+  c.G = round_workgroups(c.tiles * nph * c.splitk);
   {
-    const double patch = (double)((ups ? c.tw / 2 : c.tw) + 2) * ((ups ? c.th / 2 : c.th) + 2) * c.C * 2.0, wtile = 9.0 * c.bn * c.C * 2.0;
+    const double patch = (double)((ups ? c.tw / 2 : c.tw) + 2) * ((ups ? c.th / 2 : c.th) + 2) * c.C * 2.0, wtile = (phase ? 4.0 : 9.0) * c.bn * c.C * 2.0;
     int nb = g_n_block.load(std::memory_order_relaxed);
     if (nb <= 0) nb = (int)(std::sqrt(64.0 * patch / wtile) + 0.5);
     if (nb < 1) nb = 1;
@@ -964,8 +971,10 @@
   return true;
 }
 
+int lean_conv_phases(const lg::C3Params& c) { return c.geo >= 4 ? 4 : 1; }
+
 size_t lean_conv_workspace(const lg::C3Params& c) {
-  return c.splitk > 1 ? G8_HEADER_BYTES + (size_t)c.tiles * c.splitk * c.tw * c.th * c.bn * sizeof(float) : 0;
+  return c.splitk > 1 ? G8_HEADER_BYTES + (size_t)c.tiles * lean_conv_phases(c) * c.splitk * c.tw * c.th * c.bn * sizeof(float) : 0;
 }
 
 bool lean_stats_probe(const udt_gemm_desc* d, int& rows, int& slots) {
@@ -974,7 +983,7 @@
     lg::C3Params c3;
     if (lean_conv_plan(d, c3, true)) {
       rows = c3.tw * c3.th / c3.wgm;
-      slots = c3.tiles_m * c3.wgm;
+      slots = c3.tiles_m * c3.wgm * lean_conv_phases(c3);
       return true;
     }
   }
@@ -1053,6 +1062,12 @@
   return conv3p_geometry(d, ge, true) ? 1 : 0;
 }
 
+extern "C" int32_t udt_gemm_up4_ok(const udt_gemm_desc* d) {
+  if (!d || d->upsample != 2) return 0;
+  lg::C3Params c3;
+  return lean_conv_plan(d, c3, d->colstats != nullptr) ? 1 : 0;
+}
+
 extern "C" int udt_gn_silu_conv3x3_fwd(const udt_gemm_desc* d, void* workspace, size_t workspace_bytes, void* stream) {
   if (!d || !(d->flags & UDT_GEMM_CONV) || d->ksize != 3 || d->stride != 1 || d->pad_t != 1 || d->pad_l != 1 || !d->in_scsh)
     return UDT_ERR_BAD_ARG;
@@ -1179,7 +1194,9 @@
   p.M = d->M; p.N = d->N; p.K = d->K;
   p.lda = d->lda; p.ldo = d->ldo; p.ldr = d->ldr;
   p.ldw = d->ldw > 0 ? d->ldw : d->K;
-  if (p.ldw < d->K || p.ldw % 8 != 0) return UDT_ERR_BAD_SHAPE;
+  if (d->upsample == 2) {
+    if (!udt_gemm_up4_ok(d)) return UDT_ERR_BAD_SHAPE;
+  } else if (p.ldw < d->K || p.ldw % 8 != 0) return UDT_ERR_BAD_SHAPE;
   if (mx8 && d->lda < d->K) return UDT_ERR_BAD_SHAPE;
   p.sA = d->stride_a; p.sW = d->stride_w; p.sO = d->stride_out; p.sR = d->stride_res;
   p.Hin = d->Hin; p.Win = d->Win; p.C1 = d->C1; p.C2 = d->C2; p.Hout = d->Hout; p.Wout = d->Wout;
@@ -1255,8 +1272,10 @@
       UdtProfScope profc(cls, s);
       if (profc.rec) {
         char tag[96];
-        snprintf(tag, sizeof(tag), "%s%s M=%d N=%d K=%d %dx%d tile=%dx%d units=%d splitk=%d nb=%d", c3.geo == 3 ? "wconv3" : "lconv3", d->upsample ? "+up" : "", d->M, d->N, d->K,
-                 d->Hin, d->Win, c3.tw, c3.th, c3.tiles * c3.splitk, c3.splitk, c3.n_block);
+        snprintf(tag, sizeof(tag), "%s%s M=%d N=%d K=%d %dx%d tile=%dx%d units=%d splitk=%d nb=%d%s", (c3.geo == 3 || c3.geo == 6) ? "wconv3" : "lconv3",
+                 (d->upsample && c3.geo != 6) ? "+up" : "", d->M, d->N, d->K,
+                 d->Hin, d->Win, c3.tw, c3.th, c3.tiles * lean_conv_phases(c3) * c3.splitk, c3.splitk, c3.n_block,
+                 d->upsample == 2 ? " up4" : "");
         udt_prof_tag(profc.rec, tag);
       }
       const hipError_t ec = udt_lean_launch_conv3(&c3, s);
diff --git a/udifftext_amd/csrc/lean.h b/udifftext_amd/csrc/lean.h
--- a/udifftext_amd/csrc/lean.h
+++ b/udifftext_amd/csrc/lean.h
@@ -626,9 +626,11 @@
   static_assert(SMEM <= 80 * 1024, "two workgroups per CU");
 };
 
-template <int TW, int TH, bool UPS, bool STATS = false>
+template <int TW, int TH, bool UPS, bool STATS = false, bool PHASE = false>
 __global__ void __launch_bounds__(256, 2) lconv3_kernel(const C3Params p) {
+  static_assert(!(UPS && PHASE), "the phase form runs on the low-resolution geometries");
   using Geo = C3Geo<TW, TH, UPS>;
+  constexpr int NT = PHASE ? 4 : 9;
   constexpr int NW = 4, TM = Geo::TM, TN = 2, BN = 128, BMPX = Geo::PX;
   constexpr int C3_PW = Geo::PW, C3_PROWS = Geo::PROWS, C3_PIECES = Geo::PIECES, C3_PATCH_BYTES = Geo::PATCH_BYTES;
   constexpr int C3_W_BYTES = Geo::W_BYTES, C3_TW = TW, C3_TH = TH;
@@ -654,9 +656,12 @@
   const int w_frag_row = (col0 + l31) * ROW_BYTES;
 
   const int unit = range_index(blockIdx.x, p.G);
-  if (unit >= p.tiles * p.splitk) return;
-  const int tile = unit / p.splitk;
-  const int slice = unit - tile * p.splitk;
+  if (unit >= p.tiles * p.splitk * (PHASE ? 4 : 1)) return;
+  const int phase = PHASE ? unit / (p.tiles * p.splitk) : 0;
+  const int pha = phase >> 1, phb = phase & 1;
+  const int ptile = unit / p.splitk;
+  const int slice = unit - ptile * p.splitk;
+  const int tile = ptile - phase * p.tiles;
   int tile_m, n0;
   {
     const int per_block = p.tiles_m * p.n_block;
@@ -677,7 +682,8 @@
   if (c1 > p.chunks) c1 = p.chunks;
 
   const __amdgpu_buffer_rsrc_t rsrc_a = __builtin_amdgcn_make_buffer_rsrc(const_cast<uint16_t*>(p.a), 0, p.a_bytes, 0x00020000);
-  const __amdgpu_buffer_rsrc_t rsrc_w = __builtin_amdgcn_make_buffer_rsrc(const_cast<uint16_t*>(p.w), 0, p.w_bytes, 0x00020000);
+  const __amdgpu_buffer_rsrc_t rsrc_w =
+      __builtin_amdgcn_make_buffer_rsrc(const_cast<uint16_t*>(p.w) + (PHASE ? (long long)phase * p.w_phase : 0LL), 0, p.w_bytes, 0x00020000);
   auto patch_swz = [](int prow, int yy) { return ((prow - 2 * yy) >> 1) & 7; };
   unsigned w_voff[WP], p_voff[PP];
   int p_piece[PP];
@@ -706,8 +712,8 @@
   for (int tm = 0; tm < TM; ++tm) {
     const int ml = row0 + tm * 32 + l31;
     const int py = ml / TW, px = ml - py * TW;
-    a_py[tm] = py;
-    a_prow[tm] = UPS ? (py | (px << 16)) : (py * C3_PW + px);
+    a_py[tm] = PHASE ? py + pha : py;
+    a_prow[tm] = UPS ? (py | (px << 16)) : PHASE ? ((py + pha) * C3_PW + px + phb) : (py * C3_PW + px);
   }
   auto issue_w = [&](int st, int c, int tap) {
     const int soff = (tap * p.C + c * 64) * 2;
@@ -732,14 +738,15 @@
   issue_patch(c0);
 #pragma unroll
   for (int j = 0; j < NR - 1; ++j) issue_w(j, c0, j);
+  static_assert(NR - 1 < NT, "the ring's prologue stays inside the first chunk");
   int st = 0;
   for (int c = c0; c < c1; ++c) {
     const bool nxt = (c + 1 < c1);
     const char* pbuf = patches + (c & 1) * C3_PATCH_BYTES;
 #pragma unroll
-    for (int tap = 0; tap < 9; ++tap) {
+    for (int tap = 0; tap < NT; ++tap) {
       {
-        const int w_ahead = nxt ? NR - 2 : ((8 - tap) < NR - 2 ? (8 - tap) : NR - 2);
+        const int w_ahead = nxt ? NR - 2 : ((NT - 1 - tap) < NR - 2 ? (NT - 1 - tap) : NR - 2);
         const bool patch_ahead = nxt && tap >= 1 && tap <= NR - 1;
         wait_vm_upto<(NR - 2) * WP + PP>(w_ahead * WP + (patch_ahead ? PP : 0));
       }
@@ -748,11 +755,11 @@
         const int ahead = tap + NR - 1;
         int s2 = st + NR - 1;
         if (s2 >= NR) s2 -= NR;
-        if (ahead < 9) issue_w(s2, c, ahead);
-        else if (nxt) issue_w(s2, c + 1, ahead - 9);
+        if (ahead < NT) issue_w(s2, c, ahead);
+        else if (nxt) issue_w(s2, c + 1, ahead - NT);
       }
       if (tap == 0 && nxt && !UDT_DBG(p.dbg, 1)) issue_patch(c + 1);
-      const int dy = tap / 3, dx = tap - dy * 3;
+      const int dy = PHASE ? tap >> 1 : tap / 3, dx = PHASE ? tap & 1 : tap - dy * 3;
       const char* wbuf = wring + st * C3_W_BYTES;
       bf16x8_t fx[4][TM], fw[4][TN];
       if (!UDT_DBG(p.dbg, 3)) {
@@ -814,11 +821,11 @@
     __syncthreads();
     int* const bcast = reinterpret_cast<int*>(smem);
     if (tid == 0) {
-      const int t = __hip_atomic_fetch_add(p.counters + tile, 1, __ATOMIC_RELAXED, __HIP_MEMORY_SCOPE_AGENT);
+      const int t = __hip_atomic_fetch_add(p.counters + ptile, 1, __ATOMIC_RELAXED, __HIP_MEMORY_SCOPE_AGENT);
       const int last = (t == p.splitk - 1) ? 1 : 0;
       if (last) {
         __builtin_amdgcn_fence(__ATOMIC_ACQUIRE, "agent");
-        __hip_atomic_store(p.counters + tile, 0, __ATOMIC_RELAXED, __HIP_MEMORY_SCOPE_AGENT);
+        __hip_atomic_store(p.counters + ptile, 0, __ATOMIC_RELAXED, __HIP_MEMORY_SCOPE_AGENT);
       }
       *bcast = last;
     }
@@ -833,7 +840,7 @@
 #pragma unroll
         for (int r = 0; r < 16; ++r) acc[i][j][r] = 0.f;
     for (int s = 0; s < p.splitk; ++s) {
-      const f32x4* sl = reinterpret_cast<const f32x4*>(p.slabs + ((long long)tile * p.splitk + s) * (BMPX * BN));
+      const f32x4* sl = reinterpret_cast<const f32x4*>(p.slabs + ((long long)ptile * p.splitk + s) * (BMPX * BN));
 #pragma unroll
       for (int tm = 0; tm < TM; ++tm)
 #pragma unroll
@@ -877,13 +884,14 @@
     }
   }
   constexpr int NIT = TM * 4;
-  const int Ho = UPS ? 2 * p.H : p.H, Wo = UPS ? 2 * p.W : p.W;
+  const int Ho = (UPS || PHASE) ? 2 * p.H : p.H, Wo = (UPS || PHASE) ? 2 * p.W : p.W;
   long long mrow[NIT];
 #pragma unroll
   for (int i = 0; i < NIT; ++i) {
     const int ml = row0 + i * 8 + rl;
     const int py = ml / TW, px = ml - py * TW;
-    mrow[i] = ((long long)b * Ho + (y0 + py)) * Wo + (x0 + px);
+    mrow[i] = PHASE ? ((long long)b * Ho + (2 * (y0 + py) + pha)) * Wo + (2 * (x0 + px) + phb)
+                    : ((long long)b * Ho + (y0 + py)) * Wo + (x0 + px);
   }
   u32x4 rv[NIT];
   if (p.res) {
@@ -931,7 +939,7 @@
     }
   }
   if constexpr (STATS) {
-    const int slot = tile_m * 2 + wm;
+    const int slot = (PHASE ? (b * 4 + phase) * per_img + rt : tile_m) * 2 + wm;
     wave_colstats<8, 8>(wl, lane, cs, cq, p.colstats + ((long long)slot * p.N + n) * 2, col_ok);
   }
 }
diff --git a/udifftext_amd/csrc/lean.hip b/udifftext_amd/csrc/lean.hip
--- a/udifftext_amd/csrc/lean.hip
+++ b/udifftext_amd/csrc/lean.hip
@@ -60,27 +60,27 @@
   return emit ? launch_lean_mx8_k<false, false, false, true, true>(lp, smem, G, s) : launch_lean_mx8_k<false, false, false, true, false>(lp, smem, G, s);
 }
 
-template <int TW, int TH, bool UPS, bool STATS>
+template <int TW, int TH, bool UPS, bool STATS, bool PHASE>
 hipError_t launch_lconv3s(const lg::C3Params& c3, hipStream_t s) {
   static AttrOnce once;
   constexpr int smem = lg::C3Geo<TW, TH, UPS>::SMEM;
-  hipError_t e = once.ensure(reinterpret_cast<const void*>(lg::lconv3_kernel<TW, TH, UPS, STATS>), smem);
+  hipError_t e = once.ensure(reinterpret_cast<const void*>(lg::lconv3_kernel<TW, TH, UPS, STATS, PHASE>), smem);
   if (e != hipSuccess) return e;
-  hipLaunchKernelGGL((lg::lconv3_kernel<TW, TH, UPS, STATS>), dim3(c3.G), dim3(256), smem, s, c3);
+  hipLaunchKernelGGL((lg::lconv3_kernel<TW, TH, UPS, STATS, PHASE>), dim3(c3.G), dim3(256), smem, s, c3);
   return hipGetLastError();
 }
-template <int TW, int TH, bool UPS>
+template <int TW, int TH, bool UPS, bool PHASE = false>
 hipError_t launch_lconv3(const lg::C3Params& c3, hipStream_t s) {
-  return c3.colstats ? launch_lconv3s<TW, TH, UPS, true>(c3, s) : launch_lconv3s<TW, TH, UPS, false>(c3, s);
+  return c3.colstats ? launch_lconv3s<TW, TH, UPS, true, PHASE>(c3, s) : launch_lconv3s<TW, TH, UPS, false, PHASE>(c3, s);
 }
 
-template <bool STATS>
+template <bool STATS, bool PHASE>
 hipError_t launch_wconv3s(const lg::C3Params& c3, hipStream_t s) {
   static AttrOnce once;
   constexpr int smem = wd::WGeo::SMEM;
-  hipError_t e = once.ensure(reinterpret_cast<const void*>(wd::wconv3_kernel<STATS>), smem);
+  hipError_t e = once.ensure(reinterpret_cast<const void*>(wd::wconv3_kernel<STATS, PHASE>), smem);
   if (e != hipSuccess) return e;
-  hipLaunchKernelGGL((wd::wconv3_kernel<STATS>), dim3(c3.G), dim3(256), smem, s, c3);
+  hipLaunchKernelGGL((wd::wconv3_kernel<STATS, PHASE>), dim3(c3.G), dim3(256), smem, s, c3);
   return hipGetLastError();
 }
 template <int KT, bool GEGLU, bool EMIT = false>
@@ -93,8 +93,9 @@
   return hipGetLastError();
 }
 
+template <bool PHASE>
 hipError_t launch_wconv3(const lg::C3Params& c3, hipStream_t s) {
-  return c3.colstats ? launch_wconv3s<true>(c3, s) : launch_wconv3s<false>(c3, s);
+  return c3.colstats ? launch_wconv3s<true, PHASE>(c3, s) : launch_wconv3s<false, PHASE>(c3, s);
 }
 
 }
@@ -117,6 +118,7 @@
 
 hipError_t udt_lean_launch_conv3(const void* c3params, hipStream_t s) {
   const lg::C3Params& c3 = *static_cast<const lg::C3Params*>(c3params);
-  return c3.geo == 3 ? launch_wconv3(c3, s) : c3.geo == 2 ? launch_lconv3<16, 8, true>(c3, s)
+  return c3.geo == 3 ? launch_wconv3<false>(c3, s) : c3.geo == 6 ? launch_wconv3<true>(c3, s) : c3.geo == 2 ? launch_lconv3<16, 8, true>(c3, s)
+         : c3.geo == 4 ? launch_lconv3<16, 8, false, true>(c3, s) : c3.geo == 5 ? launch_lconv3<8, 8, false, true>(c3, s)
          : c3.geo == 1 ? launch_lconv3<8, 8, false>(c3, s) : launch_lconv3<16, 8, false>(c3, s);
 }
diff --git a/udifftext_amd/csrc/lean_params.h b/udifftext_amd/csrc/lean_params.h
--- a/udifftext_amd/csrc/lean_params.h
+++ b/udifftext_amd/csrc/lean_params.h
@@ -56,6 +56,7 @@
   float* colstats;
   int geo, tw, th;
   int bn, wgm;
+  long long w_phase;
   int dbg;
 };
 
diff --git a/udifftext_amd/csrc/wide.h b/udifftext_amd/csrc/wide.h
--- a/udifftext_amd/csrc/wide.h
+++ b/udifftext_amd/csrc/wide.h
@@ -26,9 +26,10 @@
   static_assert(SMEM <= 160 * 1024, "one workgroup per CU");
 };
 
-template <bool STATS>
+template <bool STATS, bool PHASE = false>
 __global__ void __launch_bounds__(256, 1) wconv3_kernel(const C3Params p) {
   using G = WGeo;
+  constexpr int NT = PHASE ? 4 : 9;
   constexpr int NW = G::NW, TM = G::TM, TN = G::TN, BN = G::BN, PW = G::PW, NR = G::NRING;
   constexpr int WP = (BN / 8) / NW;
   constexpr int PP = (G::PIECES + NW - 1) / NW;
@@ -50,9 +51,12 @@
   const int w_frag_row = l31 * ROW_BYTES;
 
   const int unit = range_index(blockIdx.x, p.G);
-  if (unit >= p.tiles * p.splitk) return;
-  const int tile = unit / p.splitk;
-  const int slice = unit - tile * p.splitk;
+  if (unit >= p.tiles * p.splitk * (PHASE ? 4 : 1)) return;
+  const int phase = PHASE ? unit / (p.tiles * p.splitk) : 0;
+  const int pha = phase >> 1, phb = phase & 1;
+  const int ptile = unit / p.splitk;
+  const int slice = unit - ptile * p.splitk;
+  const int tile = ptile - phase * p.tiles;
   int tile_m, n0;
   {
     const int per_block = p.tiles_m * p.n_block;
@@ -73,7 +77,8 @@
   if (c1 > p.chunks) c1 = p.chunks;
 
   const __amdgpu_buffer_rsrc_t rsrc_a = __builtin_amdgcn_make_buffer_rsrc(const_cast<uint16_t*>(p.a), 0, p.a_bytes, 0x00020000);
-  const __amdgpu_buffer_rsrc_t rsrc_w = __builtin_amdgcn_make_buffer_rsrc(const_cast<uint16_t*>(p.w), 0, p.w_bytes, 0x00020000);
+  const __amdgpu_buffer_rsrc_t rsrc_w =
+      __builtin_amdgcn_make_buffer_rsrc(const_cast<uint16_t*>(p.w) + (PHASE ? (long long)phase * p.w_phase : 0LL), 0, p.w_bytes, 0x00020000);
   auto patch_swz = [](int prow, int yy) { return ((prow - 2 * yy) >> 1) & 7; };
   unsigned w_voff[WP], p_voff[PP];
   int p_piece[PP];
@@ -102,8 +107,8 @@
   for (int tm = 0; tm < TM; ++tm) {
     const int ml = row0 + tm * 32 + l31;
     const int py = ml / G::TW, px = ml - py * G::TW;
-    a_py[tm] = py;
-    a_prow[tm] = py * PW + px;
+    a_py[tm] = PHASE ? py + pha : py;
+    a_prow[tm] = PHASE ? (py + pha) * PW + px + phb : py * PW + px;
   }
   auto issue_w = [&](int st, int c, int tap) {
     const int soff = (tap * p.C + c * 64) * 2;
@@ -125,8 +130,9 @@
 #pragma unroll
       for (int r = 0; r < 16; ++r) acc[i][j][r] = 0.f;
 
-  constexpr int PPT = 2, PTAPS = (PP + PPT - 1) / PPT;
-  static_assert(PTAPS <= 7, "the next patch is complete two taps before its chunk starts");
+  constexpr int PPT = PHASE ? 6 : 2, PTAPS = (PP + PPT - 1) / PPT;
+  static_assert(PTAPS <= NT - 2, "the next patch is complete two taps before its chunk starts");
+  static_assert(NR - 1 < NT, "the ring's prologue stays inside the first chunk");
   auto issue_patch_part = [&](int buf, int c, int part) {
     char* pbuf = patches + buf * G::PATCH_BYTES;
 #pragma unroll
@@ -144,10 +150,10 @@
     const char* pbuf = patches + (c & 1) * G::PATCH_BYTES;
     auto tap_body = [&](auto tap_c) {
       constexpr int tap = decltype(tap_c)::value;
-      constexpr auto pcount = [](int t) { const int tt = (t + 9) % 9; return tt < PTAPS ? ((tt + 1) * PPT <= PP ? PPT : PP - tt * PPT) : 0; };
+      constexpr auto pcount = [](int t) { const int tt = (t + NT) % NT; return tt < PTAPS ? ((tt + 1) * PPT <= PP ? PPT : PP - tt * PPT) : 0; };
       wait_vm<pcount(tap - 2) + WP + pcount(tap - 1)>();
       raw_barrier();
-      const int dy = tap / 3, dx = tap - dy * 3;
+      const int dy = PHASE ? tap >> 1 : tap / 3, dx = PHASE ? tap & 1 : tap - dy * 3;
       const char* wbuf = wring + st * G::W_BYTES;
       int arow[TM], aswz[TM];
 #pragma unroll
@@ -174,8 +180,8 @@
           int s2 = st + NR - 1;
           if (s2 >= NR) s2 -= NR;
           if (!UDT_DBG(p.dbg, 0)) {
-            if (ahead < 9) issue_w(s2, c, ahead);
-            else issue_w(s2, cn, ahead - 9);
+            if (ahead < NT) issue_w(s2, c, ahead);
+            else issue_w(s2, cn, ahead - NT);
           }
           if constexpr (tap < PTAPS) {
             if (!UDT_DBG(p.dbg, 1)) issue_patch_part((c + 1) & 1, cn, tap);
@@ -203,18 +209,22 @@
         }
         __builtin_amdgcn_sched_group_barrier(0x008, TM * TN - (TM + TN), 0);
       }
-      constexpr int NV = WP + pcount(tap);
-#pragma unroll
-      for (int i = 0; i < NV; ++i) {
+      constexpr int NV = WP + pcount(tap), NVI = NV < TM * TN ? NV : TM * TN;
+#pragma unroll
+      for (int i = 0; i < NVI; ++i) {
         __builtin_amdgcn_sched_group_barrier(0x008, 1, 0);
         __builtin_amdgcn_sched_group_barrier(0x020, 1, 0);
       }
-      __builtin_amdgcn_sched_group_barrier(0x008, TM * TN - NV, 0);
+      if constexpr (NV > NVI) __builtin_amdgcn_sched_group_barrier(0x020, NV - NVI, 0);
+      else __builtin_amdgcn_sched_group_barrier(0x008, TM * TN - NV, 0);
       st = (st + 1 == NR) ? 0 : st + 1;
     };
     tap_body(std::integral_constant<int, 0>{}); tap_body(std::integral_constant<int, 1>{}); tap_body(std::integral_constant<int, 2>{});
-    tap_body(std::integral_constant<int, 3>{}); tap_body(std::integral_constant<int, 4>{}); tap_body(std::integral_constant<int, 5>{});
-    tap_body(std::integral_constant<int, 6>{}); tap_body(std::integral_constant<int, 7>{}); tap_body(std::integral_constant<int, 8>{});
+    tap_body(std::integral_constant<int, 3>{});
+    if constexpr (!PHASE) {
+      tap_body(std::integral_constant<int, 4>{}); tap_body(std::integral_constant<int, 5>{});
+      tap_body(std::integral_constant<int, 6>{}); tap_body(std::integral_constant<int, 7>{}); tap_body(std::integral_constant<int, 8>{});
+    }
   }
   constexpr int CPR = TN * 4;
   constexpr int RPI = 64 / CPR;
@@ -234,7 +244,8 @@
       rok[tm][i] = col_ok && row < 32;
       const int ml = row0 + tm * 32 + (row < 32 ? row : 0);
       const int py = ml / G::TW, px = ml - py * G::TW;
-      mrow[tm][i] = ((long long)b * p.H + (y0 + py)) * p.W + (x0 + px);
+      mrow[tm][i] = PHASE ? ((long long)b * (2 * p.H) + (2 * (y0 + py) + pha)) * (2 * p.W) + (2 * (x0 + px) + phb)
+                          : ((long long)b * p.H + (y0 + py)) * p.W + (x0 + px);
       u32x4 z = {0u, 0u, 0u, 0u};
       rv[tm][i] = z;
       if (p.res && rok[tm][i]) rv[tm][i] = *reinterpret_cast<const u32x4*>(p.res + mrow[tm][i] * p.ldr + n);
@@ -257,11 +268,11 @@
     __syncthreads();
     int* const bcast = reinterpret_cast<int*>(smem);
     if (tid == 0) {
-      const int t = __hip_atomic_fetch_add(p.counters + tile, 1, __ATOMIC_RELAXED, __HIP_MEMORY_SCOPE_AGENT);
+      const int t = __hip_atomic_fetch_add(p.counters + ptile, 1, __ATOMIC_RELAXED, __HIP_MEMORY_SCOPE_AGENT);
       const int last = (t == p.splitk - 1) ? 1 : 0;
       if (last) {
         __builtin_amdgcn_fence(__ATOMIC_ACQUIRE, "agent");
-        __hip_atomic_store(p.counters + tile, 0, __ATOMIC_RELAXED, __HIP_MEMORY_SCOPE_AGENT);
+        __hip_atomic_store(p.counters + ptile, 0, __ATOMIC_RELAXED, __HIP_MEMORY_SCOPE_AGENT);
       }
       *bcast = last;
     }
@@ -276,7 +287,7 @@
 #pragma unroll
         for (int r = 0; r < 16; ++r) acc[i][j][r] = 0.f;
     for (int s = 0; s < p.splitk; ++s) {
-      const f32x4* sl = reinterpret_cast<const f32x4*>(p.slabs + ((long long)tile * p.splitk + s) * (G::TW * G::TH * BN));
+      const f32x4* sl = reinterpret_cast<const f32x4*>(p.slabs + ((long long)ptile * p.splitk + s) * (G::TW * G::TH * BN));
 #pragma unroll
       for (int tm = 0; tm < TM; ++tm)
 #pragma unroll
@@ -356,7 +367,7 @@
     }
   }
   if constexpr (STATS) {
-    const int slot = tile_m * NW + wave;
+    const int slot = (PHASE ? (b * 4 + phase) * per_img + rt : tile_m) * NW + wave;
     wave_colstats<CPR, RPI>(wl, lane, cs, cq, p.colstats + ((long long)slot * p.N + n) * 2, col_ok);
   }
 }
diff --git a/udifftext_amd/lib.py b/udifftext_amd/lib.py
--- a/udifftext_amd/lib.py
+++ b/udifftext_amd/lib.py
@@ -71,6 +71,7 @@
     "udt_gemm_rowstat_parts": (_i32, [C.POINTER(GemmDesc)]),
     "udt_gemm_q8_ok": (_i32, [C.POINTER(GemmDesc)]),
     "udt_gemm_in_scsh_ok": (_i32, [C.POINTER(GemmDesc)]),
+    "udt_gemm_up4_ok": (_i32, [C.POINTER(GemmDesc)]),
     "udt_gn_silu_conv3x3_fwd": (C.c_int, [C.POINTER(GemmDesc), _vp, C.c_size_t, _vp]),
     "udt_ln_gemm_fwd": (C.c_int, [C.POINTER(GemmDesc), _vp, C.c_size_t, _vp]),
     "udt_gn_finalize": (C.c_int, [_fp, _i32, _i32, _fp, _i32, _i32, _fp, _fp, _fp, _i32, _i64, _i32, _f32, _vp]),
diff --git a/udifftext_amd/ops.py b/udifftext_amd/ops.py
--- a/udifftext_amd/ops.py
+++ b/udifftext_amd/ops.py
@@ -333,7 +333,7 @@
            out_hw: Optional[tuple] = None, residual: Optional[torch.Tensor] = None,
            rowvec: Optional[torch.Tensor] = None, flags: int = 0, n_out: Optional[int] = None,
            out: Optional[torch.Tensor] = None, colstats: bool = False, in_scsh: Optional[torch.Tensor] = None,
-           in_act: int = 0, probe_in_scsh: bool = False):
+           in_act: int = 0, probe_in_scsh: bool = False, w_up4: Optional[torch.Tensor] = None):
     _bf16(x); _bf16(w)
     assert x.is_contiguous() and w.is_contiguous()
     B, H, W_, C1 = x.shape
@@ -363,6 +363,13 @@
                   ld_rowvec=(rowvec.stride(0) if rowvec is not None else 0), flags=flags | L.GEMM_CONV)
     if probe_in_scsh:
         return bool(L.load().udt_gemm_in_scsh_ok(C.byref(d)))
+    if w_up4 is not None and upsample and ksize == 3 and x2 is None and in_scsh is None:
+        _bf16(w_up4)
+        assert w_up4.is_contiguous() and w_up4.dim() == 3 and w_up4.shape[0] == 4 and w_up4.shape[1] >= N and w_up4.shape[2] == 4 * C1, \
+            (w_up4.shape, N, C1)
+        d.upsample, d.w, d.ldw, d.stride_w = 2, _ptr(w_up4), w_up4.shape[2], w_up4.stride(0)
+        if not L.load().udt_gemm_up4_ok(C.byref(d)):
+            d.upsample, d.w, d.ldw, d.stride_w = 1, _ptr(w), 0, 0
     if in_scsh is not None:
         assert in_scsh.dtype == torch.float32 and in_scsh.is_contiguous() and in_scsh.numel() == B * (C1 + C2) * 2
         d.in_scsh = in_scsh.data_ptr()
diff --git a/udifftext_amd/packing.py b/udifftext_amd/packing.py
--- a/udifftext_amd/packing.py
+++ b/udifftext_amd/packing.py
@@ -37,6 +37,24 @@
         c0 += seg
     out = torch.cat(parts, dim=3) if len(parts) > 1 else parts[0]
     return out.reshape(Np, -1).contiguous()
+
+
+UP4_TAPS = (((0,), (1, 2)), ((0, 1), (2,)))
+
+
+def pack_conv_up4(w: torch.Tensor, n_pad_to: int = 4) -> torch.Tensor:
+    N, Cin, kh, kw = w.shape
+    assert (kh, kw) == (3, 3), "the phase form exists for 3x3 convolutions"
+    Np, Cp = _round_up(N, n_pad_to), pad_channels(Cin)
+    wb = w.to(torch.bfloat16).float()
+    out = torch.zeros((4, Np, 2, 2, Cp), dtype=torch.bfloat16, device=w.device)
+    for a in range(2):
+        for b in range(2):
+            for r in range(2):
+                for s in range(2):
+                    v = sum(wb[:, :, dy, dx] for dy in UP4_TAPS[a][r] for dx in UP4_TAPS[b][s])
+                    out[2 * a + b, :N, r, s, :Cin] = v.to(torch.bfloat16)
+    return out.reshape(4, Np, 4 * Cp).contiguous()
 
 
 def pad_bias(b: torch.Tensor | None, n_pad_to: int = 4) -> torch.Tensor | None:
diff --git a/udifftext_amd/prepare.py b/udifftext_amd/prepare.py
--- a/udifftext_amd/prepare.py
+++ b/udifftext_amd/prepare.py
@@ -46,6 +46,8 @@
             seen.add(id(m))
             report["packed_modules"] += 1
             report["packed_bytes"] += H.nbytes(m.packed())
+            if getattr(m, "upsamples", False):
+                report["packed_bytes"] += H.nbytes(m.packed_up4())
         report["packed_bytes"] += H.nbytes(unet._emb_pack())
         from sgm.modules.attention import BasicTransformerBlock
         if H.LN_GEMM:
diff --git a/udifftext_amd/sgm/modules/diffusionmodules/model.py b/udifftext_amd/sgm/modules/diffusionmodules/model.py
--- a/udifftext_amd/sgm/modules/diffusionmodules/model.py
+++ b/udifftext_amd/sgm/modules/diffusionmodules/model.py
@@ -20,6 +20,7 @@
         assert with_conv
         self.conv = H.Conv2d(in_channels, in_channels, 3, padding=1)
         self.conv.emit_colstats = True
+        self.conv.upsamples = True
 
     def forward(self, x):
         return self.conv(x, upsample=True)
diff --git a/udifftext_amd/sgm/modules/diffusionmodules/openaimodel.py b/udifftext_amd/sgm/modules/diffusionmodules/openaimodel.py
--- a/udifftext_amd/sgm/modules/diffusionmodules/openaimodel.py
+++ b/udifftext_amd/sgm/modules/diffusionmodules/openaimodel.py
@@ -38,6 +38,7 @@
         self.out_channels = out_channels or channels
         self.conv = H.Conv2d(channels, self.out_channels, 3, padding=padding)
         self.conv.emit_colstats = True
+        self.conv.upsamples = True
 
     def forward(self, x):
         assert x.shape[-1] == self.channels
diff --git a/udifftext_amd/sgm/modules/hipnn.py b/udifftext_amd/sgm/modules/hipnn.py
--- a/udifftext_amd/sgm/modules/hipnn.py
+++ b/udifftext_amd/sgm/modules/hipnn.py
@@ -194,6 +194,9 @@
 
     def packed(self):
         return layout(self, "plain", self._pack, self.segments, self.n_pad)
+
+    def packed_up4(self):
+        return layout(self, "up4", lambda: packing.pack_conv_up4(self.weight, self.n_pad), self.n_pad)
 
     def forward(self, x, x2=None, residual=None, rowvec=None, upsample: bool = False, flags: int = 0,
                 pad: Optional[tuple] = None, out_hw: Optional[tuple] = None, norm: Optional["GroupNorm"] = None,
@@ -212,6 +215,8 @@
         colstats = bool(colstats)
         kw = dict(ksize=self.kernel_size, stride=self.stride, pad=pad, upsample=upsample, out_hw=out_hw, residual=residual,
                   rowvec=rowvec, flags=flags, n_out=w.shape[0], colstats=colstats)
+        if upsample and norm is None and x2 is None and self.kernel_size == 3 and self.stride == 1:
+            kw["w_up4"] = self.packed_up4()
         in_scsh = None
         if norm is not None:
             st1, st2 = ops.gn_stats_of(x), ops.gn_stats_of(x2)
```

After: 10.94 images/s (median of 6 runs). +2.8%, better.
